# akofke/fountain

Measured on AMD Instinct MI355X. Metric: Mrays/s (primary+secondary) at fixed spp, higher is better.
Workload: dtype f32

## Files before the change

fountain_amd/csrc/ftn_device.h:

```cpp
#ifndef FTN_DEVICE_H
#define FTN_DEVICE_H

#include <hip/hip_runtime.h>
#include "ftn_math.h"
#include "../../include/fountain_hip.h"

namespace ftn {

#define FTN_DEV_NOINLINE __device__ inline

#define FTN_GS 3
enum : uint32_t { GF_KIND_SPHERE = 1u, GF_HAS_NORMALS = 2u, GF_HAS_UVS = 4u, GF_FLIP = 8u, GF_LEAF_END = 16u , GF_HAS_TANGENTS = 32u  };
enum : uint32_t { LK_POINT = 0, LK_DISTANT = 1, LK_INFINITE = 2, LK_AREA = 3 };

struct DSphere {
    float o2w[16], o2w_inv[16], w2o[16];
    float radius, z_min, z_max, theta_min, theta_max, phi_max;
    uint32_t reverse_orientation, _pad;
};

struct DLight {
    uint32_t kind; int32_t prim;
    float rgb[3];
    float v[3];
    float world_center[3]; float world_radius; float area;
    uint32_t env_w, env_h;
    const float4* texels;
    const float* cond_func;
    const float* cond_cdf;
    const float* cond_integral;
    const float* marg_func;
    const float* marg_cdf;
    float marg_integral; uint32_t nu, nv, _pad;
    float l2w[16], w2l[16];
    const float* cond_coarse; const float* marg_coarse;
    const float4* cells;
};

struct DImage { uint32_t w, h, wrap, n_levels; uint32_t off[16], lw[16], lh[16]; };

struct DScene {
    const float4* nodes; const float4* geom; const uint4* prim_info;
    uint32_t geom_stride, _pad_gs;
    const float* N; const float* UV;
    const float* T;
    const DSphere* spheres; const ftn_material* materials; const DLight* lights;
    uint32_t n_nodes, n_prims, n_lights, n_inf_lights, n_spheres, _pad;
    const uint32_t* inf_lights;
    const float4* fat;
    float root_lo[3], root_hi[3];
    uint32_t root_is_leaf, n_fat;
    const ftn_texture* textures; const ftn_material_textures* mtex; const DImage* images; const float4* texels;
    uint32_t n_textures;
    uint32_t material_types;
    uint32_t env_only, _pad2;
    DLight env0;
    const float4* srec;
    const float4* quad;
    uint32_t n_quads, quad_stack_bound;
    const uint4* oct; const float4* oct_xbox;
    uint32_t n_octs, oct_stack_bound;
    const unsigned char* prim_class;
};

struct DCamera {
    float c2w[16]; float r2c[16];
    float shutter_open, shutter_close, lens_radius, focal_dist;
    float dx_camera[3], dy_camera[3];
};

struct DRay { V3 o, d; float t_max, time; };
struct DHit { float t; int prim; float b0, b1, b2; };
struct DSurfHit { V3 p, p_err, n; float time; };
struct DSI { DSurfHit hit; V3 wo, shading_n, s_dpdu; int prim; int mat, light;  };
struct DSIX { V2 uv; V3 dpdu, dpdv, dndu, dndv; };

__device__ inline DRay spawn_ray(const DSurfHit& h, V3 dir) {
    DRay r; r.o = offset_ray_origin(h.p, h.p_err, h.n, dir); r.d = dir; r.t_max = FTN_INF; r.time = h.time; return r;
}
__device__ inline DRay spawn_ray_to_hit(const DSurfHit& a, const DSurfHit& to) {
    V3 origin = offset_ray_origin(a.p, a.p_err, a.n, to.p - a.p);
    V3 target = offset_ray_origin(to.p, to.p_err, to.n, origin - to.p);
    DRay r; r.o = origin; r.d = target - origin; r.t_max = 1.0f - 0.0001f; r.time = a.time; return r;
}

__device__ inline bool slab_test(float4 nlo, float4 nhi, V3 o, V3 inv, float t_max);
__device__ inline bool slab_test_node(float4 a, float4 b, V3 o, V3 inv, float t_max) {
    return slab_test(make_float4(a.x, a.z, b.x, 0.0f), make_float4(a.y, a.w, b.y, 0.0f), o, inv, t_max);
}
__device__ inline bool slab_test(float4 nlo, float4 nhi, V3 o, V3 inv, float t_max) {
    const float k = 1.0f + 2.0f * gamma_n(3);
    float tnx = (nlo.x - o.x) * inv.x, tfx = (nhi.x - o.x) * inv.x;
    float tny = (nlo.y - o.y) * inv.y, tfy = (nhi.y - o.y) * inv.y;
    float tnz = (nlo.z - o.z) * inv.z, tfz = (nhi.z - o.z) * inv.z;
    if (tnx > tfx) { float s = tnx; tnx = tfx; tfx = s; }
    if (tny > tfy) { float s = tny; tny = tfy; tfy = s; }
    if (tnz > tfz) { float s = tnz; tnz = tfz; tfz = s; }
    tfx *= k; tfy *= k; tfz *= k;
    const float t0 = fmax_(fmax_(fmax_(0.0f, tnx), tny), tnz);
    const float t1 = fmin_(fmin_(fmin_(t_max, tfx), tfy), tfz);
    return !(t0 > t1);
}
__device__ inline bool slab_test_node_iv(float4 a, float4 b, V3 o, V3 inv, float t_max, float* t0o, float* t1o) {
    const float k = 1.0f + 2.0f * gamma_n(3);
    float tnx = (a.x - o.x) * inv.x, tfx = (a.y - o.x) * inv.x;
    float tny = (a.z - o.y) * inv.y, tfy = (a.w - o.y) * inv.y;
    float tnz = (b.x - o.z) * inv.z, tfz = (b.y - o.z) * inv.z;
    if (tnx > tfx) { float s = tnx; tnx = tfx; tfx = s; }
    if (tny > tfy) { float s = tny; tny = tfy; tfy = s; }
    if (tnz > tfz) { float s = tnz; tnz = tfz; tfz = s; }
    tfx *= k; tfy *= k; tfz *= k;
    const float t0 = fmax_(fmax_(fmax_(0.0f, tnx), tny), tnz);
    const float t1 = fmin_(fmin_(fmin_(t_max, tfx), tfy), tfz);
    *t0o = t0; *t1o = t1;
    return !(t0 > t1);
}
__device__ inline void pin4(float4& v) { asm volatile("" : "+v"(v.x), "+v"(v.y), "+v"(v.z), "+v"(v.w)); }

__device__ inline bool tri_hit(V3 o, V3 d, float t_max, V3 p0, V3 p1, V3 p2, float* t_out, float* b0o, float* b1o, float* b2o) {
    V3 p0t = p0 - o, p1t = p1 - o, p2t = p2 - o;
    int kz = max_dimension(vabs(d));
    int kx = kz + 1; if (kx == 3) kx = 0;
    int ky = kx + 1; if (ky == 3) ky = 0;
    V3 dir(d.get(kx), d.get(ky), d.get(kz));
    p0t = V3(p0t.get(kx), p0t.get(ky), p0t.get(kz));
    p1t = V3(p1t.get(kx), p1t.get(ky), p1t.get(kz));
    p2t = V3(p2t.get(kx), p2t.get(ky), p2t.get(kz));
    float sx = -dir.x / dir.z, sy = -dir.y / dir.z, sz = 1.0f / dir.z;
    p0t.x += sx * p0t.z; p0t.y += sy * p0t.z;
    p1t.x += sx * p1t.z; p1t.y += sy * p1t.z;
    p2t.x += sx * p2t.z; p2t.y += sy * p2t.z;
    float e0 = p1t.x * p2t.y - p1t.y * p2t.x;
    float e1 = p2t.x * p0t.y - p2t.y * p0t.x;
    float e2 = p0t.x * p1t.y - p0t.y * p1t.x;
    if (e0 == 0.0f || e1 == 0.0f || e2 == 0.0f) {
        e0 = (float)((double)p1t.x * (double)p2t.y - (double)p1t.y * (double)p2t.x);
        e1 = (float)((double)p2t.x * (double)p0t.y - (double)p2t.y * (double)p0t.x);
        e2 = (float)((double)p0t.x * (double)p1t.y - (double)p0t.y * (double)p1t.x);
    }
    if (sign_pos(e0) != sign_pos(e1) || sign_pos(e1) != sign_pos(e2)) return false;
    float det = e0 + e1 + e2;
    if (det == 0.0f) return false;
    p0t.z *= sz; p1t.z *= sz; p2t.z *= sz;
    float t_scaled = e0 * p0t.z + e1 * p1t.z + e2 * p2t.z;
    if ((det < 0.0f && (t_scaled >= 0.0f || t_scaled < t_max * det)) || (det > 0.0f && (t_scaled <= 0.0f || t_scaled > t_max * det)))
        return false;
    float inv_det = 1.0f / det;
    float b0 = e0 * inv_det, b1 = e1 * inv_det, b2 = e2 * inv_det;
    float t = t_scaled * inv_det;
    float max_zt = fmax_(fmax_(fabsf(p0t.z), fabsf(p1t.z)), fabsf(p2t.z));
    float delta_z = gamma_n(3) * max_zt;
    float max_xt = fmax_(fmax_(fabsf(p0t.x), fabsf(p1t.x)), fabsf(p2t.x));
    float max_yt = fmax_(fmax_(fabsf(p0t.y), fabsf(p1t.y)), fabsf(p2t.y));
    float delta_x = gamma_n(5) * (max_xt + max_zt);
    float delta_y = gamma_n(5) * (max_yt + max_zt);
    float delta_e = 2.0f * (gamma_n(2) * max_xt * max_yt + delta_y * max_xt + delta_x * max_yt);
    float max_e = fmax_(fmax_(fabsf(e0), fabsf(e1)), fabsf(e2));
    float delta_t = 3.0f * (gamma_n(3) * max_e * max_zt + delta_e * max_zt + delta_z * max_e) * fabsf(inv_det);
    if (t <= delta_t) return false;
    *t_out = t; *b0o = b0; *b1o = b1; *b2o = b2;
    return true;
}
__device__ inline void prim_mat_light(const DScene& S, int prim, int* mat, int* light) {
    if (S.srec) { const float4* R = S.srec + 8 * (size_t)prim; *mat = (int)__float_as_uint(R[1].w); *light = (int)__float_as_uint(R[2].w); }
    else { const uint4 pi = S.prim_info[2 * prim]; *mat = (int)pi.x; *light = (int)pi.y; }
}
__device__ inline void prim_normals(const DScene& S, int prim, V3* n0, V3* n1, V3* n2) {
    if (S.srec) { const float4* R = S.srec + 8 * (size_t)prim; const float4 r3 = R[3], r4 = R[4], r5 = R[5]; *n0 = V3(r3.x, r3.y, r3.z); *n1 = V3(r4.x, r4.y, r4.z); *n2 = V3(r5.x, r5.y, r5.z); }
    else { const uint4 vi = S.prim_info[2 * prim + 1]; const float* N = S.N;
           *n0 = V3(N[3 * vi.x], N[3 * vi.x + 1], N[3 * vi.x + 2]); *n1 = V3(N[3 * vi.y], N[3 * vi.y + 1], N[3 * vi.y + 2]); *n2 = V3(N[3 * vi.z], N[3 * vi.z + 1], N[3 * vi.z + 2]); }
}
__device__ inline void prim_uvs(const DScene& S, int prim, float* u0x, float* u0y, float* u1x, float* u1y, float* u2x, float* u2y) {
    if (S.srec) { const float4* R = S.srec + 8 * (size_t)prim; const float4 r6 = R[6]; *u0x = R[3].w; *u0y = R[4].w; *u1x = R[5].w; *u1y = r6.x; *u2x = r6.y; *u2y = r6.z; }
    else { const uint4 vi = S.prim_info[2 * prim + 1]; const float* UV = S.UV;
           *u0x = UV[2 * vi.x]; *u0y = UV[2 * vi.x + 1]; *u1x = UV[2 * vi.y]; *u1y = UV[2 * vi.y + 1]; *u2x = UV[2 * vi.z]; *u2y = UV[2 * vi.z + 1]; }
}
__device__ inline bool tri_uv_degenerate_reject(const DScene& S, int prim, V3 p0, V3 p1, V3 p2) {
    float u0x, u0y, u1x, u1y, u2x, u2y;
    prim_uvs(S, prim, &u0x, &u0y, &u1x, &u1y, &u2x, &u2y);
    float determinant = (u0x - u2x) * (u1y - u2y) - (u0y - u2y) * (u1x - u2x);
    if (!(fabsf(determinant) < 1.0e-8f)) return false;
    V3 ng = cross(p2 - p0, p1 - p0);
    return len2(ng) == 0.0f;
}

__device__ inline bool sphere_clipped(const DSphere& s, V3 p, float phi) {
    return (s.z_min > -s.radius && p.z < s.z_min) || (s.z_max < s.radius && p.z > s.z_max) || phi > s.phi_max;
}
template <bool FILL = true>
FTN_DEV_NOINLINE bool sphere_intersect(const DSphere& s, const DRay& wr, float* t_out, DSI* si, DSIX* ex = nullptr) {
    V3 o_err, d_err;
    V3 ot = m4_point_exact_to_err(s.w2o, wr.o, &o_err);
    V3 dt_ = m4_vector_exact_to_err(s.w2o, wr.d, &d_err);
    float tmax = wr.t_max;
    float lsq = len2(dt_);
    if (lsq > 0.0f) { float dt = dot(vabs(dt_), o_err) / lsq; ot = ot + dt_ * dt; tmax -= dt; }
    EF ox = ef_err(ot.x, o_err.x), oy = ef_err(ot.y, o_err.y), oz = ef_err(ot.z, o_err.z);
    EF dx = ef_err(dt_.x, d_err.x), dy = ef_err(dt_.y, d_err.y), dz = ef_err(dt_.z, d_err.z);
    EF a = dx * dx + dy * dy + dz * dz;
    EF b = EF(2.0f) * (dx * ox + dy * oy + dz * oz);
    EF c = ox * ox + oy * oy + oz * oz - EF(s.radius) * EF(s.radius);
    EF t0, t1;
    if (!quadratic(a, b, c, &t0, &t1)) return false;
    if (t0.hi > tmax || t1.lo <= 0.0f) return false;
    EF th = t0;
    if (th.lo <= 0.0f) { th = t1; if (th.hi > tmax) return false; }
    V3 p = ot + (dt_ * th.v);
    p = p * (s.radius / len(p - V3(0.0f, 0.0f, 0.0f)));
    if (p.x == 0.0f && p.y == 0.0f) p.x = 1.0e-5f * s.radius;
    float phi = ftn_det::atan2f_det(p.y, p.x);
    if (phi < 0.0f) phi += 2.0f * FTN_PI;
    if (sphere_clipped(s, p, phi)) {
        if (th.v == t1.v) return false;
        if (t1.hi > tmax) return false;
// ... 760 lines not shown
```

fountain_amd/csrc/ftn_host.cpp:

```cpp
#include "ftn_kernels.h"
#include "ftn_wavefront.h"
#include "ftn_texture.h"

#include <algorithm>
#include <chrono>
#include <cstdio>
#include <cstring>
#include <string>
#include <vector>
#include <thread>
#include <memory>
#include <sched.h>
#include <atomic>
#include <limits>
#include <functional>
#include <cstdlib>

using namespace ftn;

static_assert(sizeof(ftn_transform) == 128 && sizeof(ftn_pixel) == 16 && sizeof(ftn_bvh_node) == 32 && sizeof(ftn_prim) == 16, "ABI");
static_assert(sizeof(ftn_mesh) == 20 && sizeof(ftn_sphere) == 288 && sizeof(ftn_material) == 48 && sizeof(ftn_light) == 160, "ABI");
static_assert(sizeof(ftn_envmap) == 16 && sizeof(ftn_camera_desc) == 296 && sizeof(ftn_film_desc) == 32 && sizeof(ftn_sampler_desc) == 24, "ABI");
static_assert(sizeof(ftn_integrator_desc) == 16 && sizeof(ftn_tile_range) == 16 && sizeof(ftn_render_options) == 16 && sizeof(ftn_stats) == 152, "ABI");

// ... 334 lines not shown
    }
    if (owners.size() >= (1u << 24)) return;
    out->n_records = (uint32_t)owners.size();
    out->rec.assign((size_t)32 * owners.size(), 0.0f);
    std::vector<uint32_t> bound(owners.size(), 0);
    const float kInf = std::numeric_limits<float>::infinity();
    auto put = [&](float* slot, const ftn_bvh_node* c, uint32_t c_index, uint32_t axis_bits) {
        uint32_t link = 0, meta = axis_bits;
        if (!c) { slot[0] = 0.0f; slot[1] = 0.0f; slot[2] = 0.0f; slot[3] = 0.0f; slot[4] = kInf; slot[5] = kInf; link = 0xffffffffu; meta |= 1u << 25; }
        else {
            slot[0] = c->bmin[0]; slot[1] = c->bmax[0]; slot[2] = c->bmin[1]; slot[3] = c->bmax[1]; slot[4] = c->bmin[2]; slot[5] = c->bmax[2];
            if (c->is_leaf) { link = c->idx | 0x80000000u; meta |= 1u << 24; }
            else link = owner_id[c_index] * 128u;
        }
        slot[6] = ftn_det::u2f(link); slot[7] = ftn_det::u2f(meta);
    };
    parallel_for(owners.size(), [&](size_t q0, size_t q1) {
        for (size_t q = q0; q < q1; q++) {
            const uint32_t r = owners[q];
            const uint32_t ch[2] = {r + 1u, nodes[r].idx};
            float* R = &out->rec[(size_t)32 * q];
            for (int k = 0; k < 2; k++) {
                const ftn_bvh_node& c = nodes[ch[k]];
                const uint32_t axes = k == 0 ? ((c.is_leaf ? 0u : (1u << c.axis)) | ((1u << nodes[r].axis) << 8) | ((nodes[ch[1]].is_leaf ? 0u : (1u << nodes[ch[1]].axis)) << 16)) : 0u;
                if (c.is_leaf) { put(R + 16 * k, &c, ch[k], axes); put(R + 16 * k + 8, nullptr, 0, 0u); }
                else { const uint32_t g0 = ch[k] + 1u, g1 = c.idx; put(R + 16 * k, &nodes[g0], g0, axes); put(R + 16 * k + 8, &nodes[g1], g1, 0u); }
            }
        }
    });
    for (size_t q = owners.size(); q-- > 0;) {
        const uint32_t r = owners[q];
        const uint32_t ch[2] = {r + 1u, nodes[r].idx};
        uint32_t valid = 0, deepest = 0;
        for (int k = 0; k < 2; k++) {
            const ftn_bvh_node& c = nodes[ch[k]];
            if (c.is_leaf) valid += 1;
            else {
                const uint32_t g0 = ch[k] + 1u, g1 = c.idx; valid += 2;
                if (!nodes[g0].is_leaf) deepest = std::max(deepest, bound[owner_id[g0]]);
                if (!nodes[g1].is_leaf) deepest = std::max(deepest, bound[owner_id[g1]]);
            }
        }
        bound[q] = (valid - 1u) + deepest;
    }
    out->stack_bound = bound[0];
    out->ok = true;
}

struct OctBvh { std::vector<uint32_t> rec; std::vector<float4> xbox; uint32_t n_records = 0, stack_bound = 0; bool ok = false; };
static void build_octs(const std::vector<ftn_bvh_node>& nodes, const std::vector<float4>& geom, OctBvh* out) {
    out->rec.clear(); out->xbox.clear(); out->n_records = 0; out->stack_bound = 0; out->ok = false;
    if (nodes.empty() || nodes[0].is_leaf) return;
    auto area = [&](uint32_t i) { const ftn_bvh_node& n = nodes[i]; const double dx = (double)n.bmax[0] - n.bmin[0], dy = (double)n.bmax[1] - n.bmin[1], dz = (double)n.bmax[2] - n.bmin[2]; return 2.0 * (dx * dy + dy * dz + dz * dx); };
    struct Rec { uint32_t root; uint32_t child[8]; int n; };
    std::vector<Rec> recs; std::vector<uint32_t> rec_of(nodes.size(), 0xffffffffu);
    {
        std::vector<uint32_t> todo{0u};
        while (!todo.empty()) {
            const uint32_t r = todo.back(); todo.pop_back();
            Rec R; R.root = r; R.n = 2; R.child[0] = r + 1u; R.child[1] = nodes[r].idx;
            for (;;) {
                if (R.n == 8) break;
                int best = -1; double ba = -1.0;
                for (int k = 0; k < R.n; k++) if (!nodes[R.child[k]].is_leaf) { const double a = area(R.child[k]); if (a > ba) { ba = a; best = k; } }
                if (best < 0) break;
                const uint32_t c = R.child[best];
                R.child[best] = c + 1u; R.child[R.n++] = nodes[c].idx;
            }
            rec_of[r] = (uint32_t)recs.size(); recs.push_back(R);
            for (int k = R.n - 1; k >= 0; k--) if (!nodes[R.child[k]].is_leaf) todo.push_back(R.child[k]);
        }
    }
    if (recs.size() >= (1u << 24)) return;
    out->rec.assign((size_t)32 * recs.size(), 0u);
    std::vector<uint32_t> bound(recs.size(), 0);
    auto leaf_is_implicit = [&](const ftn_bvh_node& c) {
        if (c.n_prims != 1 || geom.empty()) return false;
        const float4 g0 = geom[(size_t)FTN_GS * c.idx], g1 = geom[(size_t)FTN_GS * c.idx + 1], g2 = geom[(size_t)FTN_GS * c.idx + 2];
        if (ftn_det::f2u(g0.w) & GF_KIND_SPHERE) return false;
        const float lo[3] = {std::min(std::min(g0.x, g1.x), g2.x), std::min(std::min(g0.y, g1.y), g2.y), std::min(std::min(g0.z, g1.z), g2.z)};
        const float hi[3] = {std::max(std::max(g0.x, g1.x), g2.x), std::max(std::max(g0.y, g1.y), g2.y), std::max(std::max(g0.z, g1.z), g2.z)};
        for (int a = 0; a < 3; a++) if (ftn_det::f2u(lo[a]) != ftn_det::f2u(c.bmin[a]) || ftn_det::f2u(hi[a]) != ftn_det::f2u(c.bmax[a])) return false;
        return true;
    };
    std::vector<uint8_t> xmask(recs.size(), 0);
    parallel_for(recs.size(), [&](size_t q0, size_t q1) {
        for (size_t q = q0; q < q1; q++) {
            const Rec& R = recs[q]; uint8_t m = 0;
            for (int k = 0; k < R.n; k++) { const ftn_bvh_node& c = nodes[R.child[k]]; if (c.is_leaf && !leaf_is_implicit(c)) m |= (uint8_t)(1u << k); }
            xmask[q] = m;
        }
    });
    std::vector<uint32_t> xbase(recs.size(), 0);
    { uint32_t run = 0; for (size_t q = recs.size(); q-- > 0;) { xbase[q] = run; run += (uint32_t)__builtin_popcount(xmask[q]); } out->xbox.assign(2 * (size_t)run, make_float4(0.0f, 0.0f, 0.0f, 0.0f)); }
    parallel_for(recs.size(), [&](size_t q0, size_t q1) {
    for (size_t q = q0; q < q1; q++) {
        const Rec& R = recs[q];
        const ftn_bvh_node& root = nodes[R.root];
        uint32_t* W = &out->rec[(size_t)32 * q];
        uint32_t ebits[3]; float step[3];
        for (int a = 0; a < 3; a++) {
            const double ext = (double)root.bmax[a] - (double)root.bmin[a];
            int e = ext > 0.0 ? (int)ceil(log2(ext / 255.0)) : -126;
            if (e < -126) e = -126;
            for (;; e++) {
                bool fits = true;
                const float st = ldexpf(1.0f, e);
                for (int k = 0; k < R.n && fits; k++) {
                    const ftn_bvh_node& c = nodes[R.child[k]];
                    const double qh = ceil(((double)c.bmax[a] - (double)root.bmin[a]) / (double)st);
                    if (qh > 254.0) fits = false;
                }
                if (fits || e >= 126) break;
            }
            step[a] = ldexpf(1.0f, e); ebits[a] = (uint32_t)(e + 127);
            memcpy(&W[a], &root.bmin[a], 4);
        }
        W[3] = ebits[0] | (ebits[1] << 8) | (ebits[2] << 16);
        uint32_t xi = xbase[q];
        for (int k = 0; k < 8; k++) {
            uint32_t link = 0xffffffffu; uint32_t qb[6] = {255u, 0u, 255u, 0u, 255u, 0u};
            if (k < R.n) {
                const uint32_t ci = R.child[k]; const ftn_bvh_node& c = nodes[ci];
                for (int a = 0; a < 3; a++) {
                    const double o = (double)root.bmin[a], stp = (double)step[a];
                    double ql = floor(((double)c.bmin[a] - o) / stp), qh = ceil(((double)c.bmax[a] - o) / stp);
                    while (ql > 0.0 && o + ql * stp > (double)c.bmin[a]) ql -= 1.0;
                    while (o + qh * stp < (double)c.bmax[a]) qh += 1.0;
                    if (ql < 0.0) ql = 0.0;
                    if (qh > 255.0) qh = 255.0;
                    qb[2 * a] = (uint32_t)ql; qb[2 * a + 1] = (uint32_t)qh;
                }
                if (!c.is_leaf) link = rec_of[ci] * 128u;
                else if (!((xmask[q] >> k) & 1u)) link = 0x80000000u | c.idx;
                else {
                    link = 0xc0000000u | xi;
                    out->xbox[2 * (size_t)xi] = make_float4(c.bmin[0], c.bmin[1], c.bmin[2], ftn_det::u2f(c.idx));
                    out->xbox[2 * (size_t)xi + 1] = make_float4(c.bmax[0], c.bmax[1], c.bmax[2], 0.0f);
                    xi++;
                }
            }
            W[4 + k] = link;
            for (int j = 0; j < 6; j++) W[12 + 2 * j + (k >> 2)] |= qb[j] << (8 * (k & 3));
        }
    }
    });
    for (size_t q = recs.size(); q-- > 0;) {
        const Rec& R = recs[q]; uint32_t deepest = 0;
        for (int k = 0; k < R.n; k++) if (!nodes[R.child[k]].is_leaf) deepest = std::max(deepest, bound[rec_of[R.child[k]]]);
        bound[q] = (uint32_t)(R.n - 1) + deepest;
    }
    if (out->xbox.size() / 2 >= (1u << 30) || nodes.size() >= (1u << 30)) return;
    out->n_records = (uint32_t)recs.size(); out->stack_bound = bound[0]; out->ok = true;
}

static int bvh_default_threads() {
    int cores = (int)std::thread::hardware_concurrency();
#ifdef __linux__
    cpu_set_t set; CPU_ZERO(&set);
    if (sched_getaffinity(0, sizeof(set), &set) == 0) { const int c = CPU_COUNT(&set); if (c > 0) cores = c; }
#endif
    int ranks = 1;
    if (const char* e = getenv("LOCAL_WORLD_SIZE")) { const int r = atoi(e); if (r > 1) ranks = r; }
    return std::max(1, cores / ranks);
}

struct HostScene {
    std::vector<ftn_bvh_node> nodes; std::vector<uint32_t> order; uint32_t max_depth = 0; Aabb world;
    std::vector<int32_t> light_kind, light_prim;
};

static Aabb prim_bounds(const ftn_scene_desc* d, const ftn_prim& p) {
    Aabb b = aabb_empty();
    if (p.shape_kind == FTN_SHAPE_TRIANGLE) {
        for (int k = 0; k < 3; k++) { uint32_t v = d->tri_indices[3 * (size_t)p.shape_index + k]; aabb_join_point(b, V3(d->P[3 * v], d->P[3 * v + 1], d->P[3 * v + 2])); }
    } else {
        const ftn_sphere& s = d->spheres[p.shape_index];
        const float lo[3] = {-s.radius, -s.radius, s.z_min}, hi[3] = {s.radius, s.radius, s.z_max};
        for (int c = 0; c < 8; c++) {
            V3 q((c & 4) ? hi[0] : lo[0], (c & 2) ? hi[1] : lo[1], (c & 1) ? hi[2] : lo[2]);
            aabb_join_point(b, m4_point(s.object_to_world.m, q));
        }
    }
    return b;
}
static int validate_desc(const ftn_scene_desc* d) {
    if (!d) return fail(FTN_ERR_INVALID_ARGUMENT, "null scene description");
    if ((d->n_prims && !d->prims) || (d->n_triangles && (!d->tri_indices || !d->tri_mesh)) || (d->n_vertices && !d->P) || (d->n_meshes && !d->meshes) ||
        (d->n_spheres && !d->spheres) || (d->n_materials && !d->materials) || (d->n_area_emit && !d->area_emit) || (d->n_lights && !d->lights) || (d->n_envmaps && !d->envmaps))
        return fail(FTN_ERR_INVALID_ARGUMENT, "a count is non-zero but its array is NULL");
    for (uint32_t i = 0; i < d->n_materials; i++) if (d->materials[i].type > FTN_MAT_GLASS) return fail(FTN_ERR_INVALID_ARGUMENT, "unknown material type");
    for (uint32_t i = 0; i < d->n_meshes; i++) {
        if (d->meshes[i].has_normals && !d->N) return fail(FTN_ERR_INVALID_ARGUMENT, "a mesh has normals but N is NULL");
        if (d->meshes[i].has_uvs && !d->UV) return fail(FTN_ERR_INVALID_ARGUMENT, "a mesh has uvs but UV is NULL");
        if (d->meshes[i].has_tangents && !d->S) return fail(FTN_ERR_INVALID_ARGUMENT, "a mesh has tangents but S is NULL");
    }
    for (uint32_t i = 0; i < d->n_envmaps; i++) if (!d->envmaps[i].texels) return fail(FTN_ERR_INVALID_ARGUMENT, "environment map without texels");
    if (d->n_textures && d->textures) {
        const int nt = (int)d->n_textures, ni = d->images ? (int)d->n_images : 0;
        for (int i = 0; i < nt; i++) {
            const ftn_texture& t = d->textures[i];
            if (t.kind > FTN_TEX_IMAGE) return fail(FTN_ERR_INVALID_ARGUMENT, "unknown texture kind");
            if (t.kind == FTN_TEX_CHECKERBOARD && (t.tex1 < 0 || t.tex1 >= nt || t.tex2 < 0 || t.tex2 >= nt)) return fail(FTN_ERR_INVALID_ARGUMENT, "checkerboard child texture out of range");
            if (t.kind == FTN_TEX_IMAGE && (t.image < 0 || t.image >= ni)) return fail(FTN_ERR_INVALID_ARGUMENT, "image index out of range");
        }
        for (int i = 0; i < ni; i++) { const ftn_image& im = d->images[i]; if (im.width == 0 || im.height == 0 || !im.texels || im.wrap > FTN_WRAP_CLAMP) return fail(FTN_ERR_INVALID_ARGUMENT, "bad image"); }
        if (d->material_textures) for (uint32_t i = 0; i < d->n_materials; i++) { const ftn_material_textures& mt = d->material_textures[i];
            for (int32_t id : {mt.a, mt.b, mt.s0, mt.s1, mt.s2}) if (id >= nt) return fail(FTN_ERR_INVALID_ARGUMENT, "material texture index out of range"); }
    }
    for (uint32_t i = 0; i < d->n_triangles; i++) {
        if (d->tri_mesh[i] >= d->n_meshes) return fail(FTN_ERR_INVALID_ARGUMENT, "triangle mesh id out of range");
        for (int k = 0; k < 3; k++) if (d->tri_indices[3 * (size_t)i + k] >= d->n_vertices) return fail(FTN_ERR_INVALID_ARGUMENT, "vertex index out of range");
    }
    for (uint32_t i = 0; i < d->n_prims; i++) {
        const ftn_prim& p = d->prims[i];
        if (p.shape_kind == FTN_SHAPE_TRIANGLE) { if (p.shape_index >= d->n_triangles) return fail(FTN_ERR_INVALID_ARGUMENT, "triangle index out of range"); }
        else if (p.shape_kind == FTN_SHAPE_SPHERE) { if (p.shape_index >= d->n_spheres) return fail(FTN_ERR_INVALID_ARGUMENT, "sphere index out of range"); }
        else return fail(FTN_ERR_INVALID_ARGUMENT, "unknown shape kind");
        if (p.material >= (int)d->n_materials || p.area_emit >= (int)d->n_area_emit) return fail(FTN_ERR_INVALID_ARGUMENT, "material / area light index out of range");
    }
    for (uint32_t i = 0; i < d->n_envmaps; i++) {
        uint32_t w = d->envmaps[i].width, h = d->envmaps[i].height;
        if (w == 0 || h == 0) return fail(FTN_ERR_INVALID_ARGUMENT, "environment map without texels");
    }
    for (uint32_t i = 0; i < d->n_lights; i++) {
        if (d->lights[i].type > FTN_LIGHT_INFINITE) return fail(FTN_ERR_INVALID_ARGUMENT, "unknown light type");
        if (d->lights[i].type == FTN_LIGHT_INFINITE && (d->lights[i].envmap < 0 || d->lights[i].envmap >= (int)d->n_envmaps)) return fail(FTN_ERR_INVALID_ARGUMENT, "envmap index out of range");
    }
    return FTN_OK;
}
static int build_host_scene(const ftn_scene_desc* d, HostScene* hs) {
    int rc = validate_desc(d); if (rc) return rc;
    std::vector<Aabb> pb(d->n_prims);
    parallel_for(d->n_prims, [&](size_t i0, size_t i1) { for (size_t i = i0; i < i1; i++) pb[i] = prim_bounds(d, d->prims[i]); });
    hs->world = aabb_empty();
    if (d->n_prims) {
        BvhBuilder b(pb);
        int n_threads = bvh_default_threads();
        if (const char* e = getenv("FTN_BVH_THREADS")) n_threads = atoi(e);
        if (n_threads > 32) n_threads = 32;
        if (n_threads > 1 && d->n_prims >= (1u << 16)) {
            const bool dbg = getenv("FTN_BVH_DEBUG") != nullptr;
            auto t0 = std::chrono::steady_clock::now();
            ParallelBvh pb2(b, std::max<size_t>(4096, d->n_prims / (size_t)(n_threads * 8)));
            auto root = pb2.split(0, d->n_prims, 0);
            auto t1 = std::chrono::steady_clock::now();
            pb2.run_tasks(n_threads);
            auto t2 = std::chrono::steady_clock::now();
            pb2.stitch(root, n_threads);
            auto t3 = std::chrono::steady_clock::now();
            if (dbg) fprintf(stderr, "[ftn bvh] %d threads, %zu tasks: top split %.2fs, subtrees %.2fs, stitch %.2fs\n", n_threads, pb2.tasks.size(),
                             std::chrono::duration<double>(t1 - t0).count(), std::chrono::duration<double>(t2 - t1).count(), std::chrono::duration<double>(t3 - t2).count());
            std::function<void(int, bool, uint32_t)> walk = [&](int i, bool t, uint32_t dep) { if (t) return; if (dep > b.max_depth) b.max_depth = dep; walk(pb2.tops[i].child[0], pb2.tops[i].is_task[0], dep + 1); walk(pb2.tops[i].child[1], pb2.tops[i].is_task[1], dep + 1); };
            walk(root.first, root.second, 0);
        } else b.build(0, d->n_prims, 0);
        hs->nodes.swap(b.nodes); hs->order.swap(b.leaf_order); hs->max_depth = b.max_depth;
        for (int k = 0; k < 3; k++) { hs->world.lo[k] = hs->nodes[0].bmin[k]; hs->world.hi[k] = hs->nodes[0].bmax[k]; }
    }
    for (uint32_t i = 0; i < d->n_lights; i++) { hs->light_kind.push_back((int)d->lights[i].type); hs->light_prim.push_back(-1); }
    for (size_t i = 0; i < hs->order.size(); i++) if (d->prims[hs->order[i]].area_emit >= 0) { hs->light_kind.push_back((int)LK_AREA); hs->light_prim.push_back((int)i); }
    return FTN_OK;
}

static float dist1d_build(const float* f, size_t n, float* cdf) {
    cdf[0] = 0.0f;
    for (size_t i = 1; i < n + 1; i++) cdf[i] = cdf[i - 1] + (f[i - 1] / (float)n);
    float integral = cdf[n];
    if (integral == 0.0f) { for (size_t i = 1; i < n + 1; i++) cdf[i] = (float)i / (float)n; }
    else { for (size_t i = 1; i < n + 1; i++) cdf[i] /= integral; }
    return integral;
}

template <class T> struct DevBuf {
    T* p = nullptr; size_t n = 0;
    int upload(const T* src, size_t count) {
        n = count; if (!count) return FTN_OK;
        HIP_TRY(hipMalloc((void**)&p, count * sizeof(T)));
        HIP_TRY(hipMemcpy(p, src, count * sizeof(T), hipMemcpyHostToDevice));
        return FTN_OK;
    }
    int alloc_zero(size_t count) {
        n = count; if (!count) return FTN_OK;
        HIP_TRY(hipMalloc((void**)&p, count * sizeof(T)));
        HIP_TRY(hipMemset(p, 0, count * sizeof(T)));
        return FTN_OK;
    }
    void release() { if (p) (void)hipFree(p); p = nullptr; n = 0; }
};

}

namespace {
struct MipLevelHost { uint32_t w, h; std::vector<float> rgb; };
struct TapLine { size_t first; std::vector<float> w; };
static std::vector<TapLine> triangle_taps(size_t n_src, size_t n_dst) {
    const float ratio = (float)n_src / (float)n_dst;
    const float scale = ratio > 1.0f ? ratio : 1.0f;
    const float radius = ceilf(scale);
    std::vector<TapLine> lines(n_dst);
    for (size_t j = 0; j < n_dst; j++) {
        const float centre = ((float)j + 0.5f) * ratio - 0.5f;
        long lo = (long)ceilf(centre - radius), hi = (long)floorf(centre + radius);
        lo = std::min<long>(std::max<long>(lo, 0), (long)n_src - 1); hi = std::min<long>(std::max<long>(hi, 0), (long)n_src - 1);
        float total = 0.0f;
        for (long k = lo; k <= hi; k++) total += fmaxf(1.0f - fabsf(((float)k - centre) / scale), 0.0f);
        lines[j].first = (size_t)lo;
        for (long k = lo; k <= hi; k++) lines[j].w.push_back(fmaxf(1.0f - fabsf(((float)k - centre) / scale), 0.0f) / total);
    }
    return lines;
}
static void shrink_triangle(uint32_t w1, uint32_t h1, uint32_t w2, uint32_t h2, const std::vector<float>& src, std::vector<float>* dst) {
    const std::vector<TapLine> across = triangle_taps(w1, w2), down = triangle_taps(h1, h2);
    std::vector<float> mid((size_t)w1 * h2 * 3);
    for (size_t x = 0; x < w1; x++)
        for (size_t y = 0; y < h2; y++) {
            float a0 = 0.0f, a1 = 0.0f, a2 = 0.0f; const TapLine& L = down[y];
            for (size_t k = 0; k < L.w.size(); k++) { const float* q = &src[((L.first + k) * w1 + x) * 3]; a0 += q[0] * L.w[k]; a1 += q[1] * L.w[k]; a2 += q[2] * L.w[k]; }
            float* o = &mid[(x * h2 + y) * 3]; o[0] = a0; o[1] = a1; o[2] = a2;
        }
    dst->assign((size_t)w2 * h2 * 3, 0.0f);
    for (size_t y = 0; y < h2; y++)
        for (size_t x = 0; x < w2; x++) {
            float a0 = 0.0f, a1 = 0.0f, a2 = 0.0f; const TapLine& L = across[x];
            for (size_t k = 0; k < L.w.size(); k++) { const float* q = &mid[((L.first + k) * h2 + y) * 3]; a0 += q[0] * L.w[k]; a1 += q[1] * L.w[k]; a2 += q[2] * L.w[k]; }
            float* o = &(*dst)[(y * w2 + x) * 3]; o[0] = a0; o[1] = a1; o[2] = a2;
        }
}
static void build_mip_pyramid(uint32_t w, uint32_t h, const float* rgb, std::vector<MipLevelHost>* out) {
    out->clear();
    MipLevelHost l0; l0.w = w; l0.h = h; l0.rgb.assign(rgb, rgb + (size_t)w * h * 3); out->push_back(l0);
    uint32_t big = std::max(w, h); int n_levels = 1; while (big >>= 1) n_levels++;
    for (int l = 1; l < n_levels; l++) {
        const MipLevelHost& prev = out->back();
        MipLevelHost nx; nx.w = std::max<uint32_t>(1, prev.w / 2); nx.h = std::max<uint32_t>(1, prev.h / 2);
        shrink_triangle(prev.w, prev.h, nx.w, nx.h, prev.rgb, &nx.rgb);
        out->push_back(std::move(nx));
    }
}
}

struct ftn_scene {
    int device = 0;
    HostScene host;
    DScene d; uint32_t stack_entries = 1;
    DevBuf<float4> nodes, geom, fat, srec, quad, oct_xbox; DevBuf<uint4> prim_info, oct; DevBuf<float> N, UV, T; DevBuf<DSphere> spheres; DevBuf<ftn_material> materials; DevBuf<DLight> lights;
    DevBuf<uint32_t> inf_lights; DevBuf<unsigned char> prim_class; std::vector<DevBuf<float>> misc; std::vector<DevBuf<float4>> misc4;
    DevBuf<ftn_texture> textures; DevBuf<ftn_material_textures> mtex; DevBuf<DImage> images; DevBuf<float4> texels;
    DevBuf<float4> accA, accB, accC; DevBuf<DTile> tiles; DevBuf<DevStats> stats; size_t acc_pixels = 0;
    bool spill_acc_dirty = true;
    WavefrontState* wf = nullptr;
    std::vector<DTile> sel; int32_t tile_key[10] = {0};
    ~ftn_scene() {
        nodes.release(); geom.release(); fat.release(); srec.release(); quad.release(); oct.release(); oct_xbox.release(); prim_info.release(); N.release(); UV.release(); T.release(); spheres.release(); materials.release(); lights.release(); inf_lights.release(); prim_class.release();
        for (auto& b : misc) b.release();
        for (auto& b : misc4) b.release();
        textures.release(); mtex.release(); images.release(); texels.release();
        accA.release(); accB.release(); accC.release(); tiles.release(); stats.release();
        wavefront_destroy(wf);
    }
};

struct PhaseClock {
    bool on; std::chrono::steady_clock::time_point t;
    PhaseClock() : on(getenv("FTN_SCENE_DEBUG") != nullptr), t(std::chrono::steady_clock::now()) {}
    void mark(const char* what) {
        if (!on) return;
        const auto n = std::chrono::steady_clock::now();
        fprintf(stderr, "[ftn scene] %-44s %.3f s\n", what, std::chrono::duration<double>(n - t).count()); t = n;
    }
};
static int upload_scene(const ftn_scene_desc* d, ftn_scene* sc) {
    const HostScene& hs = sc->host;
    PhaseClock clk;
    const size_t np = hs.order.size();
    std::vector<float4> nodes(2 * hs.nodes.size());
    parallel_for(hs.nodes.size(), [&](size_t i0, size_t i1) { for (size_t i = i0; i < i1; i++) {
        const ftn_bvh_node& n = hs.nodes[i];
        nodes[2 * i] = make_float4(n.bmin[0], n.bmax[0], n.bmin[1], n.bmax[1]);
        const uint32_t link = n.is_leaf ? n.idx : n.idx * 32u;
        nodes[2 * i + 1] = make_float4(n.bmin[2], n.bmax[2], ftn_det::u2f(link), ftn_det::u2f((uint32_t)n.n_prims | ((1u << n.axis) << 16) | ((uint32_t)n.is_leaf << 24)));
    } });
    if (hs.nodes.size() >= (1u << 27)) return fail(FTN_ERR_UNSUPPORTED, "more than 2^27 BVH nodes (node links are 32-bit byte offsets)");
    auto env_is = [](const char* name, int value) { const char* v = getenv(name); return v && atoi(v) == value; };
    const bool want_fat = env_is("FTN_TRACE4", 0) || env_is("FTN_QUAD", 0) || env_is("FTN_FAT", 1);
    std::vector<uint32_t> fat_id(want_fat ? hs.nodes.size() : 0, 0xffffffffu);
    uint32_t n_fat = 0;
    if (want_fat) for (size_t i = 0; i < hs.nodes.size(); i++) if (!hs.nodes[i].is_leaf) fat_id[i] = n_fat++;
    std::vector<float4> fat(4 * (size_t)n_fat);
    std::vector<uint8_t> leaf_end(np, 0);
    for (size_t i = 0; i < hs.nodes.size(); i++) {
        const ftn_bvh_node& n = hs.nodes[i];
        if (n.is_leaf) { if (n.n_prims) leaf_end[n.idx + n.n_prims - 1] = 1; continue; }
        if (!want_fat) continue;
        const size_t ch[2] = {i + 1, (size_t)n.idx};
        for (int k = 0; k < 2; k++) {
            const ftn_bvh_node& c = hs.nodes[ch[k]];
            const uint32_t link = c.is_leaf ? c.idx : fat_id[ch[k]] * 64u;
            const uint32_t meta = (uint32_t)c.n_prims | (k == 0 ? ((1u << n.axis) << 16) : 0u) | ((uint32_t)c.is_leaf << 24);
            fat[4 * (size_t)fat_id[i] + 2 * k] = make_float4(c.bmin[0], c.bmax[0], c.bmin[1], c.bmax[1]);
            fat[4 * (size_t)fat_id[i] + 2 * k + 1] = make_float4(c.bmin[2], c.bmax[2], ftn_det::u2f(link), ftn_det::u2f(meta));
        }
    }
    std::vector<int> prim_light(np, -1);
    for (size_t l = 0; l < hs.light_prim.size(); l++) if (hs.light_prim[l] >= 0) prim_light[hs.light_prim[l]] = (int)l;
    std::vector<float4> geom((size_t)FTN_GS * np); std::vector<uint4> info(2 * np);
    parallel_for(np, [&](size_t i0, size_t i1) { for (size_t i = i0; i < i1; i++) {
        const ftn_prim& p = d->prims[hs.order[i]];
        uint32_t fl = 0;
        if (p.shape_kind == FTN_SHAPE_SPHERE) {
            fl = GF_KIND_SPHERE | (leaf_end[i] ? GF_LEAF_END : 0u);
            geom[FTN_GS * i] = make_float4(0, 0, 0, ftn_det::u2f(fl)); geom[FTN_GS * i + 1] = make_float4(0, 0, 0, ftn_det::u2f(p.shape_index)); geom[FTN_GS * i + 2] = make_float4(0, 0, 0, 0);
            info[2 * i + 1] = make_uint4(0, 0, 0, p.shape_index);
        } else {
            const ftn_mesh& m = d->meshes[d->tri_mesh[p.shape_index]];
            if (m.has_normals && d->N) fl |= GF_HAS_NORMALS;
            if (m.has_uvs && d->UV) fl |= GF_HAS_UVS;
            if (m.has_tangents && d->S) fl |= GF_HAS_TANGENTS;
            if (m.flip_normals) fl |= GF_FLIP;
            if (leaf_end[i]) fl |= GF_LEAF_END;
            const uint32_t* vi = d->tri_indices + 3 * (size_t)p.shape_index;
            const float* P = d->P;
            geom[FTN_GS * i] = make_float4(P[3 * vi[0]], P[3 * vi[0] + 1], P[3 * vi[0] + 2], ftn_det::u2f(fl));
            geom[FTN_GS * i + 1] = make_float4(P[3 * vi[1]], P[3 * vi[1] + 1], P[3 * vi[1] + 2], ftn_det::u2f(p.shape_index));
            geom[FTN_GS * i + 2] = make_float4(P[3 * vi[2]], P[3 * vi[2] + 1], P[3 * vi[2] + 2], 0.0f);
            info[2 * i + 1] = make_uint4(vi[0], vi[1], vi[2], p.shape_index);
        }
        info[2 * i] = make_uint4((uint32_t)p.material, (uint32_t)prim_light[i], fl, 0);
    } });
    clk.mark("node records, leaf-test records (host)");
    int rc;
    if ((rc = sc->nodes.upload(nodes.data(), nodes.size()))) return rc;
    clk.mark("upload nodes");
    if (n_fat && n_fat < (1u << 25)) { if ((rc = sc->fat.upload(fat.data(), fat.size()))) return rc; }
    uint32_t n_quads = 0, quad_bound = 0;
    if (!env_is("FTN_QUAD", 0)) {
        QuadBvh qb; build_quads(hs.nodes, &qb);
        if (qb.ok && qb.n_records) {
            if ((rc = sc->quad.upload(reinterpret_cast<const float4*>(qb.rec.data()), (size_t)8 * qb.n_records))) return rc;
            n_quads = qb.n_records; quad_bound = qb.stack_bound;
        }
    }
    clk.mark("four-box records (host + upload)");
    uint32_t n_octs = 0, oct_bound = 0;
    if (!env_is("FTN_OCT", 0) && n_quads != 0 && d->n_spheres == 0) {
        OctBvh ob; build_octs(hs.nodes, geom, &ob);
        if (ob.ok && ob.n_records) {
            if ((rc = sc->oct.upload(reinterpret_cast<const uint4*>(ob.rec.data()), (size_t)8 * ob.n_records))) return rc;
            if (!ob.xbox.empty() && (rc = sc->oct_xbox.upload(ob.xbox.data(), ob.xbox.size()))) return rc;
            n_octs = ob.n_records; oct_bound = ob.stack_bound;
        }
    }
    clk.mark("eight-box records (host + upload)");
    if (!env_is("FTN_SREC", 0) && np != 0 && (uint64_t)np * 128u <= (16ull << 30)) {
        std::unique_ptr<float4[]> rec(new float4[8 * np]);
        parallel_for(np, [&](size_t i0, size_t i1) { for (size_t i = i0; i < i1; i++) {
            float4* R = &rec[8 * i];
            for (int k = 3; k < 8; k++) R[k] = make_float4(0.0f, 0.0f, 0.0f, 0.0f);
            const uint4 pi = info[2 * i], vi = info[2 * i + 1];
            R[0] = geom[FTN_GS * i]; R[1] = geom[FTN_GS * i + 1]; R[2] = geom[FTN_GS * i + 2];
            R[1].w = ftn_det::u2f(pi.x); R[2].w = ftn_det::u2f(pi.y); R[6].w = ftn_det::u2f(vi.w);
            const uint32_t fl = ftn_det::f2u(R[0].w);
            if (fl & GF_KIND_SPHERE) continue;
            const uint32_t v[3] = {vi.x, vi.y, vi.z};
            if (fl & GF_HAS_NORMALS) for (int k = 0; k < 3; k++) { R[3 + k].x = d->N[3 * (size_t)v[k]]; R[3 + k].y = d->N[3 * (size_t)v[k] + 1]; R[3 + k].z = d->N[3 * (size_t)v[k] + 2]; }
            if (fl & GF_HAS_UVS) {
                R[3].w = d->UV[2 * (size_t)v[0]]; R[4].w = d->UV[2 * (size_t)v[0] + 1]; R[5].w = d->UV[2 * (size_t)v[1]];
                R[6].x = d->UV[2 * (size_t)v[1] + 1]; R[6].y = d->UV[2 * (size_t)v[2]]; R[6].z = d->UV[2 * (size_t)v[2] + 1];
            }
        } });
        if ((rc = sc->srec.upload(rec.get(), 8 * np))) return rc;
    }
    clk.mark("shading records (host + upload)");
    const bool geom_in_srec = sc->srec.p != nullptr && d->n_spheres == 0 && !env_is("FTN_GEOM", 1);
    if (!geom_in_srec && (rc = sc->geom.upload(geom.data(), geom.size()))) return rc;
    bool any_tangents = false;
    for (uint32_t i = 0; i < d->n_meshes; i++) if (d->meshes[i].has_tangents && d->S) any_tangents = true;
    if (!sc->srec.p || any_tangents || env_is("FTN_LEGACY_ARRAYS", 1)) {
        if ((rc = sc->prim_info.upload(info.data(), info.size()))) return rc;
        if (d->N && (rc = sc->N.upload(d->N, 3 * (size_t)d->n_vertices))) return rc;
        if (d->UV && (rc = sc->UV.upload(d->UV, 2 * (size_t)d->n_vertices))) return rc;
    }
    if (any_tangents && (rc = sc->T.upload(d->S, 3 * (size_t)d->n_vertices))) return rc;
    std::vector<DSphere> sph(d->n_spheres);
    for (uint32_t i = 0; i < d->n_spheres; i++) {
        const ftn_sphere& s = d->spheres[i]; DSphere& o = sph[i];
        memcpy(o.o2w, s.object_to_world.m, 64); memcpy(o.o2w_inv, s.object_to_world.inv, 64); memcpy(o.w2o, s.world_to_object.m, 64);
        o.radius = s.radius; o.z_min = s.z_min; o.z_max = s.z_max; o.theta_min = s.theta_min; o.theta_max = s.theta_max; o.phi_max = s.phi_max;
        o.reverse_orientation = s.reverse_orientation; o._pad = 0;
    }
    if ((rc = sc->spheres.upload(sph.data(), sph.size()))) return rc;
    std::vector<ftn_material> mats(d->materials, d->materials + d->n_materials);
    const bool has_tex = d->n_textures != 0 && d->textures != nullptr;
    for (size_t i = 0; i < mats.size(); i++) {
        bool textured = false;
        if (has_tex && d->material_textures) { const ftn_material_textures& mt = d->material_textures[i]; textured = (mt.a & mt.b & mt.s0 & mt.s1 & mt.s2) >= 0; }
        if (!textured) material_finalize(mats[i]);
    }
    if ((rc = sc->materials.upload(mats.data(), mats.size()))) return rc;
    clk.mark("leaf-test / attribute arrays, spheres, materials");
    {
        std::vector<unsigned char> cls(np);
        for (size_t i = 0; i < np; i++) { const int m = (int)info[2 * i].x; cls[i] = (unsigned char)(m < 0 || (size_t)m >= mats.size() ? 7u : std::min<uint32_t>(2u + mats[(size_t)m].type, 7u)); }
        if ((rc = sc->prim_class.upload(cls.data(), cls.size()))) return rc;
    }
    std::vector<DLight> lights(hs.light_kind.size());
    std::vector<uint32_t> inf;
    V3 wc((hs.world.lo[0] + hs.world.hi[0]) / 2.0f, (hs.world.lo[1] + hs.world.hi[1]) / 2.0f, (hs.world.lo[2] + hs.world.hi[2]) / 2.0f);
    wc = V3(0.0f, 0.0f, 0.0f) + wc;
    float wr = len(wc - V3(hs.world.hi[0], hs.world.hi[1], hs.world.hi[2]));
    for (size_t l = 0; l < lights.size(); l++) {
        DLight& L = lights[l]; memset(&L, 0, sizeof(L));
        L.kind = (uint32_t)hs.light_kind[l]; L.prim = hs.light_prim[l];
        if (L.kind == LK_AREA) {
            const ftn_prim& p = d->prims[hs.order[L.prim]];
            for (int k = 0; k < 3; k++) L.rgb[k] = d->area_emit[3 * p.area_emit + k];
            if (p.shape_kind == FTN_SHAPE_SPHERE) { const ftn_sphere& s = d->spheres[p.shape_index]; L.area = s.phi_max * s.radius * (s.z_max - s.z_min); }
            else {
                const uint32_t* vi = d->tri_indices + 3 * (size_t)p.shape_index; const float* P = d->P;
                V3 p0(P[3 * vi[0]], P[3 * vi[0] + 1], P[3 * vi[0] + 2]), p1(P[3 * vi[1]], P[3 * vi[1] + 1], P[3 * vi[1] + 2]), p2(P[3 * vi[2]], P[3 * vi[2] + 1], P[3 * vi[2] + 2]);
                L.area = 0.5f * len(cross(p1 - p0, p2 - p0));
            }
            continue;
        }
        const ftn_light& src = d->lights[l];
        for (int k = 0; k < 3; k++) { L.rgb[k] = src.rgb[k]; L.v[k] = src.v[k]; }
        if (L.kind == LK_DISTANT || L.kind == LK_INFINITE) { L.world_center[0] = wc.x; L.world_center[1] = wc.y; L.world_center[2] = wc.z; L.world_radius = wr; }
        if (L.kind == LK_INFINITE) {
            inf.push_back((uint32_t)l);
            const ftn_envmap& e = d->envmaps[src.envmap];
            memcpy(L.l2w, src.light_to_world.m, 64); memcpy(L.w2l, src.light_to_world.inv, 64);
            L.env_w = e.width; L.env_h = e.height;
            const uint32_t height = e.width, width = e.height;
            std::vector<float4> tex4((size_t)e.width * e.height);
            for (size_t k = 0; k < tex4.size(); k++) tex4[k] = make_float4(e.texels[3 * k], e.texels[3 * k + 1], e.texels[3 * k + 2], 0.0f);
            DLight hostL = L; hostL.texels = tex4.data();
            std::vector<float> img((size_t)width * height);
            for (uint32_t j = 0; j < height; j++) {
                float v = (float)j / (float)height;
                float sin_theta = ftn_det::sinf_det(FTN_PI * ((float)j + 0.5f) / (float)height);
                for (uint32_t i = 0; i < width; i++) {
                    float u = (float)i / (float)width;
                    Rgb tex = (e.width == 1 && e.height == 1) ? env_texel(hostL, 0, 0) : env_lookup(hostL, V2(u, v));
                    img[i + (size_t)j * width] = tex.luminance() * sin_theta;
                }
            }
            const uint32_t nu = width, nv = height;
            std::vector<float> ccdf((size_t)nv * (nu + 1)), cint(nv), mcdf(nv + 1);
            for (uint32_t v2 = 0; v2 < nv; v2++) cint[v2] = dist1d_build(&img[(size_t)v2 * nu], nu, &ccdf[(size_t)v2 * (nu + 1)]);
            float mint = dist1d_build(cint.data(), nv, mcdf.data());
            L.nu = nu; L.nv = nv; L.marg_integral = mint;
            DevBuf<float4> b0; DevBuf<float> b1, b2, b3, b4, b5;
            if ((rc = b0.upload(tex4.data(), tex4.size()))) return rc;
            if ((rc = b1.upload(img.data(), img.size()))) return rc;
            if ((rc = b2.upload(ccdf.data(), ccdf.size()))) return rc;
            if ((rc = b3.upload(cint.data(), cint.size()))) return rc;
            if ((rc = b4.upload(cint.data(), cint.size()))) return rc;
            if ((rc = b5.upload(mcdf.data(), mcdf.size()))) return rc;
            L.texels = b0.p; L.cond_func = b1.p; L.cond_cdf = b2.p; L.cond_integral = b3.p; L.marg_func = b4.p; L.marg_cdf = b5.p;
            if (e.width == e.height && (uint64_t)e.width * e.height * 128u <= (2ull << 30) && !env_is("FTN_ENV_CELLS", 0)) {
                const int w = (int)e.width, h = (int)e.height;
                std::unique_ptr<float4[]> cells(new float4[8 * (size_t)w * h]);
                parallel_for((size_t)h, [&](size_t y0, size_t y1) { for (size_t cy = y0; cy < y1; cy++) for (int cx = 0; cx < w; cx++) {
                    float* c = reinterpret_cast<float*>(&cells[8 * (cy * (size_t)w + (size_t)cx)]);
                    for (int dy = -1; dy <= 1; dy++) for (int dx = -1; dx <= 1; dx++) {
                        const int sx = ((cx + dx) % w + w) % w, sy = (((int)cy + dy) % h + h) % h;
                        const float4 t = tex4[(size_t)sy * w + sx];
                        float* o = c + 3 * ((dy + 1) * 3 + dx + 1);
                        o[0] = t.x; o[1] = t.y; o[2] = t.z;
                    }
                    c[27] = img[(size_t)cx + cy * (size_t)width];
                    c[28] = c[29] = c[30] = c[31] = 0.0f;
                } });
                DevBuf<float4> bc;
                if ((rc = bc.upload(cells.get(), 8 * (size_t)w * h))) return rc;
                L.cells = bc.p; sc->misc4.push_back(bc);
            }
            {
                bool monotone = true;
                auto check = [&](const float* c, uint32_t n) { for (uint32_t k = 0; k < n; k++) if (!(c[k] <= c[k + 1])) monotone = false; };
                for (uint32_t v2 = 0; v2 < nv; v2++) check(&ccdf[(size_t)v2 * (nu + 1)], nu);
                check(mcdf.data(), nv);
                if (monotone && !getenv("FTN_NO_COARSE_CDF")) {
                    const uint32_t nbu = (nu + 31u) / 32u, nbv = (nv + 31u) / 32u;
                    std::vector<float> cc((size_t)nv * (nbu + 1)), mc(nbv + 1);
                    for (uint32_t v2 = 0; v2 < nv; v2++) for (uint32_t k = 0; k <= nbu; k++) cc[(size_t)v2 * (nbu + 1) + k] = ccdf[(size_t)v2 * (nu + 1) + std::min(k * 32u, nu)];
                    for (uint32_t k = 0; k <= nbv; k++) mc[k] = mcdf[std::min(k * 32u, nv)];
                    DevBuf<float> b6, b7;
                    if ((rc = b6.upload(cc.data(), cc.size()))) return rc;
                    if ((rc = b7.upload(mc.data(), mc.size()))) return rc;
                    L.cond_coarse = b6.p; L.marg_coarse = b7.p;
                    sc->misc.push_back(b6); sc->misc.push_back(b7);
                }
            }
            sc->misc4.push_back(b0); sc->misc.push_back(b1); sc->misc.push_back(b2); sc->misc.push_back(b3); sc->misc.push_back(b4); sc->misc.push_back(b5);
        }
    }
    if ((rc = sc->lights.upload(lights.data(), lights.size()))) return rc;
    if ((rc = sc->inf_lights.upload(inf.data(), inf.size()))) return rc;
    clk.mark("classes, lights, environment tables, textures");
    DScene& D = sc->d; memset(&D, 0, sizeof(D));
    D.nodes = sc->nodes.p; D.geom = geom_in_srec ? sc->srec.p : sc->geom.p; D.geom_stride = geom_in_srec ? 8u : (uint32_t)FTN_GS; D.prim_info = sc->prim_info.p; D.N = sc->N.p; D.UV = sc->UV.p; D.T = sc->T.p; D.spheres = sc->spheres.p;
    D.materials = sc->materials.p; D.lights = sc->lights.p; D.inf_lights = sc->inf_lights.p;
    D.n_nodes = (uint32_t)hs.nodes.size(); D.n_prims = (uint32_t)np; D.n_lights = (uint32_t)lights.size(); D.n_inf_lights = (uint32_t)inf.size(); D.n_spheres = d->n_spheres;
    D.srec = sc->srec.p; D.prim_class = sc->prim_class.p;
    D.quad = sc->quad.p; D.n_quads = n_quads; D.quad_stack_bound = quad_bound;
    D.oct = sc->oct.p; D.oct_xbox = sc->oct_xbox.p; D.n_octs = n_octs; D.oct_stack_bound = oct_bound;
    D.fat = sc->fat.p; D.n_fat = n_fat; D.root_is_leaf = (!hs.nodes.empty() && hs.nodes[0].is_leaf) ? 1u : 0u;
    for (int k = 0; k < 3; k++) { D.root_lo[k] = hs.nodes.empty() ? 0.0f : hs.nodes[0].bmin[k]; D.root_hi[k] = hs.nodes.empty() ? 0.0f : hs.nodes[0].bmax[k]; }
    if (lights.size() == 1 && lights[0].kind == LK_INFINITE) { D.env_only = 1; D.env0 = lights[0]; }
    sc->stack_entries = std::max<uint32_t>(hs.max_depth, 1u);
    for (const ftn_material& m : mats) if (m.type < 32u) D.material_types |= 1u << m.type;
    if ((rc = sc->stats.alloc_zero(1))) return rc;
    if (has_tex) {
        const int nt = (int)d->n_textures, ni = d->images ? (int)d->n_images : 0;
        for (int i = 0; i < nt; i++) {
            const ftn_texture& t = d->textures[i];
            if (t.kind > FTN_TEX_IMAGE) return fail(FTN_ERR_INVALID_ARGUMENT, "unknown texture kind");
            if (t.kind == FTN_TEX_CHECKERBOARD && (t.tex1 < 0 || t.tex1 >= nt || t.tex2 < 0 || t.tex2 >= nt)) return fail(FTN_ERR_INVALID_ARGUMENT, "checkerboard child texture out of range");
            if (t.kind == FTN_TEX_IMAGE && (t.image < 0 || t.image >= ni)) return fail(FTN_ERR_INVALID_ARGUMENT, "image index out of range");
        }
        std::vector<ftn_material_textures> mt(d->n_materials);
        for (uint32_t i = 0; i < d->n_materials; i++) {
            if (d->material_textures) mt[i] = d->material_textures[i]; else { mt[i].a = mt[i].b = mt[i].s0 = mt[i].s1 = mt[i].s2 = -1; }
            for (int32_t id : {mt[i].a, mt[i].b, mt[i].s0, mt[i].s1, mt[i].s2}) if (id >= nt) return fail(FTN_ERR_INVALID_ARGUMENT, "material texture index out of range");
        }
        std::vector<DImage> imgs((size_t)ni); std::vector<float4> texels;
        for (int i = 0; i < ni; i++) {
            const ftn_image& im = d->images[i];
            if (im.width == 0 || im.height == 0 || !im.texels || im.wrap > FTN_WRAP_CLAMP) return fail(FTN_ERR_INVALID_ARGUMENT, "bad image");
            std::vector<MipLevelHost> pyr; build_mip_pyramid(im.width, im.height, im.texels, &pyr);
            if (pyr.size() > 16) return fail(FTN_ERR_UNSUPPORTED, "image larger than 32768 texels on a side");
            DImage& D2 = imgs[(size_t)i]; memset(&D2, 0, sizeof(D2));
            D2.w = im.width; D2.h = im.height; D2.wrap = im.wrap; D2.n_levels = (uint32_t)pyr.size();
            for (size_t l = 0; l < pyr.size(); l++) {
                D2.off[l] = (uint32_t)texels.size(); D2.lw[l] = pyr[l].w; D2.lh[l] = pyr[l].h;
                for (size_t k = 0; k < (size_t)pyr[l].w * pyr[l].h; k++) texels.push_back(make_float4(pyr[l].rgb[3 * k], pyr[l].rgb[3 * k + 1], pyr[l].rgb[3 * k + 2], 0.0f));
            }
        }
        if ((rc = sc->textures.upload(d->textures, (size_t)nt)) || (rc = sc->mtex.upload(mt.data(), mt.size())) || (rc = sc->images.upload(imgs.data(), imgs.size())) ||
            (rc = sc->texels.upload(texels.data(), texels.size()))) return rc;
        D.textures = sc->textures.p; D.mtex = sc->mtex.p; D.images = sc->images.p; D.texels = sc->texels.p; D.n_textures = (uint32_t)nt;
    }
    return FTN_OK;
}

static int set_device(int device) {
    int n = 0;
    if (hipGetDeviceCount(&n) != hipSuccess || n == 0) return fail(FTN_ERR_NO_DEVICE, "no HIP device available: the fountain HIP path needs an AMD GPU (there is no CPU fallback)");
    if (device >= 0) {
        hipError_t e = hipSetDevice(device);
        if (e != hipSuccess) { (void)hipGetLastError();
                               return fail(FTN_ERR_NO_DEVICE, std::string("hipSetDevice(device): ") + hipGetErrorString(e)); }
    }
    return FTN_OK;
}

extern "C" {

const char* ftn_last_error(void) { return g_err.c_str(); }
const char* ftn_version(void) { return "fountain_hip 0.3 (gfx950)"; }
int ftn_abi_version(void) { return FTN_ABI_VERSION; }
int ftn_device_count(void) { int n = 0; if (hipGetDeviceCount(&n) != hipSuccess) return 0; return n; }

int ftn_bvh_build(const ftn_scene_desc* d, ftn_bvh_node* nodes_out, uint32_t* order_out, uint32_t* n_nodes_out, uint32_t* max_depth_out) {
    HostScene hs; int rc = build_host_scene(d, &hs); if (rc) return rc;
    if (nodes_out) memcpy(nodes_out, hs.nodes.data(), hs.nodes.size() * sizeof(ftn_bvh_node));
    if (order_out) memcpy(order_out, hs.order.data(), hs.order.size() * sizeof(uint32_t));
    if (n_nodes_out) *n_nodes_out = (uint32_t)hs.nodes.size();
    if (max_depth_out) *max_depth_out = hs.max_depth;
    return FTN_OK;
}

int ftn_bvh_quads(const ftn_bvh_node* nodes, uint32_t n_nodes, float* records_out, uint32_t* n_records_out, uint32_t* stack_bound_out) {
    if (!nodes && n_nodes) return fail(FTN_ERR_INVALID_ARGUMENT, "null nodes");
    std::vector<ftn_bvh_node> v(nodes, nodes + n_nodes);
    for (uint32_t i = 0; i < n_nodes; i++) if (!v[i].is_leaf && (v[i].idx <= i + 1 || v[i].idx >= n_nodes || v[i].axis > 2)) return fail(FTN_ERR_INVALID_ARGUMENT, "not a flattened BVH (bvh.rs:133-158)");
    QuadBvh qb; build_quads(v, &qb);
    if (!qb.ok) return fail(FTN_ERR_UNSUPPORTED, "more than 2^24 four-box records");
    if (records_out) memcpy(records_out, qb.rec.data(), qb.rec.size() * sizeof(float));
    if (n_records_out) *n_records_out = qb.n_records;
    if (stack_bound_out) *stack_bound_out = qb.stack_bound;
    return FTN_OK;
}

int ftn_bvh_octs(const ftn_bvh_node* nodes, uint32_t n_nodes, uint32_t* records_out, uint32_t* n_records_out, uint32_t* stack_bound_out, float* xbox_out, uint32_t* n_xbox_out) {
    if (!nodes && n_nodes) return fail(FTN_ERR_INVALID_ARGUMENT, "null nodes");
    std::vector<ftn_bvh_node> v(nodes, nodes + n_nodes);
    for (uint32_t i = 0; i < n_nodes; i++) if (!v[i].is_leaf && (v[i].idx <= i + 1 || v[i].idx >= n_nodes || v[i].axis > 2)) return fail(FTN_ERR_INVALID_ARGUMENT, "not a flattened BVH (bvh.rs:133-158)");
    OctBvh ob; build_octs(v, std::vector<float4>(), &ob);
    if (!ob.ok) return fail(FTN_ERR_UNSUPPORTED, "no interior node, or more than 2^24 eight-box records");
    if (records_out) memcpy(records_out, ob.rec.data(), ob.rec.size() * sizeof(uint32_t));
    if (n_records_out) *n_records_out = ob.n_records;
    if (stack_bound_out) *stack_bound_out = ob.stack_bound;
    if (xbox_out) memcpy(xbox_out, ob.xbox.data(), ob.xbox.size() * sizeof(float4));
    if (n_xbox_out) *n_xbox_out = (uint32_t)(ob.xbox.size() / 2);
    return FTN_OK;
}

int ftn_scene_create(const ftn_scene_desc* d, int device, ftn_scene** out) {
    if (!out) return fail(FTN_ERR_INVALID_ARGUMENT, "null output");
    int rc = set_device(device); if (rc) return rc;
    ftn_scene* sc = new ftn_scene();
    sc->device = device;
    PhaseClock clk;
    rc = build_host_scene(d, &sc->host);
    clk.mark("host scene: bounds, BVH, lights");
    if (!rc && sc->host.max_depth > 64) rc = fail(FTN_ERR_BVH_TOO_DEEP, "BVH deeper than the reference's 64-entry traversal stack (bvh.rs:168)");
    if (!rc) rc = upload_scene(d, sc);
    if (rc) { delete sc; return rc; }
    *out = sc; return FTN_OK;
}
void ftn_scene_destroy(ftn_scene* s) { delete s; }
int ftn_scene_info(const ftn_scene* s, uint32_t* n_nodes, uint32_t* n_prims, uint32_t* n_lights, uint32_t* max_depth, float wb[6]) {
    if (n_nodes) *n_nodes = (uint32_t)s->host.nodes.size();
    if (n_prims) *n_prims = (uint32_t)s->host.order.size();
    if (n_lights) *n_lights = (uint32_t)s->host.light_kind.size();
    if (max_depth) *max_depth = s->host.max_depth;
    if (wb) for (int i = 0; i < 3; i++) { wb[i] = s->host.world.lo[i]; wb[3 + i] = s->host.world.hi[i]; }
    return FTN_OK;
}
int ftn_scene_memory_info(const ftn_scene* s, ftn_scene_memory* m) {
    if (!s || !m) return fail(FTN_ERR_INVALID_ARGUMENT, "null scene / output");
    memset(m, 0, sizeof(*m));
    m->oct = s->oct.n * sizeof(uint4) + s->oct_xbox.n * sizeof(float4);
    m->nodes = s->nodes.n * sizeof(float4); m->quad = s->quad.n * sizeof(float4); m->fat = s->fat.n * sizeof(float4); m->geom = s->geom.n * sizeof(float4);
    m->srec = s->srec.n * sizeof(float4); m->indexed_attributes = s->prim_info.n * sizeof(uint4) + (s->N.n + s->UV.n + s->T.n) * sizeof(float);
    m->prim_class = s->prim_class.n;
    m->lights = s->lights.n * sizeof(DLight) + s->inf_lights.n * sizeof(uint32_t);
    for (const auto& b : s->misc) m->lights += b.n * sizeof(float);
    for (const auto& b : s->misc4) m->lights += b.n * sizeof(float4);
    m->textures = s->textures.n * sizeof(ftn_texture) + s->mtex.n * sizeof(ftn_material_textures) + s->images.n * sizeof(DImage) + s->texels.n * sizeof(float4);
    m->other = s->spheres.n * sizeof(DSphere) + s->materials.n * sizeof(ftn_material) + s->stats.n * sizeof(DevStats);
    m->total = m->oct + m->nodes + m->quad + m->fat + m->geom + m->srec + m->indexed_attributes + m->prim_class + m->lights + m->textures + m->other;
    return FTN_OK;
}
int ftn_scene_get_nodes(const ftn_scene* s, ftn_bvh_node* nodes, uint32_t* order) {
    if (nodes) memcpy(nodes, s->host.nodes.data(), s->host.nodes.size() * sizeof(ftn_bvh_node));
    if (order) memcpy(order, s->host.order.data(), s->host.order.size() * sizeof(uint32_t));
    return FTN_OK;
}
int ftn_scene_get_lights(const ftn_scene* s, int32_t* kind, int32_t* prim) {
    for (size_t i = 0; i < s->host.light_kind.size(); i++) { kind[i] = s->host.light_kind[i]; prim[i] = s->host.light_prim[i]; }
    return FTN_OK;
}

static void stats_out(const DevStats& ds, ftn_stats* st, double ms) {
    if (!st) return;
    memset(st, 0, sizeof(*st));
    st->rays_closest = ds.rays_closest; st->rays_any = ds.rays_any; st->nodes_visited = ds.nodes_visited; st->prims_tested = ds.prims_tested;
    st->camera_samples = ds.camera_samples; st->spill_samples = ds.spill_samples; st->kernel_ms = ms;
    st->nodes_visited_any = ds.nodes_any; st->prims_tested_any = ds.prims_any;
    st->quad_records = ds.quad_records; st->quad_records_any = ds.quad_records_any;
}
static int trace_batch(const ftn_scene* cs, const float* rays, size_t n, int mode, float* t_hit, int32_t* prim, float* bary, uint8_t* occ, float* out24, ftn_stats* st) {
    ftn_scene* s = const_cast<ftn_scene*>(cs);
    int rc = set_device(s->device); if (rc) return rc;
    DevBuf<float> d_rays, d_t, d_b, d_o; DevBuf<int> d_p; DevBuf<unsigned char> d_occ;
    auto cleanup = [&]() { d_rays.release(); d_t.release(); d_b.release(); d_o.release(); d_p.release(); d_occ.release(); };
    if ((rc = d_rays.upload(rays, 8 * n))) { cleanup(); return rc; }
    if (mode == 0) { if ((rc = d_t.alloc_zero(n)) || (rc = d_p.alloc_zero(n)) || (rc = d_b.alloc_zero(3 * n))) { cleanup(); return rc; } }
    else if (mode == 1) { if ((rc = d_occ.alloc_zero(n))) { cleanup(); return rc; } }
    else { if ((rc = d_o.alloc_zero(24 * n))) { cleanup(); return rc; } }
    HIP_TRY(hipMemset(s->stats.p, 0, sizeof(DevStats)));
    hipEvent_t e0, e1; HIP_TRY(hipEventCreate(&e0)); HIP_TRY(hipEventCreate(&e1));
    HIP_TRY(hipEventRecord(e0, 0));
    if (getenv("FTN_BATCH_SIMPLE")) launch_trace_batch(s->d, d_rays.p, n, mode, d_t.p, d_p.p, d_b.p, d_occ.p, d_o.p, s->stats.p, s->stack_entries, st != nullptr, 0);
    else if ((rc = wavefront_trace_batch(&s->wf, s->d, s->stack_entries, d_rays.p, n, mode, st != nullptr, d_t.p, d_p.p, d_b.p, d_occ.p, d_o.p, s->stats.p, 0))) { cleanup(); return fail(rc, wavefront_error()); }
    HIP_TRY(hipEventRecord(e1, 0));
    HIP_TRY(hipEventSynchronize(e1));
    HIP_TRY(hipGetLastError());
    float ms = 0.0f; (void)hipEventElapsedTime(&ms, e0, e1); (void)hipEventDestroy(e0); (void)hipEventDestroy(e1);
    if (t_hit) HIP_TRY(hipMemcpy(t_hit, d_t.p, n * 4, hipMemcpyDeviceToHost));
    if (prim) HIP_TRY(hipMemcpy(prim, d_p.p, n * 4, hipMemcpyDeviceToHost));
    if (bary) HIP_TRY(hipMemcpy(bary, d_b.p, 3 * n * 4, hipMemcpyDeviceToHost));
    if (occ) HIP_TRY(hipMemcpy(occ, d_occ.p, n, hipMemcpyDeviceToHost));
    if (out24) HIP_TRY(hipMemcpy(out24, d_o.p, 24 * n * 4, hipMemcpyDeviceToHost));
    DevStats ds; HIP_TRY(hipMemcpy(&ds, s->stats.p, sizeof(ds), hipMemcpyDeviceToHost));
    stats_out(ds, st, ms);
    cleanup();
    return FTN_OK;
}
int ftn_intersect(const ftn_scene* s, const float* rays, size_t n, float* t_hit, int32_t* prim, float* bary, ftn_stats* st) {
    return trace_batch(s, rays, n, 0, t_hit, prim, bary, nullptr, nullptr, st);
}
int ftn_intersect_test(const ftn_scene* s, const float* rays, size_t n, uint8_t* occluded, ftn_stats* st) {
    return trace_batch(s, rays, n, 1, nullptr, nullptr, nullptr, occluded, nullptr, st);
}
int ftn_intersect_full(const ftn_scene* s, const float* rays, size_t n, float* out24) {
    return trace_batch(s, rays, n, 2, nullptr, nullptr, nullptr, nullptr, out24, nullptr);
}

int ftn_render_device(const ftn_scene* cs, const ftn_camera_desc* cam, const ftn_film_desc* film, const ftn_sampler_desc* sd, const ftn_integrator_desc* id,
                      const ftn_tile_range* tr, const ftn_render_options* opt, void* device_pixels, void* stream_v, ftn_stats* st) {
    if (!cs || !cam || !film || !sd || !id || !device_pixels) return fail(FTN_ERR_INVALID_ARGUMENT, "null argument");
    ftn_scene* s = const_cast<ftn_scene*>(cs);
    if (opt && opt->device >= 0 && s->device >= 0 && opt->device != s->device) return fail(FTN_ERR_INVALID_ARGUMENT, "ftn_render_options.device differs from the device the scene was created on");
    int rc = set_device(opt && opt->device >= 0 ? opt->device : s->device); if (rc) return rc;
    hipStream_t stream = (hipStream_t)stream_v;
    const bool indexed = sd->kind == FTN_SAMPLER_INDEXED;
    if (indexed && ((uint64_t)sd->first_sample > (uint64_t)sd->samples_per_pixel || (uint64_t)sd->first_sample + (uint64_t)sd->sample_count > (uint64_t)sd->samples_per_pixel))
        return fail(FTN_ERR_INVALID_ARGUMENT, "sample range outside [0, samples_per_pixel]");
    if (!indexed && sd->kind != FTN_SAMPLER_TILE_SERIAL) return fail(FTN_ERR_INVALID_ARGUMENT, "unknown sampler kind");
    if (!indexed && (sd->first_sample != 0 || (sd->sample_count != 0 && sd->sample_count != sd->samples_per_pixel)))
        return fail(FTN_ERR_INVALID_ARGUMENT, "sample ranges need FTN_SAMPLER_INDEXED");
    if (id->kind != FTN_INTEGRATOR_PATH && id->kind != FTN_INTEGRATOR_DIRECT_LIGHTING && id->kind != FTN_INTEGRATOR_WHITTED) return fail(FTN_ERR_INVALID_ARGUMENT, "unknown integrator kind");
    if (id->max_depth > 65535u) return fail(FTN_ERR_INVALID_ARGUMENT, "max_depth is a u16 in the reference (integrator/path.rs:14)");
    uint32_t pipeline = opt ? opt->pipeline : FTN_PIPELINE_AUTO;
    const bool wf_ok = indexed ? (id->kind != FTN_INTEGRATOR_WHITTED || s->d.n_lights <= 32u) : id->kind == FTN_INTEGRATOR_PATH;
    const bool auto_pipeline = pipeline == FTN_PIPELINE_AUTO;
    if (auto_pipeline) pipeline = wf_ok ? FTN_PIPELINE_WAVEFRONT : FTN_PIPELINE_MEGAKERNEL;
    if (pipeline == FTN_PIPELINE_WAVEFRONT && !wf_ok)
        return fail(FTN_ERR_UNSUPPORTED, "the wavefront pipeline renders PathIntegrator with either sampler, DirectLightingIntegrator / WhittedIntegrator (up to 32 lights) with FTN_SAMPLER_INDEXED");
    const bool count = opt && opt->count_traffic;
    const bool count_production = opt && opt->count_traffic == 2;

    const uint32_t stride = tr && tr->stride ? tr->stride : 1, first = tr ? tr->first : 0, cnt = tr ? tr->count : 0;
    int32_t key[10] = {film->crop[0], film->crop[1], film->crop[2], film->crop[3], (int32_t)ftn_det::f2u(film->filter_radius[0]), (int32_t)ftn_det::f2u(film->filter_radius[1]),
                       (int32_t)first, (int32_t)stride, (int32_t)cnt, 1};
    const bool tiles_cached = memcmp(key, s->tile_key, sizeof(key)) == 0;
    if (!tiles_cached) {
        memset(s->tile_key, 0, sizeof(s->tile_key));
        std::vector<DTile> all; list_tiles(film, &all);
        s->sel.clear();
        for (size_t i = first, k = 0; i < all.size() && (cnt == 0 || k < cnt); i += stride, k++) s->sel.push_back(all[i]);
        uint32_t off = 0; for (DTile& t : s->sel) { t.valid_off = off; t._pad = 0; off += (uint32_t)((t.x1 - t.x0) * (t.y1 - t.y0)); }
    }
    std::vector<DTile>& sel = s->sel;
    if (auto_pipeline && !indexed && pipeline == FTN_PIPELINE_WAVEFRONT && sel.size() < 2048) pipeline = FTN_PIPELINE_MEGAKERNEL;

    RenderParams P; memset(&P, 0, sizeof(P));
    P.S = s->d;
    memcpy(P.C.c2w, cam->camera_to_world.m, 64); memcpy(P.C.r2c, cam->raster_to_camera.m, 64);
    P.C.shutter_open = cam->shutter_open; P.C.shutter_close = cam->shutter_close; P.C.lens_radius = cam->lens_radius; P.C.focal_dist = cam->focal_dist;
    for (int k = 0; k < 3; k++) { P.C.dx_camera[k] = cam->dx_camera[k]; P.C.dy_camera[k] = cam->dy_camera[k]; }
    for (int i = 0; i < 4; i++) P.crop[i] = film->crop[i];
    P.radius[0] = film->filter_radius[0]; P.radius[1] = film->filter_radius[1]; P.inv_radius[0] = 1.0f / P.radius[0]; P.inv_radius[1] = 1.0f / P.radius[1];
    P.sampler_kind = sd->kind; P.spp = sd->samples_per_pixel; P.seed = sd->seed;
    P.first_sample = indexed ? sd->first_sample : 0;
    P.last_sample = indexed ? sd->first_sample + (sd->sample_count ? sd->sample_count : (sd->samples_per_pixel - sd->first_sample)) : sd->samples_per_pixel;
    P.integrator_kind = id->kind; P.max_depth = id->max_depth; P.rr_threshold = id->rr_threshold;
    P.stack_entries = s->stack_entries;

    const size_t npix = (size_t)std::max(0, film->crop[2] - film->crop[0]) * (size_t)std::max(0, film->crop[3] - film->crop[1]);
    if (npix > s->acc_pixels) {
        s->accA.release(); s->accB.release(); s->accC.release();
        HIP_TRY(hipMalloc((void**)&s->accA.p, npix * sizeof(float4))); HIP_TRY(hipMalloc((void**)&s->accB.p, npix * sizeof(float4))); HIP_TRY(hipMalloc((void**)&s->accC.p, npix * sizeof(float4)));
        s->acc_pixels = npix; s->spill_acc_dirty = true;
    }
    if (sel.size() > s->tiles.n) { s->tiles.release(); HIP_TRY(hipMalloc((void**)&s->tiles.p, sel.size() * sizeof(DTile))); s->tiles.n = sel.size(); }
    HIP_TRY(hipMemsetAsync(s->accA.p, 0, npix * sizeof(float4), stream));
    if (s->spill_acc_dirty) {
        HIP_TRY(hipMemsetAsync(s->accB.p, 0, npix * sizeof(float4), stream));
        HIP_TRY(hipMemsetAsync(s->accC.p, 0, npix * sizeof(float4), stream));
    }
    s->spill_acc_dirty = true;
    HIP_TRY(hipMemsetAsync(s->stats.p, 0, sizeof(DevStats), stream));
    if (!tiles_cached) {
        if (!sel.empty()) HIP_TRY(hipMemcpyAsync(s->tiles.p, sel.data(), sel.size() * sizeof(DTile), hipMemcpyHostToDevice, stream));
        memcpy(s->tile_key, key, sizeof(key));
    }
    P.tiles = s->tiles.p; P.n_tiles = (uint32_t)sel.size();
    P.accA = s->accA.p; P.accB = s->accB.p; P.accC = s->accC.p; P.stats = s->stats.p;

    struct EventPair {
        hipEvent_t a = nullptr, b = nullptr;
        ~EventPair() { if (a) (void)hipEventDestroy(a); if (b) (void)hipEventDestroy(b); }
    } ev;
    HIP_TRY(hipEventCreate(&ev.a)); HIP_TRY(hipEventCreate(&ev.b));
    HIP_TRY(hipEventRecord(ev.a, stream));
    WavefrontTimes wt; memset(&wt, 0, sizeof(wt));
    if (pipeline == FTN_PIPELINE_WAVEFRONT) { rc = wavefront_render(&s->wf, P, sel, count, stream, &wt, count_production); if (rc) return fail(rc, wavefront_error()); }
    else launch_render_mega(P, count, stream);
    launch_film_resolve(P, (ftn_pixel*)device_pixels, stream);
    HIP_TRY(hipEventRecord(ev.b, stream));
    HIP_TRY(hipEventSynchronize(ev.b));
    HIP_TRY(hipGetLastError());
    float ms = 0.0f; (void)hipEventElapsedTime(&ms, ev.a, ev.b);
    DevStats ds; HIP_TRY(hipMemcpy(&ds, s->stats.p, sizeof(ds), hipMemcpyDeviceToHost));
// ... 81 lines not shown
```

fountain_amd/csrc/ftn_trace4.hip:

```cpp
#include "ftn_wf_common.h"

namespace ftn {

enum : uint32_t { T4_IDLE = 0, T4_NODE = 1, T4_LEAF = 2 };
#define T4_NONE 0xffffffffu

typedef float t4_f2 __attribute__((ext_vector_type(2)));
__device__ inline bool slab4(float4 a, float4 b, V3 o, V3 inv, float t_max, float* t0o, float* t1o) {
    const float k = 1.0f + 2.0f * gamma_n(3);
    const t4_f2 px = {a.x, a.y}, py = {a.z, a.w}, pz = {b.x, b.y};
    const t4_f2 tx = (px - (t4_f2){o.x, o.x}) * (t4_f2){inv.x, inv.x};
    const t4_f2 ty = (py - (t4_f2){o.y, o.y}) * (t4_f2){inv.y, inv.y};
    const t4_f2 tz = (pz - (t4_f2){o.z, o.z}) * (t4_f2){inv.z, inv.z};
    const float far_k = fmin_(fmin_(fmax_(tx.x, tx.y), fmax_(ty.x, ty.y)), fmax_(tz.x, tz.y)) * k;
    const float t0 = fmax_(fmax_(fmax_(0.0f, fmin_(tx.x, tx.y)), fmin_(ty.x, ty.y)), fmin_(tz.x, tz.y));
    const float t1 = fmin_(t_max, far_k);
    *t0o = t0; *t1o = t1;
    return !(t0 > t1);
}

struct WaveQueue {
    uint32_t chunk_next, chunk_end, slice, slices_done, chunk; bool exhausted;
};
__device__ inline void wq_init(WaveQueue& q, uint32_t count, uint32_t chunk_max) {
    q.chunk_next = 0; q.chunk_end = 0; q.exhausted = count == 0; q.slice = blockIdx.x & 7u; q.slices_done = 0;
    uint32_t c = count / (gridDim.x * 4u * 16u); c &= ~63u; q.chunk = c < 64u ? 64u : (c > chunk_max ? chunk_max : c);
}
__device__ inline bool wq_refill(WaveQueue& q, uint32_t count, uint32_t* head, uint32_t lane) {
    bool just_dry = false;
    while (q.chunk_next == q.chunk_end && !q.exhausted) {
        const uint32_t s_lo = (uint32_t)(((unsigned long long)count * q.slice) >> 3) & ~63u, s_hi = q.slice == 7u ? count : ((uint32_t)(((unsigned long long)count * (q.slice + 1u)) >> 3) & ~63u);
        uint32_t base = 0;
        if (lane == 0) base = atomicAdd(head + CTR(q.slice), q.chunk);
        base = __shfl(base, 0, 64) + s_lo;
        if (base >= s_hi) { q.slice = (q.slice + 1u) & 7u; if (++q.slices_done == 8u) { q.exhausted = true; just_dry = true; } }
        else { q.chunk_next = base; q.chunk_end = base + q.chunk < s_hi ? base + q.chunk : s_hi; }
    }
    return just_dry;
}

struct RaySetup { V3 o, inv, dorig; float t_max, sx, sy, sz; uint32_t neg24 ; int kz; };
__device__ inline bool ray_is_exceptional(float ox, float oy, float oz, float ix, float iy, float iz) {
    return !(fabsf(ix) < FTN_INF && fabsf(iy) < FTN_INF && fabsf(iz) < FTN_INF && ix != 0.0f && iy != 0.0f && iz != 0.0f &&
             fabsf(ox) < FTN_INF && fabsf(oy) < FTN_INF && fabsf(oz) < FTN_INF &&
             fabsf(ox * ix) < FTN_INF && fabsf(oy * iy) < FTN_INF && fabsf(oz * iz) < FTN_INF);
}
template <bool SPHERES>
__device__ inline void ray_setup(RaySetup& R, float4 a, float4 b) {
    R.o = V3(a.x, a.y, a.z); const V3 d(b.x, b.y, b.z); R.t_max = b.w;
    if (SPHERES) R.dorig = d;
    R.inv = V3(1.0f / d.x, 1.0f / d.y, 1.0f / d.z);
    R.neg24 = ((d.x < 0.0f ? 1u : 0u) | (d.y < 0.0f ? 2u : 0u) | (d.z < 0.0f ? 4u : 0u)) * 0x010101u;
    R.kz = max_dimension(vabs(d));
    const bool k0 = R.kz == 0, k1 = R.kz == 1;
    const V3 dperm(k0 ? d.y : (k1 ? d.z : d.x), k0 ? d.z : (k1 ? d.x : d.y), k0 ? d.x : (k1 ? d.y : d.z));
    R.sx = -dperm.x / dperm.z; R.sy = -dperm.y / dperm.z; R.sz = 1.0f / dperm.z;
}

template <class E> struct T4Stack {
    E* base; E* lim; E* sp; E* spill; size_t n_lanes, gl; uint32_t spill_levels;
    __device__ inline size_t spill_at() const { const uint32_t lv = (uint32_t)((sp - lim) >> 8); return (size_t)(lv < spill_levels ? lv : spill_levels - 1u) * n_lanes + gl; }
    template <bool CHECK> __device__ inline void push(E v) {
        if (!CHECK || sp < lim) *sp = v; else if (spill_levels) spill[spill_at()] = v;
        sp += 256;
    }
    template <bool CHECK> __device__ inline E pop() {
        sp -= 256;
        if (!CHECK || sp < lim) return *sp;
        return spill_levels ? spill[spill_at()] : *base;
    }
    __device__ inline bool empty() const { return sp == base; }
};

struct T4Lane { uint32_t mode, cur, lp; bool finish; };

template <bool CHECK>
__device__ inline void t4_pop_next(T4Stack<uint2>& St, T4Lane& L, float t_max) {
    for (;;) {
        if (St.empty()) { L.finish = true; return; }
        const uint2 v = St.template pop<CHECK>();
        if (!(__uint_as_float(v.y) > t_max)) {
            if (v.x >> 31) { L.lp = v.x & 0x7fffffffu; L.mode = T4_LEAF; } else { L.cur = v.x; L.mode = T4_NODE; }
            return;
        }
    }
}

template <bool CHECK>
__device__ inline void t4_record_step(const DScene& S, const RaySetup& R, T4Stack<uint2>& St, T4Lane& L) {
    const float4* rec = reinterpret_cast<const float4*>(reinterpret_cast<const char*>(S.quad) + L.cur);
    const float4 q0 = rec[0], q1 = rec[1], q2 = rec[2], q3 = rec[3], q4 = rec[4], q5 = rec[5], q6 = rec[6], q7 = rec[7];
    float ta, tb, tc, td, x1;
    const bool ha = slab4(q0, q1, R.o, R.inv, R.t_max, &ta, &x1), hb = slab4(q2, q3, R.o, R.inv, R.t_max, &tb, &x1);
    const bool hc = slab4(q4, q5, R.o, R.inv, R.t_max, &tc, &x1), hd = slab4(q6, q7, R.o, R.inv, R.t_max, &td, &x1);
    const uint32_t ea = ha ? __float_as_uint(q1.z) : T4_NONE, eb = hb ? __float_as_uint(q3.z) : T4_NONE, ec = hc ? __float_as_uint(q5.z) : T4_NONE, ed = hd ? __float_as_uint(q7.z) : T4_NONE;
    const uint32_t ax = __float_as_uint(q1.w) & R.neg24;
    const bool sA = (ax & 0xffu) != 0, sR = (ax & 0xff00u) != 0, sB = (ax & 0xff0000u) != 0;
    const uint32_t ex0 = sA ? eb : ea, ex1 = sA ? ea : eb, ey0 = sB ? ed : ec, ey1 = sB ? ec : ed;
    const float tx0 = sA ? tb : ta, tx1 = sA ? ta : tb, ty0 = sB ? td : tc, ty1 = sB ? tc : td;
    const uint32_t e0 = sR ? ey0 : ex0, e1 = sR ? ey1 : ex1, e2 = sR ? ex0 : ey0, e3 = sR ? ex1 : ey1;
    const float t1_ = sR ? ty1 : tx1, t2_ = sR ? tx0 : ty0, t3_ = sR ? tx1 : ty1;
    const bool h0 = e0 != T4_NONE, h1 = e1 != T4_NONE, h2 = e2 != T4_NONE, h3 = e3 != T4_NONE;
    const bool h01 = h0 || h1, h012 = h01 || h2;
    if (h3 && h012) St.template push<CHECK>(make_uint2(e3, __float_as_uint(t3_)));
    if (h2 && h01) St.template push<CHECK>(make_uint2(e2, __float_as_uint(t2_)));
    if (h1 && h0) St.template push<CHECK>(make_uint2(e1, __float_as_uint(t1_)));
    if (h012 || h3) {
        const uint32_t next = h0 ? e0 : (h1 ? e1 : (h2 ? e2 : e3));
        if (next >> 31) { L.lp = next & 0x7fffffffu; L.mode = T4_LEAF; } else L.cur = next;
    } else t4_pop_next<CHECK>(St, L, R.t_max);
}

template <bool COUNT, bool SPHERES, int BURST>
__global__ void __launch_bounds__(256, (SPHERES ? 1 : 5)) k_wf_trace4(DScene S, WfBuffers W, const uint32_t* __restrict__ queue, const uint32_t* count_ptr, uint32_t* head, DevStats* stats,
                                                   uint32_t refill, uint32_t leaf_batch, uint32_t chunk_max, uint32_t lds_entries, uint2* __restrict__ spill, uint32_t spill_levels) {
    T4Stack<uint2> St;
    extern __shared__ uint2 lds_stack2[];
    St.base = lds_stack2 + threadIdx.x;
    St.lim = St.base + 256u * lds_entries; St.sp = St.base; St.spill = spill; St.spill_levels = spill_levels;
    St.n_lanes = (size_t)gridDim.x * 256u; St.gl = (size_t)blockIdx.x * 256u + threadIdx.x;
    const bool st_tiny = lds_entries < 3u;
    uint2* const st_soft = st_tiny ? St.base : St.lim - 3 * 256;
    const uint32_t count = *count_ptr;
    const uint32_t lane = lane_id();
    unsigned long long n_rec = 0, n_prim = 0;
    unsigned long long occ[7] = {0, 0, 0, 0, 0, 0, 0};
    T4Lane L; L.mode = T4_IDLE; L.cur = 0; L.lp = 0; L.finish = false;
    WaveQueue Q; wq_init(Q, count, chunk_max);
    uint32_t rid = 0;
    RaySetup R; R.o = V3(0.0f, 0.0f, 0.0f); R.inv = R.o; R.dorig = R.o; R.t_max = 0.0f; R.neg24 = 0; R.kz = 0; R.sx = R.sy = R.sz = 0.0f;
    int hprim = -1; float hb0 = 0.0f, hb1 = 0.0f, hb2 = 0.0f; bool found = false;
    const float4 rlo = make_float4(S.root_lo[0], S.root_lo[1], S.root_lo[2], 0.0f), rhi = make_float4(S.root_hi[0], S.root_hi[1], S.root_hi[2], 0.0f);
    for (;;) {
        const unsigned long long idle = __ballot(L.mode == T4_IDLE);
        if (!Q.exhausted && (uint32_t)__popcll(idle) >= refill) {
            const uint32_t need = (uint32_t)__popcll(idle);
            if (wq_refill(Q, count, head, lane)) {
                if (W.drain_sig && lane == 0 && atomicAdd(&W.counters[CTR(11)], 1u) + 1u == W.drain_at)
                    __hip_atomic_store(W.drain_sig, W.drain_seq, __ATOMIC_RELAXED, __HIP_MEMORY_SCOPE_SYSTEM);
            }
            const uint32_t avail = Q.chunk_end - Q.chunk_next;
            const uint32_t rank = (uint32_t)__popcll(idle & ((1ull << lane) - 1ull));
            bool hand_back = false; uint32_t q_entry = 0;
            if (COUNT) { occ[5]++; occ[6] += need < avail ? need : avail; }
            if (L.mode == T4_IDLE && rank < avail) {
                float4 a, b;
                q_entry = queue[Q.chunk_next + rank];
                load_queued_ray<false>(W, q_entry, &a, &b, &rid);
                ray_setup<SPHERES>(R, a, b);
                St.sp = St.base; L.cur = 0; found = false; hprim = -1; hb0 = 0.0f; hb1 = 0.0f; hb2 = 0.0f;
                if (ray_is_exceptional(R.o.x, R.o.y, R.o.z, R.inv.x, R.inv.y, R.inv.z)) hand_back = true;
                else if (S.n_nodes == 0 || !slab_test(rlo, rhi, R.o, R.inv, R.t_max)) { W.hit[rid] = make_float4(FTN_INF, 0.0f, 0.0f, 0.0f); W.hit_prim[rid] = -1; }
                else if (S.root_is_leaf) { L.lp = 0; L.mode = T4_LEAF; }
                else L.mode = T4_NODE;
            }
            if (__ballot(hand_back) != 0) wave_push(hand_back, q_entry, W.q_exc_closest, &W.counters[CTR(32)]);
            Q.chunk_next += (need < avail ? need : avail);
        }
        const unsigned long long m_node = __ballot(L.mode == T4_NODE), m_leaf = __ballot(L.mode == T4_LEAF);
        if ((m_node | m_leaf) == 0) { if (Q.exhausted) break; else continue; }
        L.finish = false;
        if (COUNT) occ[0]++;
        if (m_node != 0 && (uint32_t)__popcll(m_leaf) < leaf_batch) {
#pragma unroll
            for (int burst = 0; burst < BURST; burst++) {
                const bool on = L.mode == T4_NODE && !L.finish;
                if (COUNT && on) n_rec++;
                if (COUNT) { const unsigned long long m_on = __ballot(on); if (m_on) { occ[1]++; occ[2] += (unsigned long long)__popcll(m_on); } }
                if (__builtin_expect(__ballot(on && (st_tiny || St.sp > st_soft)) == 0, 1)) { if (on) t4_record_step<false>(S, R, St, L); }
                else if (on) t4_record_step<true>(S, R, St, L);
            }
        } else {
            if (COUNT) { occ[3]++; occ[4] += (unsigned long long)__popcll(m_leaf); }
            if (L.mode == T4_LEAF) {
                const uint32_t prim = L.lp;
                float4 g0 = S.geom[S.geom_stride * prim], g1 = S.geom[S.geom_stride * prim + 1], g2 = S.geom[S.geom_stride * prim + 2];
                pin4(g0); pin4(g1); pin4(g2);
                if (COUNT) n_prim++;
                float t = 0.0f, b0 = 0.0f, b1 = 0.0f, b2 = 0.0f;
                const bool hh = prim_hit<SPHERES>(S, prim, g0, g1, g2, R.o, R.dorig, R.t_max, R.kz, R.sx, R.sy, R.sz, &t, &b0, &b1, &b2);
                if (hh) { found = true; R.t_max = t; hprim = (int)prim; hb0 = b0; hb1 = b1; hb2 = b2; }
                if (__float_as_uint(g0.w) & GF_LEAF_END) t4_pop_next<true>(St, L, R.t_max);
                else L.lp++;
            }
        }
        if (L.finish) {
            W.hit[rid] = make_float4(found ? R.t_max : FTN_INF, hb0, hb1, hb2); W.hit_prim[rid] = hprim;
            L.mode = T4_IDLE;
        }
    }
    if (COUNT) {
        for (int off = 32; off > 0; off >>= 1) { n_rec += __shfl_down(n_rec, off, 64); n_prim += __shfl_down(n_prim, off, 64); }
        if (lane == 0) { if (n_rec) atomicAdd(&stats->quad_records, n_rec); if (n_prim) atomicAdd(&stats->prims_tested, n_prim); for (int k = 0; k < 7; k++) if (occ[k]) atomicAdd(&stats->t4_occ[k], occ[k]); }
    }
    if (blockIdx.x == 0 && threadIdx.x == 0) atomicAdd(&stats->rays_closest, (unsigned long long)count);
}

extern __shared__ uint32_t lds_stack1[];
template <bool CHECK, int POLICY>
__device__ inline void t4_any_step(const DScene& S, const RaySetup& R, T4Stack<uint32_t>& St, T4Lane& L) {
    const float4* rec = reinterpret_cast<const float4*>(reinterpret_cast<const char*>(S.quad) + L.cur);
    const float4 q0 = rec[0], q1 = rec[1], q2 = rec[2], q3 = rec[3], q4 = rec[4], q5 = rec[5], q6 = rec[6], q7 = rec[7];
    float a0, a1, b0, b1, c0, c1, d0, d1;
    const bool ha = slab4(q0, q1, R.o, R.inv, R.t_max, &a0, &a1), hb = slab4(q2, q3, R.o, R.inv, R.t_max, &b0, &b1);
    const bool hc = slab4(q4, q5, R.o, R.inv, R.t_max, &c0, &c1), hd = slab4(q6, q7, R.o, R.inv, R.t_max, &d0, &d1);
    const uint32_t ea = __float_as_uint(q1.z), eb = __float_as_uint(q3.z), ec = __float_as_uint(q5.z), ed = __float_as_uint(q7.z);
    uint32_t next = 0; bool have = ha || hb || hc || hd;
    if (POLICY == 1) {
        const float sa = ha ? fmaxf(a1 - a0, 0.0f) : -1.0f, sb = hb ? fmaxf(b1 - b0, 0.0f) : -1.0f, sc = hc ? fmaxf(c1 - c0, 0.0f) : -1.0f, sd = hd ? fmaxf(d1 - d0, 0.0f) : -1.0f;
        const float best = fmaxf(fmaxf(sa, sb), fmaxf(sc, sd));
        const bool pa = sa == best, pb = !pa && sb == best, pc = !pa && !pb && sc == best, pd = !pa && !pb && !pc;
        next = pa ? ea : (pb ? eb : (pc ? ec : ed));
        if (ha && !pa) St.template push<CHECK>(ea);
        if (hb && !pb) St.template push<CHECK>(eb);
        if (hc && !pc) St.template push<CHECK>(ec);
        if (hd && !pd) St.template push<CHECK>(ed);
    } else {
        next = ha ? ea : (hb ? eb : (hc ? ec : ed));
        if (hd && (ha || hb || hc)) St.template push<CHECK>(ed);
        if (hc && (ha || hb)) St.template push<CHECK>(ec);
        if (hb && ha) St.template push<CHECK>(eb);
    }
    if (!have) {
        if (St.empty()) { L.finish = true; return; }
        next = St.template pop<CHECK>();
    }
    if (next >> 31) { L.lp = next & 0x7fffffffu; L.mode = T4_LEAF; } else L.cur = next;
}

template <bool COUNT, bool SPHERES, int BURST, int POLICY>
__global__ void __launch_bounds__(256) k_wf_trace4_any(DScene S, WfBuffers W, const uint32_t* __restrict__ queue, const uint32_t* count_ptr, uint32_t* head, DevStats* stats,
                                                       uint32_t refill, uint32_t leaf_batch, uint32_t chunk_max, uint32_t lds_entries, uint32_t* __restrict__ spill, uint32_t spill_levels) {
    T4Stack<uint32_t> St;
    St.base = lds_stack1 + threadIdx.x;
    St.lim = St.base + 256u * lds_entries; St.sp = St.base; St.spill = spill; St.spill_levels = spill_levels;
    St.n_lanes = (size_t)gridDim.x * 256u; St.gl = (size_t)blockIdx.x * 256u + threadIdx.x;
    const bool st_tiny = lds_entries < 3u;
    uint32_t* const st_soft = st_tiny ? St.base : St.lim - 3 * 256;
    const uint32_t count = *count_ptr;
    const uint32_t lane = lane_id();
    unsigned long long n_rec = 0, n_prim = 0;
    unsigned long long occ[7] = {0, 0, 0, 0, 0, 0, 0};
    T4Lane L; L.mode = T4_IDLE; L.cur = 0; L.lp = 0; L.finish = false;
    WaveQueue Q; wq_init(Q, count, chunk_max);
    uint32_t rid = 0;
    RaySetup R; R.o = V3(0.0f, 0.0f, 0.0f); R.inv = R.o; R.dorig = R.o; R.t_max = 0.0f; R.neg24 = 0; R.kz = 0; R.sx = R.sy = R.sz = 0.0f;
    bool found = false;
    const float4 rlo = make_float4(S.root_lo[0], S.root_lo[1], S.root_lo[2], 0.0f), rhi = make_float4(S.root_hi[0], S.root_hi[1], S.root_hi[2], 0.0f);
    for (;;) {
        const unsigned long long idle = __ballot(L.mode == T4_IDLE);
        if (!Q.exhausted && (uint32_t)__popcll(idle) >= refill) {
            const uint32_t need = (uint32_t)__popcll(idle);
            (void)wq_refill(Q, count, head, lane);
            const uint32_t avail = Q.chunk_end - Q.chunk_next;
            const uint32_t rank = (uint32_t)__popcll(idle & ((1ull << lane) - 1ull));
            bool hand_back = false; uint32_t q_entry = 0;
            if (COUNT) { occ[5]++; occ[6] += need < avail ? need : avail; }
            if (L.mode == T4_IDLE && rank < avail) {
                float4 a, b;
                q_entry = queue[Q.chunk_next + rank];
                load_queued_ray<true>(W, q_entry, &a, &b, &rid);
                ray_setup<SPHERES>(R, a, b);
                St.sp = St.base; L.cur = 0; found = false;
                if (ray_is_exceptional(R.o.x, R.o.y, R.o.z, R.inv.x, R.inv.y, R.inv.z)) hand_back = true;
                else if (S.n_nodes == 0 || !slab_test(rlo, rhi, R.o, R.inv, R.t_max)) store_occluded(W, rid, false);
                else if (S.root_is_leaf) { L.lp = 0; L.mode = T4_LEAF; }
                else L.mode = T4_NODE;
            }
            if (__ballot(hand_back) != 0) wave_push(hand_back, q_entry, W.q_exc_any, &W.counters[CTR(33)]);
            Q.chunk_next += (need < avail ? need : avail);
        }
        const unsigned long long m_node = __ballot(L.mode == T4_NODE), m_leaf = __ballot(L.mode == T4_LEAF);
        if ((m_node | m_leaf) == 0) { if (Q.exhausted) break; else continue; }
        L.finish = false;
        if (COUNT) occ[0]++;
        if (m_node != 0 && (uint32_t)__popcll(m_leaf) < leaf_batch) {
#pragma unroll
            for (int burst = 0; burst < BURST; burst++) {
                const bool on = L.mode == T4_NODE && !L.finish;
                if (COUNT && on) n_rec++;
                if (COUNT) { const unsigned long long m_on = __ballot(on); if (m_on) { occ[1]++; occ[2] += (unsigned long long)__popcll(m_on); } }
                if (__builtin_expect(__ballot(on && (st_tiny || St.sp > st_soft)) == 0, 1)) { if (on) t4_any_step<false, POLICY>(S, R, St, L); }
                else if (on) t4_any_step<true, POLICY>(S, R, St, L);
            }
        } else {
            if (COUNT) { occ[3]++; occ[4] += (unsigned long long)__popcll(m_leaf); }
            if (L.mode == T4_LEAF) {
                const uint32_t prim = L.lp;
                float4 g0 = S.geom[S.geom_stride * prim], g1 = S.geom[S.geom_stride * prim + 1], g2 = S.geom[S.geom_stride * prim + 2];
                pin4(g0); pin4(g1); pin4(g2);
                if (COUNT) n_prim++;
                float t = 0.0f, b0 = 0.0f, b1 = 0.0f, b2 = 0.0f;
                const bool hh = prim_hit<SPHERES>(S, prim, g0, g1, g2, R.o, R.dorig, R.t_max, R.kz, R.sx, R.sy, R.sz, &t, &b0, &b1, &b2);
                if (hh) { found = true; L.finish = true; }
                else if (__float_as_uint(g0.w) & GF_LEAF_END) {
                    if (St.empty()) L.finish = true;
                    else { const uint32_t next = St.template pop<true>(); if (next >> 31) L.lp = next & 0x7fffffffu; else { L.cur = next; L.mode = T4_NODE; } }
                } else L.lp++;
            }
        }
        if (L.finish) { store_occluded(W, rid, found); L.mode = T4_IDLE; }
    }
    if (COUNT) {
        for (int off = 32; off > 0; off >>= 1) { n_rec += __shfl_down(n_rec, off, 64); n_prim += __shfl_down(n_prim, off, 64); }
        if (lane == 0) {
            if (n_rec) { atomicAdd(&stats->quad_records, n_rec); atomicAdd(&stats->quad_records_any, n_rec); }
            if (n_prim) { atomicAdd(&stats->prims_tested, n_prim); atomicAdd(&stats->prims_any, n_prim); }
            for (int k = 0; k < 7; k++) if (occ[k]) atomicAdd(&stats->t4_occ[7 + k], occ[k]);
        }
    }
    if (blockIdx.x == 0 && threadIdx.x == 0) atomicAdd(&stats->rays_any, (unsigned long long)count);
}

enum : uint32_t { T8_IDLE = 0, T8_NODE = 1, T8_LEAF = 2, T8_LEAF_IN = 3  };
#define T8_XBOX 0x40000000u
__device__ inline bool ray_out_of_range8(float ox, float oy, float oz, float ix, float iy, float iz) {
    const float big_i = 1.152921504606846976e18f , big_o = 1.099511627776e12f ;
    return !(fabsf(ix) <= big_i && fabsf(iy) <= big_i && fabsf(iz) <= big_i && fabsf(ox) <= big_o && fabsf(oy) <= big_o && fabsf(oz) <= big_o);
}
struct T8Axis { float a, bn, bf; uint32_t n03, n47, f03, f47; };
__device__ inline T8Axis t8_axis(float org, uint32_t ebyte, float o, float inv, uint32_t lo03, uint32_t lo47, uint32_t hi03, uint32_t hi47) {
    T8Axis A;
    const float step = __uint_as_float(ebyte << 23);
    A.a = step * inv;
    const float b = (org - o) * inv;
    const float m = (fabsf(b) + 255.0f * fabsf(A.a)) * 9.5367431640625e-07f;
    A.bn = b - m; A.bf = b + m;
    const bool neg = inv < 0.0f;
    A.n03 = neg ? hi03 : lo03; A.n47 = neg ? hi47 : lo47; A.f03 = neg ? lo03 : hi03; A.f47 = neg ? lo47 : hi47;
    return A;
}
#define T8_BYTE(w, k) ((float)(((w) >> (8 * (k))) & 0xffu))
#define T8_CHILD(c, t0v, t1v) \
    { const uint32_t kx_ = (c) & 3; \
      const t4_f2 tx_ = __builtin_elementwise_fma((t4_f2){T8_BYTE((c) < 4 ? X.n03 : X.n47, kx_), T8_BYTE((c) < 4 ? X.f03 : X.f47, kx_)}, (t4_f2){X.a, X.a}, (t4_f2){X.bn, X.bf}); \
      const t4_f2 ty_ = __builtin_elementwise_fma((t4_f2){T8_BYTE((c) < 4 ? Y.n03 : Y.n47, kx_), T8_BYTE((c) < 4 ? Y.f03 : Y.f47, kx_)}, (t4_f2){Y.a, Y.a}, (t4_f2){Y.bn, Y.bf}); \
      const t4_f2 tz_ = __builtin_elementwise_fma((t4_f2){T8_BYTE((c) < 4 ? Z.n03 : Z.n47, kx_), T8_BYTE((c) < 4 ? Z.f03 : Z.f47, kx_)}, (t4_f2){Z.a, Z.a}, (t4_f2){Z.bn, Z.bf}); \
      t0v = fmax_(fmax_(fmax_(0.0f, tx_.x), ty_.x), tz_.x); t1v = fmin_(t_max, fmin_(fmin_(tx_.y, ty_.y), tz_.y) * k2); }

template <bool CHECK, int POLICY>
__device__ __forceinline__ void t8_any_step(const DScene& S, T4Stack<uint32_t>& St, T4Lane& L, V3 o, V3 inv, float t_max) {
    const uint4* rec = reinterpret_cast<const uint4*>(reinterpret_cast<const char*>(S.oct) + L.cur);
    const uint4 r0 = rec[0], r1 = rec[1], r2 = rec[2], r3 = rec[3], r4 = rec[4], r5 = rec[5];
    const float k2 = 1.0f + 4.0f * gamma_n(3);
    const T8Axis X = t8_axis(__uint_as_float(r0.x), r0.w & 0xffu, o.x, inv.x, r3.x, r3.y, r3.z, r3.w);
    const T8Axis Y = t8_axis(__uint_as_float(r0.y), (r0.w >> 8) & 0xffu, o.y, inv.y, r4.x, r4.y, r4.z, r4.w);
    const T8Axis Z = t8_axis(__uint_as_float(r0.z), (r0.w >> 16) & 0xffu, o.z, inv.z, r5.x, r5.y, r5.z, r5.w);
    float a0, a1, b0, b1, c0, c1, d0, d1, e0, e1, f0, f1, g0, g1, h0, h1;
    T8_CHILD(0, a0, a1) T8_CHILD(1, b0, b1) T8_CHILD(2, c0, c1) T8_CHILD(3, d0, d1) T8_CHILD(4, e0, e1) T8_CHILD(5, f0, f1) T8_CHILD(6, g0, g1) T8_CHILD(7, h0, h1)
    const uint32_t la = r1.x, lb = r1.y, lc = r1.z, ld = r1.w, le = r2.x, lf = r2.y, lg = r2.z, lh = r2.w;
    const bool ha = !(a0 > a1) && la != T4_NONE, hb = !(b0 > b1) && lb != T4_NONE, hc = !(c0 > c1) && lc != T4_NONE, hd = !(d0 > d1) && ld != T4_NONE;
    const bool he = !(e0 > e1) && le != T4_NONE, hf = !(f0 > f1) && lf != T4_NONE, hg = !(g0 > g1) && lg != T4_NONE, hh = !(h0 > h1) && lh != T4_NONE;
    uint32_t next = T4_NONE;
    if (POLICY == 1) {
        const float sa = ha ? a1 - a0 : -1.0f, sb = hb ? b1 - b0 : -1.0f, sc = hc ? c1 - c0 : -1.0f, sd = hd ? d1 - d0 : -1.0f;
        const float se = he ? e1 - e0 : -1.0f, sf = hf ? f1 - f0 : -1.0f, sg = hg ? g1 - g0 : -1.0f, sh = hh ? h1 - h0 : -1.0f;
        const float best = fmaxf(fmaxf(fmaxf(sa, sb), fmaxf(sc, sd)), fmaxf(fmaxf(se, sf), fmaxf(sg, sh)));
        bool taken = !(best >= 0.0f);
#define T8_PICK(hx, sx, lx) { const bool me_ = hx && !taken && sx == best; if (me_) { next = lx; taken = true; } else if (hx) St.template push<CHECK>(lx); }
        T8_PICK(ha, sa, la) T8_PICK(hb, sb, lb) T8_PICK(hc, sc, lc) T8_PICK(hd, sd, ld) T8_PICK(he, se, le) T8_PICK(hf, sf, lf) T8_PICK(hg, sg, lg) T8_PICK(hh, sh, lh)
#undef T8_PICK
    } else {
        bool taken = false;
#define T8_PICK(hx, lx) { if (hx) { if (!taken) { next = lx; taken = true; } else St.template push<CHECK>(lx); } }
        T8_PICK(ha, la) T8_PICK(hb, lb) T8_PICK(hc, lc) T8_PICK(hd, ld) T8_PICK(he, le) T8_PICK(hf, lf) T8_PICK(hg, lg) T8_PICK(hh, lh)
#undef T8_PICK
    }
    if (next == T4_NONE) {
        if (St.empty()) { L.finish = true; return; }
        next = St.template pop<CHECK>();
    }
    if (next >> 31) { L.lp = next & 0x7fffffffu; L.mode = T8_LEAF; } else L.cur = next;
}

template <bool COUNT, int BURST, int POLICY>
__global__ void __launch_bounds__(256) k_wf_trace8_any(DScene S, WfBuffers W, const uint32_t* __restrict__ queue, const uint32_t* count_ptr, uint32_t* head, DevStats* stats,
                                                       uint32_t refill, uint32_t leaf_batch, uint32_t chunk_max, uint32_t lds_entries, uint32_t* __restrict__ spill, uint32_t spill_levels) {
    T4Stack<uint32_t> St;
    St.base = lds_stack1 + threadIdx.x;
    St.lim = St.base + 256u * lds_entries; St.sp = St.base; St.spill = spill; St.spill_levels = spill_levels;
    St.n_lanes = (size_t)gridDim.x * 256u; St.gl = (size_t)blockIdx.x * 256u + threadIdx.x;
    const bool st_tiny = lds_entries < 7u;
    uint32_t* const st_soft = st_tiny ? St.base : St.lim - 7 * 256;
    const uint32_t count = *count_ptr;
    const uint32_t lane = lane_id();
    unsigned long long n_rec = 0, n_prim = 0;
    unsigned long long occ[7] = {0, 0, 0, 0, 0, 0, 0};
    T4Lane L; L.mode = T8_IDLE; L.cur = 0; L.lp = 0; L.finish = false;
    WaveQueue Q; wq_init(Q, count, chunk_max);
    uint32_t rid = 0;
    RaySetup R; R.o = V3(0.0f, 0.0f, 0.0f); R.inv = R.o; R.dorig = R.o; R.t_max = 0.0f; R.neg24 = 0; R.kz = 0; R.sx = R.sy = R.sz = 0.0f;
    bool found = false;
    const float4 rlo = make_float4(S.root_lo[0], S.root_lo[1], S.root_lo[2], 0.0f), rhi = make_float4(S.root_hi[0], S.root_hi[1], S.root_hi[2], 0.0f);
    for (;;) {
        const unsigned long long idle = __ballot(L.mode == T8_IDLE);
        if (!Q.exhausted && (uint32_t)__popcll(idle) >= refill) {
            const uint32_t need = (uint32_t)__popcll(idle);
            (void)wq_refill(Q, count, head, lane);
            const uint32_t avail = Q.chunk_end - Q.chunk_next;
            const uint32_t rank = (uint32_t)__popcll(idle & ((1ull << lane) - 1ull));
            bool hand_back = false; uint32_t q_entry = 0;
            if (COUNT) { occ[5]++; occ[6] += need < avail ? need : avail; }
            if (L.mode == T8_IDLE && rank < avail) {
                float4 a, b;
                q_entry = queue[Q.chunk_next + rank];
                load_queued_ray<true>(W, q_entry, &a, &b, &rid);
                ray_setup<false>(R, a, b);
                St.sp = St.base; L.cur = 0; found = false;
                if (ray_is_exceptional(R.o.x, R.o.y, R.o.z, R.inv.x, R.inv.y, R.inv.z) || ray_out_of_range8(R.o.x, R.o.y, R.o.z, R.inv.x, R.inv.y, R.inv.z)) hand_back = true;
                else if (!slab_test(rlo, rhi, R.o, R.inv, R.t_max)) store_occluded(W, rid, false);
                else L.mode = T8_NODE;
            }
            if (__ballot(hand_back) != 0) wave_push(hand_back, q_entry, W.q_exc_any, &W.counters[CTR(33)]);
            Q.chunk_next += (need < avail ? need : avail);
        }
        const unsigned long long m_node = __ballot(L.mode == T8_NODE), m_leaf = __ballot(L.mode >= T8_LEAF);
        if ((m_node | m_leaf) == 0) { if (Q.exhausted) break; else continue; }
        L.finish = false;
        if (COUNT) occ[0]++;
        if (m_node != 0 && (uint32_t)__popcll(m_leaf) < leaf_batch) {
#pragma unroll
            for (int burst = 0; burst < BURST; burst++) {
                const bool on = L.mode == T8_NODE && !L.finish;
                if (COUNT && on) n_rec++;
                if (COUNT) { const unsigned long long m_on = __ballot(on); if (m_on) { occ[1]++; occ[2] += (unsigned long long)__popcll(m_on); } }
                if (__builtin_expect(__ballot(on && (st_tiny || St.sp > st_soft)) == 0, 1)) { if (on) t8_any_step<false, POLICY>(S, St, L, R.o, R.inv, R.t_max); }
                else if (on) t8_any_step<true, POLICY>(S, St, L, R.o, R.inv, R.t_max);
            }
        } else {
            if (COUNT) { occ[3]++; occ[4] += (unsigned long long)__popcll(m_leaf); }
            if (L.mode >= T8_LEAF) {
                const bool entering = L.mode == T8_LEAF;
                uint32_t prim = L.lp & 0x3fffffffu;
                float4 x0 = make_float4(0.0f, 0.0f, 0.0f, 0.0f), x1 = x0;
                const bool explicit_box = entering && (L.lp & T8_XBOX);
                if (explicit_box) { x0 = S.oct_xbox[2 * (size_t)prim]; x1 = S.oct_xbox[2 * (size_t)prim + 1]; prim = __float_as_uint(x0.w); }
                float4 g0 = S.geom[S.geom_stride * prim], g1 = S.geom[S.geom_stride * prim + 1], g2 = S.geom[S.geom_stride * prim + 2];
                pin4(g0); pin4(g1); pin4(g2);
                bool pass = true;
                if (entering) {
                    if (!explicit_box) {
                        x0 = make_float4(fmin_(fmin_(g0.x, g1.x), g2.x), fmin_(fmin_(g0.y, g1.y), g2.y), fmin_(fmin_(g0.z, g1.z), g2.z), 0.0f);
                        x1 = make_float4(fmax_(fmax_(g0.x, g1.x), g2.x), fmax_(fmax_(g0.y, g1.y), g2.y), fmax_(fmax_(g0.z, g1.z), g2.z), 0.0f);
                    }
                    pass = slab_test(x0, x1, R.o, R.inv, R.t_max);
                }
                bool hh = false;
                if (pass) {
                    if (COUNT) n_prim++;
                    float t = 0.0f, b0 = 0.0f, b1 = 0.0f, b2 = 0.0f;
                    hh = prim_hit<false>(S, prim, g0, g1, g2, R.o, R.dorig, R.t_max, R.kz, R.sx, R.sy, R.sz, &t, &b0, &b1, &b2);
                }
                if (hh) { found = true; L.finish = true; }
                else if (!pass || (__float_as_uint(g0.w) & GF_LEAF_END)) {
                    if (St.empty()) L.finish = true;
                    else { const uint32_t next = St.template pop<true>(); if (next >> 31) { L.lp = next & 0x7fffffffu; L.mode = T8_LEAF; } else { L.cur = next; L.mode = T8_NODE; } }
                } else { L.lp = prim + 1u; L.mode = T8_LEAF_IN; }
            }
        }
        if (L.finish) { store_occluded(W, rid, found); L.mode = T8_IDLE; }
    }
    if (COUNT) {
        for (int off = 32; off > 0; off >>= 1) { n_rec += __shfl_down(n_rec, off, 64); n_prim += __shfl_down(n_prim, off, 64); }
        if (lane == 0) {
            if (n_rec) { atomicAdd(&stats->quad_records, n_rec); atomicAdd(&stats->quad_records_any, n_rec); }
            if (n_prim) { atomicAdd(&stats->prims_tested, n_prim); atomicAdd(&stats->prims_any, n_prim); }
            for (int k = 0; k < 7; k++) if (occ[k]) atomicAdd(&stats->t4_occ[7 + k], occ[k]);
        }
    }
    if (blockIdx.x == 0 && threadIdx.x == 0) atomicAdd(&stats->rays_any, (unsigned long long)count);
}

Trace4Plan trace4_plan(const DScene& S, int n_cu, uint32_t knob_entries_closest, uint32_t knob_entries_any, uint32_t knob_wg_closest, uint32_t knob_wg_any, uint32_t knob_wg_oct, uint32_t knob_entries_oct) {
    Trace4Plan p; memset(&p, 0, sizeof(p));
    const uint32_t bound = S.quad_stack_bound ? S.quad_stack_bound : 1u;
    const uint32_t wg_c = knob_wg_closest ? knob_wg_closest : 5u, wg_a = knob_wg_any ? knob_wg_any : 4u;
    const uint32_t budget_c = ((158u * 1024u) / wg_c) & ~1023u, budget_a = ((158u * 1024u) / wg_a) & ~1023u;
    uint32_t ec = knob_entries_closest ? knob_entries_closest : budget_c / (256u * 8u);
    uint32_t ea = knob_entries_any ? knob_entries_any : budget_a / (256u * 4u);
    p.entries_closest = ec < bound ? ec : bound; p.entries_any = ea < bound ? ea : bound;
    if (p.entries_closest == 0) p.entries_closest = 1;
    if (p.entries_any == 0) p.entries_any = 1;
    p.spill_closest = bound - p.entries_closest; p.spill_any = bound - p.entries_any;
    p.lds_closest = (size_t)p.entries_closest * 256u * 8u; p.lds_any = (size_t)p.entries_any * 256u * 4u;
    auto per_cu = [](size_t lds, uint32_t wg) { return (unsigned)std::max<size_t>(1, std::min<size_t>(wg, (size_t)(158 * 1024) / std::max<size_t>(lds, 1))); };
    p.grid_closest = (unsigned)n_cu * per_cu(p.lds_closest, wg_c); p.grid_any = (unsigned)n_cu * per_cu(p.lds_any, wg_a);
    if (S.oct && S.n_octs) {
        const uint32_t wg_8 = knob_wg_oct ? knob_wg_oct : 5u, budget_8 = ((158u * 1024u) / wg_8) & ~1023u, bound8 = S.oct_stack_bound ? S.oct_stack_bound : 1u;
        const uint32_t e8 = knob_entries_oct ? knob_entries_oct : budget_8 / (256u * 4u);
        p.entries_oct = e8 < bound8 ? e8 : bound8;
        p.spill_oct = bound8 - p.entries_oct;
        p.lds_oct = (size_t)p.entries_oct * 256u * 4u;
        p.grid_oct = (unsigned)n_cu * per_cu(p.lds_oct, wg_8);
        p.oct_ok = true;
    }
    return p;
}

void launch_trace4(int kind, bool count, bool spheres, unsigned grid, size_t lds, uint32_t lds_entries, void* spill, hipStream_t stream, const DScene& S, const WfBuffers& W,
                   const uint32_t* queue, const uint32_t* count_ptr, uint32_t* head, DevStats* stats, uint32_t refill, uint32_t leaf_batch, uint32_t chunk, uint32_t burst, uint32_t any_policy, uint32_t spill_levels) {
    const bool any = kind != T4K_CLOSEST;
#define FTN_T4(K, SPILL_T, ...) hipLaunchKernelGGL((K<__VA_ARGS__>), dim3(grid), dim3(256), lds, stream, S, W, queue, count_ptr, head, stats, refill, leaf_batch, chunk, lds_entries, (SPILL_T)spill, spill_levels)
    if (kind == T4K_ANY_OCT) {
#define FTN_T8(C, B) do { if (any_policy == 0) FTN_T4(k_wf_trace8_any, uint32_t*, C, B, 0); else FTN_T4(k_wf_trace8_any, uint32_t*, C, B, 1); } while (0)
        if (count) FTN_T8(true, 2);
        else if (burst <= 1) FTN_T8(false, 1); else if (burst == 2) FTN_T8(false, 2); else FTN_T8(false, 3);
#undef FTN_T8
    } else if (any) {
#define FTN_T4A(C, Sp, B) do { if (any_policy == 0) FTN_T4(k_wf_trace4_any, uint32_t*, C, Sp, B, 0); else FTN_T4(k_wf_trace4_any, uint32_t*, C, Sp, B, 1); } while (0)
        if (count) { if (spheres) FTN_T4A(true, true, 2); else FTN_T4A(true, false, 2); }
        else if (spheres) { if (burst <= 2) FTN_T4A(false, true, 2); else FTN_T4A(false, true, 4); }
        else { if (burst <= 1) FTN_T4A(false, false, 1); else if (burst == 2) FTN_T4A(false, false, 2); else if (burst == 3) FTN_T4A(false, false, 3); else FTN_T4A(false, false, 4); }
#undef FTN_T4A
    } else {
        if (count) { if (spheres) FTN_T4(k_wf_trace4, uint2*, true, true, 2); else FTN_T4(k_wf_trace4, uint2*, true, false, 2); }
        else if (spheres) { if (burst <= 2) FTN_T4(k_wf_trace4, uint2*, false, true, 2); else FTN_T4(k_wf_trace4, uint2*, false, true, 4); }
        else { if (burst <= 1) FTN_T4(k_wf_trace4, uint2*, false, false, 1); else if (burst == 2) FTN_T4(k_wf_trace4, uint2*, false, false, 2); else if (burst == 3) FTN_T4(k_wf_trace4, uint2*, false, false, 3); else FTN_T4(k_wf_trace4, uint2*, false, false, 4); }
    }
#undef FTN_T4
}

}
```

fountain_amd/csrc/ftn_wavefront.hip:

```cpp
#include "ftn_wf_common.h"
#include "ftn_texture.h"
#include <string>
#include <cstdlib>
#include <hipcub/hipcub.hpp>

namespace ftn {

__global__ void __launch_bounds__(256) k_wf_generate(RenderParams P, WfBuffers W, int write_state) {
    const uint32_t i = blockIdx.x * 256u + threadIdx.x;
    if (i >= W.n_paths) return;
    const uint32_t slot = i / W.samples, s = i % W.samples;
    const DTile tile = P.tiles[slot >> 8];
    const int px = tile.x0 + (int)(slot & 15u), py = tile.y0 + (int)((slot >> 4) & 15u);
    if (px < tile.x1 && py < tile.y1) {
        Rng rng; rng.seed(indexed_key(P.seed, px, py, W.first_sample + s));
        V2 j = rng.next2();
        V2 p_film((float)px + j.x, (float)py + j.y);
        V2 p_lens = rng.next2();
        float time_u = rng.next();
        DRay ray = camera_ray(P.C, p_film, p_lens, time_u);
        W.ray[2 * (size_t)(i)] = make_float4(ray.o.x, ray.o.y, ray.o.z, 0.0f);
        W.ray[2 * (size_t)(i) + 1] = make_float4(ray.d.x, ray.d.y, ray.d.z, ray.t_max);
        if (write_state) {
            W.beta[i] = make_float4(1.0f, 1.0f, 1.0f, __uint_as_float(PS_ALIVE));
// ... 829 lines not shown
            }
            float* f = reinterpret_cast<float*>((in_tile ? P.accB : P.accC) + ((size_t)(y - F.crop[1]) * width + (size_t)(x - F.crop[0])));
            atomicAdd(f + 0, contrib.r); atomicAdd(f + 1, contrib.g); atomicAdd(f + 2, contrib.b); atomicAdd(f + 3, 1.0f);
            (*bc_writes)++;
        }
    if (touched != 1) (*spill)++;
}
#define WF_ACC_CHUNK 8u
__global__ void __launch_bounds__(256) k_wf_accumulate(RenderParams P, WfBuffers W) {
    __shared__ float4 s_rad[256 * WF_ACC_CHUNK];
    const uint32_t slot = blockIdx.x * 256u + threadIdx.x;
    uint32_t spill = 0, bc = 0, cam = 0; int err = 0;
    bool valid = false, in_crop = false; int px = 0, py = 0; size_t ai = 0;
    FilmCtxW F; float4 acc = make_float4(0.0f, 0.0f, 0.0f, 0.0f);
    if (slot < W.n_slots) {
        const DTile tile = P.tiles[slot >> 8];
        px = tile.x0 + (int)(slot & 15u); py = tile.y0 + (int)((slot >> 4) & 15u);
        if (px < tile.x1 && py < tile.y1) {
            valid = true;
            for (int i = 0; i < 4; i++) F.crop[i] = P.crop[i];
            F.sb[0] = tile.x0; F.sb[1] = tile.y0; F.sb[2] = tile.x1; F.sb[3] = tile.y1; F.radius[0] = P.radius[0]; F.radius[1] = P.radius[1];
            int p0x = f2i_sat(ceilf((float)tile.x0 - 0.5f - P.radius[0])), p0y = f2i_sat(ceilf((float)tile.y0 - 0.5f - P.radius[1]));
            int p1x = f2i_sat(ceilf((float)tile.x1 - 0.5f + P.radius[0] + 1.0f)), p1y = f2i_sat(ceilf((float)tile.y1 - 0.5f - P.radius[1] + 1.0f));
            F.tpb[0] = max(p0x, P.crop[0]); F.tpb[1] = max(p0y, P.crop[1]); F.tpb[2] = min(p1x, P.crop[2]); F.tpb[3] = min(p1y, P.crop[3]);
            in_crop = px >= P.crop[0] && px < P.crop[2] && py >= P.crop[1] && py < P.crop[3];
            ai = in_crop ? ((size_t)(py - P.crop[1]) * (size_t)(P.crop[2] - P.crop[0]) + (size_t)(px - P.crop[0])) : 0;
            if (in_crop) acc = P.accA[ai];
        }
    }
    const size_t block_first = (size_t)blockIdx.x * 256u * W.samples;
    for (uint32_t s0 = 0; s0 < W.samples; s0 += WF_ACC_CHUNK) {
        const uint32_t n = W.samples - s0 < WF_ACC_CHUNK ? W.samples - s0 : WF_ACC_CHUNK;
        for (uint32_t e = threadIdx.x; e < 256u * n; e += 256u) {
            const uint32_t sl = e / n, k = e - sl * n;
            const size_t p = block_first + (size_t)sl * W.samples + s0 + k;
            if (p < W.n_paths) s_rad[sl * WF_ACC_CHUNK + k] = W.rad[p];
        }
        __syncthreads();
        if (valid) {
            for (uint32_t k = 0; k < n; k++) {
                const float4 l = s_rad[threadIdx.x * WF_ACC_CHUNK + k];
                Rgb L(l.x, l.y, l.z);
                if (L.has_nans()) err = FTN_ERR_NAN_RADIANCE;
                Rng crng; crng.seed(indexed_key(P.seed, px, py, W.first_sample + s0 + k));
                const V2 j = crng.next2();
                wf_film_add(P, F, V2((float)px + j.x, (float)py + j.y), L, in_crop ? px : (-2147483647), py, &acc, &spill, &bc);
                cam++;
            }
        }
        __syncthreads();
    }
    if (valid && in_crop) P.accA[ai] = acc;
    (void)cam;
    if (spill) atomicAdd(&P.stats->spill_samples, (unsigned long long)spill);
    if (bc) atomicAdd(&P.stats->bc_writes, (unsigned long long)bc);
    if (err) atomicCAS(&P.stats->error, 0, err);
}

template <bool TEX>
__global__ void __launch_bounds__(256) k_wf_serial_advance(RenderParams P, WfBuffers W, int out_q, int init) {
    const uint32_t t = blockIdx.x * 256u + threadIdx.x;
    bool push = false;
    uint32_t spill = 0, bc = 0, cam = 0; int err = 0;
    if (t < W.n_paths) {
        const DTile tile = P.tiles[t];
        const uint32_t tw = (uint32_t)(tile.x1 - tile.x0), npix = tw * (uint32_t)(tile.y1 - tile.y0);
        Rng rng; uint2 cur = make_uint2(0u, 0u); bool start = false;
        if (init) { rng.seed(tile.tile_id); start = npix > 0u && P.spp > 0u; W.ser_retired[t] = 0; }
        else if (W.ser_retired[t]) {
            W.ser_retired[t] = 0;
            { const ulonglong2 a = W.rng01[t], b = W.rng23[t]; rng.s0 = a.x; rng.s1 = a.y; rng.s2 = b.x; rng.s3 = b.y; }
            cur = W.ser_cursor[t];
            const float4 l = W.rad[t]; const float2 pf = W.ser_pfilm[t];
            Rgb L(l.x, l.y, l.z);
            if (L.has_nans()) err = FTN_ERR_NAN_RADIANCE;
            FilmCtxW F;
            for (int i = 0; i < 4; i++) F.crop[i] = P.crop[i];
            F.sb[0] = tile.x0; F.sb[1] = tile.y0; F.sb[2] = tile.x1; F.sb[3] = tile.y1; F.radius[0] = P.radius[0]; F.radius[1] = P.radius[1];
            const int p0x = f2i_sat(ceilf((float)tile.x0 - 0.5f - P.radius[0])), p0y = f2i_sat(ceilf((float)tile.y0 - 0.5f - P.radius[1]));
            const int p1x = f2i_sat(ceilf((float)tile.x1 - 0.5f + P.radius[0] + 1.0f)), p1y = f2i_sat(ceilf((float)tile.y1 - 0.5f - P.radius[1] + 1.0f));
            F.tpb[0] = max(p0x, P.crop[0]); F.tpb[1] = max(p0y, P.crop[1]); F.tpb[2] = min(p1x, P.crop[2]); F.tpb[3] = min(p1y, P.crop[3]);
            float4 none = make_float4(0.0f, 0.0f, 0.0f, 0.0f);
            wf_film_add(P, F, V2(pf.x, pf.y), L, WF_OWN_SERIAL, 0, &none, &spill, &bc);
            cam = 1;
            if (++cur.y == P.spp) { cur.y = 0; cur.x++; }
            start = cur.x < npix;
        }
        if (start) {
            const int px = tile.x0 + (int)(cur.x % tw), py = tile.y0 + (int)(cur.x / tw);
            const V2 j = rng.next2();
            const V2 p_film((float)px + j.x, (float)py + j.y);
            const V2 p_lens = rng.next2();
            const float time_u = rng.next();
            const DRay ray = camera_ray(P.C, p_film, p_lens, time_u);
            W.ray[2 * (size_t)t] = make_float4(ray.o.x, ray.o.y, ray.o.z, 0.0f);
            W.ray[2 * (size_t)t + 1] = make_float4(ray.d.x, ray.d.y, ray.d.z, ray.t_max);
            W.beta[t] = make_float4(1.0f, 1.0f, 1.0f, __uint_as_float(PS_ALIVE));
            W.rad[t] = make_float4(0.0f, 0.0f, 0.0f, 0.0f);
            W.rng01[t] = make_ulonglong2(rng.s0, rng.s1); W.rng23[t] = make_ulonglong2(rng.s2, rng.s3);
            W.ser_cursor[t] = cur; W.ser_pfilm[t] = make_float2(p_film.x, p_film.y);
            if (TEX) {
                const DRayDiff rd = camera_ray_diff(P.C, p_film, p_lens, ray, 1.0f / sqrtf((float)P.spp));
                W.dfd[t] = make_float4(rd.rxo.x, rd.rxo.y, rd.rxo.z, rd.rxd.x); W.dfd[(size_t)W.n_paths + t] = make_float4(rd.ryo.x, rd.ryo.y, rd.ryo.z, rd.rxd.y);
                W.dfd[2 * (size_t)W.n_paths + t] = make_float4(rd.ryd.x, rd.ryd.y, rd.ryd.z, rd.rxd.z);
            }
            push = true;
        }
    }
    {
        const bool pred[2] = {push, push};
        const uint32_t val[2] = {t | (P.max_depth == 0 ? WF_Q_DEPTH : 0u), t};
        uint32_t* const qs[2] = {W.q_active[out_q], W.q_closest};
        uint32_t* const cs[2] = {&W.counters[CTR(out_q == 0 ? 0 : 1)], &W.counters[CTR(2)]};
        block_push<2>(pred, val, qs, cs);
    }
    if (cam) atomicAdd(&P.stats->camera_samples, (unsigned long long)cam);
    if (spill) atomicAdd(&P.stats->spill_samples, (unsigned long long)spill);
    if (bc) atomicAdd(&P.stats->bc_writes, (unsigned long long)bc);
    if (err) atomicCAS(&P.stats->error, 0, err);
}

static thread_local std::string g_wf_err;
const char* wavefront_error() { return g_wf_err.c_str(); }

__device__ inline uint32_t spread3(uint32_t v) {
    v &= 0x3ffu; v = (v | (v << 16)) & 0x030000ffu; v = (v | (v << 8)) & 0x0300f00fu; v = (v | (v << 4)) & 0x030c30c3u; v = (v | (v << 2)) & 0x09249249u; return v;
}
template <bool ANY>
__global__ void __launch_bounds__(256) k_wf_ray_keys(DScene S, WfBuffers W, const uint32_t* __restrict__ queue, uint32_t count, uint32_t* __restrict__ keys, uint32_t bits) {
    const uint32_t i = blockIdx.x * 256u + threadIdx.x;
    if (i >= count) return;
    float4 a, b; uint32_t slot;
    load_queued_ray<ANY>(W, queue[i], &a, &b, &slot);
    const float ex = S.root_hi[0] - S.root_lo[0], ey = S.root_hi[1] - S.root_lo[1], ez = S.root_hi[2] - S.root_lo[2];
    const float sc = (float)(1u << bits);
    const float fx = fminf(fmaxf((a.x - S.root_lo[0]) / ex, 0.0f), 0.999f) * sc, fy = fminf(fmaxf((a.y - S.root_lo[1]) / ey, 0.0f), 0.999f) * sc, fz = fminf(fmaxf((a.z - S.root_lo[2]) / ez, 0.0f), 0.999f) * sc;
    const uint32_t m = spread3((uint32_t)fx) | (spread3((uint32_t)fy) << 1) | (spread3((uint32_t)fz) << 2);
    const uint32_t oct = (b.x < 0.0f ? 1u : 0u) | (b.y < 0.0f ? 2u : 0u) | (b.z < 0.0f ? 4u : 0u);
    keys[i] = (m << 3) | oct;
}

struct WavefrontState {
    void* sort_tmp = nullptr; size_t sort_tmp_bytes = 0;
    size_t cap_paths = 0;
    void* mem[40]; int n_mem = 0;
    WfBuffers W;
    float4* br = nullptr; float4* pd = nullptr;
    hipEvent_t ev[64]; int n_ev = 0;
    hipStream_t side = nullptr; hipEvent_t ev_ready = nullptr, ev_side = nullptr;
    uint32_t* drain_sig = nullptr; uint32_t drain_seq = 0;
    uint32_t* host_counters = nullptr;
    int n_cu = 256;
    void* dl_mem[8] = {nullptr, nullptr, nullptr, nullptr, nullptr, nullptr, nullptr, nullptr}; size_t dl_paths = 0; uint32_t dl_levels = 0, dl_slots = 0; bool dl_tex = false;
    Trace4Plan t4; bool t4_on = false, t8_on = false;
    void* ser_mem[4] = {nullptr, nullptr, nullptr, nullptr}; size_t ser_paths = 0; bool ser_tex = false; uint32_t* ser_host = nullptr;
    void* t4_spill_c = nullptr; void* t4_spill_a = nullptr; size_t t4_spill_c_bytes = 0, t4_spill_a_bytes = 0;
};
#define WF_TRY(expr) do { hipError_t e_ = (expr); if (e_ != hipSuccess) { g_wf_err = std::string(#expr ": ") + hipGetErrorString(e_); return e_ == hipErrorOutOfMemory ? FTN_ERR_OUT_OF_MEMORY : FTN_ERR_NO_DEVICE; } } while (0)

static void wf_free(WavefrontState* st) { for (int i = 0; i < st->n_mem; i++) (void)hipFree(st->mem[i]); st->n_mem = 0; st->cap_paths = 0; }
void wavefront_destroy(WavefrontState* st) {
    if (!st) return;
    wf_free(st);
    if (st->sort_tmp) (void)hipFree(st->sort_tmp);
    for (int i = 0; i < st->n_ev; i++) (void)hipEventDestroy(st->ev[i]);
    if (st->ev_ready) (void)hipEventDestroy(st->ev_ready);
    if (st->ev_side) (void)hipEventDestroy(st->ev_side);
    if (st->side) (void)hipStreamDestroy(st->side);
    if (st->drain_sig) (void)hipFree(st->drain_sig);
    for (void* m : st->dl_mem) if (m) (void)hipFree(m);
    for (void* m : st->ser_mem) if (m) (void)hipFree(m);
    if (st->t4_spill_c) (void)hipFree(st->t4_spill_c);
    if (st->t4_spill_a) (void)hipFree(st->t4_spill_a);
    if (st->host_counters) (void)hipHostFree(st->host_counters);
    if (st->ser_host) (void)hipHostFree(st->ser_host);
    delete st;
}
template <class T> static int wf_alloc(WavefrontState* st, T** p, size_t n) {
    WF_TRY(hipMalloc((void**)p, n * sizeof(T)));
    st->mem[st->n_mem++] = (void*)*p;
    return FTN_OK;
}
static int wf_reserve(WavefrontState* st, size_t n) {
    if (n <= st->cap_paths) return FTN_OK;
    wf_free(st);
    WfBuffers& W = st->W; int rc;
    if ((rc = wf_alloc(st, &W.ray, 4 * n)) || (rc = wf_alloc(st, &W.hit, 2 * n)) || (rc = wf_alloc(st, &W.hit_prim, 2 * n)) ||
        (rc = wf_alloc(st, &W.sh, 2 * n)) || (rc = wf_alloc(st, &W.occluded, 2 * n)) || (rc = wf_alloc(st, &W.beta, n)) || (rc = wf_alloc(st, &W.rad, n)) ||
        (rc = wf_alloc(st, &W.rng01, n)) || (rc = wf_alloc(st, &W.rng23, n)) || (rc = wf_alloc(st, &W.pend0, n)) || (rc = wf_alloc(st, &W.pend1, n)) || (rc = wf_alloc(st, &W.pend2, n)) ||
        (rc = wf_alloc(st, &W.q_active[0], n)) || (rc = wf_alloc(st, &W.q_active[1], n)) || (rc = wf_alloc(st, &W.q_closest, 2 * n)) || (rc = wf_alloc(st, &W.q_shadow, 2 * n)) || (rc = wf_alloc(st, &W.q_sorted, 8 * n)) || (rc = wf_alloc(st, &W.cls, 8 * 32)) ||
        (rc = wf_alloc(st, &W.q_exc_closest, 2 * n)) || (rc = wf_alloc(st, &W.q_exc_any, 2 * n)) || (rc = wf_alloc(st, &W.counters, 64 * 32)) || (rc = wf_alloc(st, &st->br, 2 * n)) || (rc = wf_alloc(st, &st->pd, 4 * n))) return rc;
    st->cap_paths = n;
    return FTN_OK;
}

#include <unordered_map>
static thread_local std::unordered_map<std::string, std::pair<bool, uint32_t>> g_knobs;
static void knobs_begin() { g_knobs.clear(); }
static uint32_t knob(const char* name, uint32_t def) {
    auto it = g_knobs.find(name);
    if (it == g_knobs.end()) { const char* v = getenv(name); it = g_knobs.emplace(name, std::make_pair(v != nullptr, v ? (uint32_t)atoi(v) : 0u)).first; }
    return it->second.first ? it->second.second : def;
}

static int sort_ray_queue(WavefrontState* st, const RenderParams& P, const WfBuffers& W, bool any, uint32_t* queue, uint32_t cnt, uint32_t* out,
                          uint32_t* k_in, uint32_t* k_out, uint32_t bits, hipStream_t stream, const uint32_t** sorted_q) {
    *sorted_q = queue;
    if (cnt < knob("FTN_WF_SORT_MIN", 16384u)) return FTN_OK;
    if (any) hipLaunchKernelGGL(k_wf_ray_keys<true>, dim3((cnt + 255) / 256), dim3(256), 0, stream, P.S, W, queue, cnt, k_in, bits);
    else hipLaunchKernelGGL(k_wf_ray_keys<false>, dim3((cnt + 255) / 256), dim3(256), 0, stream, P.S, W, queue, cnt, k_in, bits);
    const int end_bit = (int)(3 * bits + 3);
    size_t need = 0;
    hipcub::DoubleBuffer<uint32_t> keys(k_in, k_out), vals(queue, out);
    WF_TRY(hipcub::DeviceRadixSort::SortPairs(nullptr, need, keys, vals, (int)cnt, 0, end_bit, stream));
    if (need > st->sort_tmp_bytes) { if (st->sort_tmp) (void)hipFree(st->sort_tmp); st->sort_tmp = nullptr; st->sort_tmp_bytes = 0; WF_TRY(hipMalloc(&st->sort_tmp, need)); st->sort_tmp_bytes = need; }
    WF_TRY(hipcub::DeviceRadixSort::SortPairs(st->sort_tmp, need, keys, vals, (int)cnt, 0, end_bit, stream));
    *sorted_q = vals.Current();
    return FTN_OK;
}


#ifdef FTN_DRAIN_PROBE
static uint32_t g_probe_bounce = 0;
#endif
static int trace4_prepare(WavefrontState* st, const DScene& S) {
    st->t4_on = S.quad != nullptr && knob("FTN_TRACE4", 1) != 0;
    if (!st->t4_on) return FTN_OK;
    st->t4 = trace4_plan(S, st->n_cu, knob("FTN_T4_ENTRIES", 0), knob("FTN_T4_ENTRIES_ANY", 0), knob("FTN_T4_WG", 0), knob("FTN_T4_WG_ANY", 0), knob("FTN_T8_WG", 0), knob("FTN_T8_ENTRIES", 0));
    const size_t need_c = (size_t)st->t4.grid_closest * 256u * st->t4.spill_closest * sizeof(uint2);
    st->t8_on = st->t4.oct_ok && S.n_spheres == 0 && knob("FTN_T8", 1) != 0;
    const size_t need_a8 = st->t8_on ? (size_t)st->t4.grid_oct * 256u * st->t4.spill_oct * sizeof(uint32_t) : 0;
    const size_t need_a = std::max<size_t>(need_a8, (size_t)st->t4.grid_any * 256u * st->t4.spill_any * sizeof(uint32_t));
    if (need_c > st->t4_spill_c_bytes) { if (st->t4_spill_c) (void)hipFree(st->t4_spill_c); st->t4_spill_c = nullptr; st->t4_spill_c_bytes = 0; WF_TRY(hipMalloc(&st->t4_spill_c, need_c)); st->t4_spill_c_bytes = need_c; }
    if (need_a > st->t4_spill_a_bytes) { if (st->t4_spill_a) (void)hipFree(st->t4_spill_a); st->t4_spill_a = nullptr; st->t4_spill_a_bytes = 0; WF_TRY(hipMalloc(&st->t4_spill_a, need_a)); st->t4_spill_a_bytes = need_a; }
    return FTN_OK;
}

static void launch_trace(WavefrontState* st, bool any, int count, bool spheres, unsigned grid, size_t lds, hipStream_t stream, const RenderParams& P, const WfBuffers& W,
                         const uint32_t* queue, const uint32_t* count_ptr, uint32_t* head, uint32_t max_rays, bool camera_rays = false) {
    if (st->t4_on && count != 1) {
        const Trace4Plan& T = st->t4;
        const bool oct = any && st->t8_on;
        const unsigned g = std::min<unsigned>(oct ? T.grid_oct : (any ? T.grid_any : T.grid_closest), std::max<unsigned>(1u, (max_rays + 255u) / 256u));
        uint32_t chunk4 = knob("FTN_TRACE_CHUNK", 128);
        while (chunk4 > 64u && (uint64_t)chunk4 * g * 4u * 4u > (uint64_t)max_rays) chunk4 >>= 1;
        if (oct) launch_trace4(T4K_ANY_OCT, count == 2, false, g, T.lds_oct, T.entries_oct, st->t4_spill_a, stream, P.S, W, queue, count_ptr, head, P.stats,
                               camera_rays ? knob("FTN_T8_REFILL1", 16) : knob("FTN_T8_REFILL", 24), camera_rays ? knob("FTN_T8_LEAF_BATCH1", 16) : knob("FTN_T8_LEAF_BATCH", 16), chunk4, knob("FTN_T8_BURST", 2), knob("FTN_T8_POLICY", 1), T.spill_oct);
        else launch_trace4(any ? T4K_ANY : T4K_CLOSEST, count == 2, spheres, g, any ? T.lds_any : T.lds_closest, any ? T.entries_any : T.entries_closest, any ? st->t4_spill_a : st->t4_spill_c, stream, P.S, W,
                      queue, count_ptr, head, P.stats,
                      any ? knob("FTN_T4_ANY_REFILL", 32) : (camera_rays ? knob("FTN_T4_REFILL0", 64) : knob("FTN_T4_REFILL", 32)),
                      any ? knob("FTN_T4_ANY_LEAF_BATCH", 16) : (camera_rays ? knob("FTN_T4_LEAF_BATCH0", 2) : knob("FTN_T4_LEAF_BATCH", 16)), chunk4,
                      any ? knob("FTN_T4_ANY_BURST", 4) : (camera_rays ? knob("FTN_T4_BURST0", 3) : knob("FTN_T4_BURST", 2)), knob("FTN_T4_ANY_POLICY", 1), any ? T.spill_any : T.spill_closest);
        const unsigned ge = std::min<unsigned>(grid, (unsigned)st->n_cu);
        uint32_t* ecount = &W.counters[CTR(any ? 33 : 32)]; uint32_t* ehead = &W.counters[CTR(any ? 48 : 40)];
        DevStats* none = nullptr;
#define FTN_TRE(A, Sp) hipLaunchKernelGGL((k_wf_trace<A, false, Sp, 8>), dim3(ge), dim3(256), lds, stream, P.S, W, any ? W.q_exc_any : W.q_exc_closest, ecount, ehead, none, 24u, 2u, 64u, 8u)
        if (any) { if (spheres) FTN_TRE(true, true); else FTN_TRE(true, false); } else { if (spheres) FTN_TRE(false, true); else FTN_TRE(false, false); }
#undef FTN_TRE
        return;
    }
    const bool count_b = count != 0;
    const uint32_t refill = knob("FTN_TRACE_REFILL", 24), leaf_batch = knob("FTN_TRACE_LEAF_BATCH", 2), chunk_knob = knob("FTN_TRACE_CHUNK", 128), node_burst = knob("FTN_TRACE_BURST", 8);
    uint32_t chunk = chunk_knob;
    const uint32_t waves = grid * 4u;
    while (chunk > 64u && (uint64_t)chunk * waves * 4u > (uint64_t)max_rays) chunk >>= 1;
    if (any && !count_b && knob("FTN_TRACE_ANY2", 1) && P.S.fat) {
        const uint32_t refill2 = knob("FTN_ANY2_REFILL", 16), leaf_batch2 = knob("FTN_ANY2_LEAF_BATCH", leaf_batch);
        uint32_t policy2 = knob("FTN_ANY2_POLICY", 2);
#ifdef FTN_DRAIN_PROBE
        policy2 |= g_probe_bounce << 8;
#endif
        if (spheres) hipLaunchKernelGGL((k_wf_trace_any2<true>), dim3(grid), dim3(256), lds, stream, P.S, W, queue, count_ptr, head, P.stats, refill2, leaf_batch2, chunk, policy2);
        else hipLaunchKernelGGL((k_wf_trace_any2<false>), dim3(grid), dim3(256), lds, stream, P.S, W, queue, count_ptr, head, P.stats, refill2, leaf_batch2, chunk, policy2);
        return;
    }
    lds += knob("FTN_TRACE_LDS_PAD", 0);
#define FTN_TR(A, C, Sp, B) hipLaunchKernelGGL((k_wf_trace<A, C, Sp, B>), dim3(grid), dim3(256), lds, stream, P.S, W, queue, count_ptr, head, P.stats, refill, leaf_batch, chunk, node_burst)
    const bool fixed = node_burst == 8 && !count_b && !knob("FTN_TRACE_NO_UNROLL", 0);
    if (fixed) { if (any) { if (spheres) FTN_TR(true, false, true, 8); else FTN_TR(true, false, false, 8); } else { if (spheres) FTN_TR(false, false, true, 8); else FTN_TR(false, false, false, 8); } }
    else if (any) { if (count_b) { if (spheres) FTN_TR(true, true, true, 0); else FTN_TR(true, true, false, 0); } else { if (spheres) FTN_TR(true, false, true, 0); else FTN_TR(true, false, false, 0); } }
    else { if (count_b) { if (spheres) FTN_TR(false, true, true, 0); else FTN_TR(false, true, false, 0); } else { if (spheres) FTN_TR(false, false, true, 0); else FTN_TR(false, false, false, 0); } }
#undef FTN_TR
}

static void wf_free_dl(WavefrontState* st) { for (void*& m : st->dl_mem) { if (m) (void)hipFree(m); m = nullptr; } st->dl_paths = 0; st->dl_levels = 0; st->dl_slots = 0; st->dl_tex = false; }
static int wf_reserve_dl(WavefrontState* st, size_t n, uint32_t levels, uint32_t slots, bool tex) {
    if (n <= st->dl_paths && levels <= st->dl_levels && slots <= st->dl_slots && (!tex || st->dl_tex)) return FTN_OK;
    wf_free_dl(st);
    const size_t sl = std::max<uint32_t>(slots, 2u);
    WF_TRY(hipMalloc(&st->dl_mem[0], (size_t)levels * n * sizeof(float4)));
    WF_TRY(hipMalloc(&st->dl_mem[1], (size_t)levels * n * sizeof(float4)));
    WF_TRY(hipMalloc(&st->dl_mem[2], (size_t)slots * n * sizeof(float4)));
    WF_TRY(hipMalloc(&st->dl_mem[3], 2 * (size_t)slots * n * sizeof(float4)));
    WF_TRY(hipMalloc(&st->dl_mem[4], sl * n));
    WF_TRY(hipMalloc(&st->dl_mem[5], sl * n * sizeof(uint32_t)));
    WF_TRY(hipMalloc(&st->dl_mem[6], sl * n * sizeof(uint32_t)));
    if (tex) WF_TRY(hipMalloc(&st->dl_mem[7], 3 * n * sizeof(float4)));
    st->dl_paths = n; st->dl_levels = levels; st->dl_slots = slots; st->dl_tex = tex;
    return FTN_OK;
}

static int wf_state_init(WavefrontState** state) {
    if (*state) return FTN_OK;
    *state = new WavefrontState();
    for (int i = 0; i < 64; i++) { WF_TRY(hipEventCreate(&(*state)->ev[i])); (*state)->n_ev = i + 1; }
    {
        int least = 0, greatest = 0;
        WF_TRY(hipDeviceGetStreamPriorityRange(&least, &greatest));
        WF_TRY(hipStreamCreateWithPriority(&(*state)->side, hipStreamNonBlocking, knob("FTN_WF_SIDE_PRIO", 1) ? least : 0));
    }
    WF_TRY(hipEventCreateWithFlags(&(*state)->ev_ready, hipEventDisableTiming));
    WF_TRY(hipEventCreateWithFlags(&(*state)->ev_side, hipEventDisableTiming));
    {
        int dev = 0, can = 0;
        WF_TRY(hipGetDevice(&dev));
        if (hipDeviceGetAttribute(&can, hipDeviceAttributeCanUseStreamWaitValue, dev) == hipSuccess && can) {
            if (hipExtMallocWithFlags((void**)&(*state)->drain_sig, 8, hipMallocSignalMemory) != hipSuccess) { (void)hipGetLastError(); (*state)->drain_sig = nullptr; }
            else WF_TRY(hipMemset((*state)->drain_sig, 0, 8));
        }
    }
    WF_TRY(hipHostMalloc((void**)&(*state)->host_counters, 16 * 32 * sizeof(uint32_t)));
    hipDeviceProp_t prop; int dev = 0; WF_TRY(hipGetDevice(&dev)); WF_TRY(hipGetDeviceProperties(&prop, dev));
    (*state)->n_cu = prop.multiProcessorCount > 0 ? prop.multiProcessorCount : 256;
    return FTN_OK;
}

__global__ void __launch_bounds__(256) k_batch_setup(const float* __restrict__ rays8, uint32_t n, float4* __restrict__ ray, uint32_t* __restrict__ queue) {
    const uint32_t i = blockIdx.x * 256u + threadIdx.x;
    if (i >= n) return;
    const float* r = rays8 + 8 * (size_t)i;
    ray[2 * (size_t)i] = make_float4(r[0], r[1], r[2], r[7]);
    ray[2 * (size_t)i + 1] = make_float4(r[3], r[4], r[5], r[6]);
    queue[i] = i;
}
__global__ void __launch_bounds__(256) k_batch_finish(DScene S, const float* __restrict__ rays8, uint32_t n, const float4* __restrict__ hit, const int* __restrict__ hit_prim,
                                                      float* t_hit, int* prim, float* bary, float* out24) {
    const uint32_t i = blockIdx.x * 256u + threadIdx.x;
    if (i >= n) return;
    const float4 h4 = hit[i]; const int hp = hit_prim[i];
    if (t_hit) t_hit[i] = hp >= 0 ? h4.x : FTN_INF;
    if (prim) prim[i] = hp;
    if (bary) { bary[3 * (size_t)i] = hp >= 0 ? h4.y : 0.0f; bary[3 * (size_t)i + 1] = hp >= 0 ? h4.z : 0.0f; bary[3 * (size_t)i + 2] = hp >= 0 ? h4.w : 0.0f; }
    if (out24) {
        float* o = out24 + 24 * (size_t)i;
        if (hp < 0) { for (int k = 0; k < 24; k++) o[k] = 0.0f; o[23] = -1.0f; }
        else {
            const float* r = rays8 + 8 * (size_t)i;
            DRay ray0; ray0.o = V3(r[0], r[1], r[2]); ray0.d = V3(r[3], r[4], r[5]); ray0.t_max = r[6]; ray0.time = r[7];
            DHit h; h.t = h4.x; h.b0 = h4.y; h.b1 = h4.z; h.b2 = h4.w; h.prim = hp;
            DSI si; make_interaction(S, h, ray0, &si);
            o[0] = si.hit.p.x; o[1] = si.hit.p.y; o[2] = si.hit.p.z; o[3] = si.hit.p_err.x; o[4] = si.hit.p_err.y; o[5] = si.hit.p_err.z;
            o[6] = si.hit.n.x; o[7] = si.hit.n.y; o[8] = si.hit.n.z; o[9] = 0.0f; o[10] = 0.0f;
            o[11] = si.wo.x; o[12] = si.wo.y; o[13] = si.wo.z; o[14] = si.s_dpdu.x; o[15] = si.s_dpdu.y; o[16] = si.s_dpdu.z;
            o[17] = 0.0f; o[18] = 0.0f; o[19] = 0.0f; o[20] = si.shading_n.x; o[21] = si.shading_n.y; o[22] = si.shading_n.z; o[23] = h.t;
        }
    }
}
int wavefront_trace_batch(WavefrontState** state, const DScene& S, uint32_t stack_entries, const float* d_rays8, size_t n_rays, int mode, bool count,
                          float* t_hit, int* prim, float* bary, unsigned char* occluded, float* out24, DevStats* stats, hipStream_t stream) {
    if (n_rays == 0) return FTN_OK;
    if (n_rays >= (1ull << 31)) { g_wf_err = "too many rays in one batch"; return FTN_ERR_INVALID_ARGUMENT; }
    knobs_begin();
    int rc = wf_state_init(state); if (rc) return rc;
    WavefrontState* st = *state;
    if ((rc = trace4_prepare(st, S))) return rc;
    const uint32_t n = (uint32_t)n_rays;
    const bool any = mode == 1;
    float4 *ray = nullptr, *hit = nullptr; int* hit_prim = nullptr; uint32_t *queue = nullptr, *scratch = nullptr, *counters = nullptr, *q_exc = nullptr;
    auto cleanup = [&]() { (void)hipFree(ray); (void)hipFree(hit); (void)hipFree(hit_prim); (void)hipFree(queue); (void)hipFree(scratch); (void)hipFree(counters); (void)hipFree(q_exc); };
#define WFB_TRY(expr) do { hipError_t e_ = (expr); if (e_ != hipSuccess) { g_wf_err = std::string(#expr ": ") + hipGetErrorString(e_); cleanup(); return e_ == hipErrorOutOfMemory ? FTN_ERR_OUT_OF_MEMORY : FTN_ERR_NO_DEVICE; } } while (0)
    WFB_TRY(hipMalloc((void**)&ray, (size_t)n * 32)); WFB_TRY(hipMalloc((void**)&queue, (size_t)n * 4)); WFB_TRY(hipMalloc((void**)&scratch, (size_t)n * 12));
    WFB_TRY(hipMalloc((void**)&counters, 64 * 32 * 4)); WFB_TRY(hipMemsetAsync(counters, 0, 64 * 32 * 4, stream));
    WFB_TRY(hipMalloc((void**)&q_exc, (size_t)n * 4));
    if (!any) { WFB_TRY(hipMalloc((void**)&hit, (size_t)n * 16)); WFB_TRY(hipMalloc((void**)&hit_prim, (size_t)n * 4)); }
    hipLaunchKernelGGL(k_batch_setup, dim3((n + 255) / 256), dim3(256), 0, stream, d_rays8, n, ray, queue);
    WFB_TRY(hipMemcpyAsync(&counters[CTR(any ? 3 : 2)], &n, 4, hipMemcpyHostToDevice, stream));
    WfBuffers W; memset(&W, 0, sizeof(W));
    W.n_paths = n; W.ray = ray; W.sh = ray; W.hit = hit; W.hit_prim = hit_prim; W.occluded = occluded; W.counters = counters; W.q_exc_closest = q_exc; W.q_exc_any = q_exc;
    RenderParams P; memset(&P, 0, sizeof(P)); P.S = S; P.stats = stats;
    const uint32_t* q = queue;
    if (knob("FTN_WF_SORT", 0)) { rc = sort_ray_queue(st, P, W, any, queue, n, scratch, scratch + n, scratch + 2 * (size_t)n, 7, stream, &q); if (rc) { cleanup(); return rc; } }
    const size_t lds = (size_t)stack_entries * 256 * sizeof(uint32_t);
    const unsigned per_cu = (unsigned)std::max<size_t>(1, std::min<size_t>(8, (size_t)(160 * 1024) / std::max<size_t>(lds, 1)));
    const unsigned grid = std::min<unsigned>((unsigned)st->n_cu * per_cu, (n + 255) / 256);
    launch_trace(st, any, count ? 1 : 0, S.n_spheres != 0, grid, lds, stream, P, W, q, &counters[CTR(any ? 3 : 2)], &counters[CTR(any ? 24 : 16)], n);
    if (!any) hipLaunchKernelGGL(k_batch_finish, dim3((n + 255) / 256), dim3(256), 0, stream, S, d_rays8, n, hit, hit_prim, t_hit, prim, bary, out24);
    WFB_TRY(hipStreamSynchronize(stream));
    WFB_TRY(hipGetLastError());
#undef WFB_TRY
    cleanup();
    return FTN_OK;
}

static int wavefront_render_serial(WavefrontState* st, const RenderParams& P, uint32_t n_tiles, bool count, bool count_production, hipStream_t stream, WavefrontTimes* times) {
    int rc = wf_reserve(st, (size_t)std::max<uint32_t>(n_tiles, 256u));
    if (rc) { wf_free(st); return rc; }
    const bool tex = P.S.n_textures != 0;
    if (n_tiles > st->ser_paths || (tex && !st->ser_tex)) {
        for (void*& m : st->ser_mem) { if (m) (void)hipFree(m); m = nullptr; }
        st->ser_paths = 0;
        WF_TRY(hipMalloc(&st->ser_mem[0], (size_t)n_tiles * sizeof(uint2)));
        WF_TRY(hipMalloc(&st->ser_mem[1], (size_t)n_tiles * sizeof(float2)));
        WF_TRY(hipMalloc(&st->ser_mem[2], (size_t)n_tiles));
        if (tex) WF_TRY(hipMalloc(&st->ser_mem[3], 3 * (size_t)n_tiles * sizeof(float4)));
        st->ser_paths = n_tiles; st->ser_tex = tex;
// ... 286 lines not shown
```

fountain_amd/csrc/ftn_wf_common.h:

```cpp
#ifndef FTN_WF_COMMON_H
#define FTN_WF_COMMON_H
#include "ftn_wavefront.h"

namespace ftn {

enum : uint32_t { PS_BOUNCE_MASK = 0xffffu, PS_SPECULAR = 1u << 16, PS_ALIVE = 1u << 17, PS_DIRECT = 1u << 18, PS_SHADOW = 1u << 19, PS_MIS = 1u << 20, PS_DELTA = 1u << 21, PS_MIS_ANY = 1u << 22  };
#define PS_DRAWS_SHIFT 23
#define WF_MIS_BIT 0x80000000u

struct WfBuffers {
    uint32_t n_paths;
    uint32_t n_slots;
    uint32_t samples;
    uint32_t first_sample;
    float4 *ray;
    float4* hit;
    int* hit_prim;
    float4 *sh;
    unsigned char* occluded;
    float4 *beta;
    float4 *rad;
    float4* br;
    ulonglong2 *rng01, *rng23;
    float4 *pend0, *pend1, *pend2;
    float4* pd;
    uint32_t pd_md, pd_occ;
    uint32_t *q_active[2], *q_closest, *q_shadow;
    uint32_t* q_sorted;
    uint32_t* cls;
    uint32_t seg_cap;
    uint32_t* counters;
    uint32_t valid_per_sample;
    uint32_t* drain_sig; uint32_t drain_seq, drain_at;
    uint32_t *q_exc_closest, *q_exc_any;
    float4 *dlA, *dlB, *whT;
    float4* dfd;
    uint32_t serial;
    uint2* ser_cursor;
    float2* ser_pfilm;
    unsigned char* ser_retired;
    uint32_t rng_replay;
    uint32_t gen_blocks;
    uint32_t mis_any;
};

#define WF_Q_FIN 0x80000000u
#define WF_Q_DEPTH 0x40000000u
#define WF_Q_ID_MASK 0x0fffffffu

#define CTR(i) ((i) * 32)
__device__ inline uint32_t lane_id() { return threadIdx.x & 63u; }
__device__ inline void wave_push(bool pred, uint32_t value, uint32_t* queue, uint32_t* counter) {
    const unsigned long long m = __ballot(pred);
    if (m == 0) return;
    const int leader = __ffsll((long long)m) - 1;
    uint32_t base = 0;
    if ((int)lane_id() == leader) base = atomicAdd(counter, (uint32_t)__popcll(m));
    base = __shfl(base, leader, 64);
    if (pred) queue[base + (uint32_t)__popcll(m & ((1ull << lane_id()) - 1ull))] = value;
}

template <int NQ>
__device__ inline void block_push(const bool (&pred)[NQ], const uint32_t (&value)[NQ], uint32_t* const (&queue)[NQ], uint32_t* const (&counter)[NQ]) {
    __shared__ uint32_t s_cnt[NQ][4];
    __shared__ uint32_t s_base[NQ];
    const uint32_t wave = threadIdx.x >> 6, lane = lane_id();
    unsigned long long m[NQ];
#pragma unroll
    for (int q = 0; q < NQ; q++) { m[q] = __ballot(pred[q]); if (lane == 0) s_cnt[q][wave] = (uint32_t)__popcll(m[q]); }
    __syncthreads();
    if (threadIdx.x < NQ) {
        const uint32_t q = threadIdx.x;
        const uint32_t tot = s_cnt[q][0] + s_cnt[q][1] + s_cnt[q][2] + s_cnt[q][3];
        s_base[q] = tot ? atomicAdd(counter[q], tot) : 0u;
    }
    __syncthreads();
#pragma unroll
    for (int q = 0; q < NQ; q++) {
        if (pred[q]) {
            uint32_t off = s_base[q];
            for (uint32_t w = 0; w < wave; w++) off += s_cnt[q][w];
            if (queue[q]) queue[q][off + (uint32_t)__popcll(m[q] & ((1ull << lane) - 1ull))] = value[q];
        }
    }
    __syncthreads();
}

__device__ inline void store_occluded(const WfBuffers& W, uint32_t slot, bool occ) {
    if (W.pd_occ) {
        if (!occ) return;
        const bool mis = slot >= W.n_paths;
        const uint32_t p = mis ? slot - W.n_paths : slot;
        ((unsigned char*)(W.pd + 4 * (size_t)p + 3))[12 + (mis ? 1 : 0)] = occ ? 1 : 0;
    } else W.occluded[slot] = occ ? 1 : 0;
}

template <bool ANY>
__device__ inline void load_queued_ray(const WfBuffers& W, uint32_t rid, float4* a, float4* b, uint32_t* slot) {
    const uint32_t pid = rid & ~WF_MIS_BIT;
    if (ANY && !(rid & WF_MIS_BIT)) { *a = W.sh[2 * (size_t)pid]; *b = W.sh[2 * (size_t)pid + 1]; *slot = pid; }
    else { const uint32_t r = (rid & WF_MIS_BIT) ? pid + W.n_paths : pid; *a = W.ray[2 * (size_t)r]; *b = W.ray[2 * (size_t)r + 1]; *slot = r; }
}

template <bool SPHERES>
__device__ inline bool prim_hit(const DScene& S, uint32_t prim, float4 g0, float4 g1, float4 g2, V3 o, V3 dorig, float t_max, int kz, float sx, float sy, float sz,
                                float* t_out, float* b0o, float* b1o, float* b2o) {
    const uint32_t fl = __float_as_uint(g0.w);
    float t = 0.0f, b0 = 0.0f, b1 = 0.0f, b2 = 0.0f; bool hh = false;
    if (SPHERES && (fl & GF_KIND_SPHERE)) {
        DRay r; r.o = o; r.d = dorig; r.t_max = t_max; r.time = 0.0f;
        hh = sphere_intersect<false>(S.spheres[__float_as_uint(g1.w)], r, &t, nullptr);
    } else {
        const bool k0 = kz == 0, k1 = kz == 1;
#define FTN_PERM(v) V3(k0 ? (v).y : (k1 ? (v).z : (v).x), k0 ? (v).z : (k1 ? (v).x : (v).y), k0 ? (v).x : (k1 ? (v).y : (v).z))
        const V3 op = FTN_PERM(o);
        V3 p0t = FTN_PERM(g0), p1t = FTN_PERM(g1), p2t = FTN_PERM(g2);
#undef FTN_PERM
        p0t = V3(p0t.x - op.x, p0t.y - op.y, p0t.z - op.z);
        p1t = V3(p1t.x - op.x, p1t.y - op.y, p1t.z - op.z);
        p2t = V3(p2t.x - op.x, p2t.y - op.y, p2t.z - op.z);
        p0t.x += sx * p0t.z; p0t.y += sy * p0t.z;
        p1t.x += sx * p1t.z; p1t.y += sy * p1t.z;
        p2t.x += sx * p2t.z; p2t.y += sy * p2t.z;
        float e0 = p1t.x * p2t.y - p1t.y * p2t.x;
        float e1 = p2t.x * p0t.y - p2t.y * p0t.x;
        float e2 = p0t.x * p1t.y - p0t.y * p1t.x;
        if (e0 == 0.0f || e1 == 0.0f || e2 == 0.0f) {
            e0 = (float)((double)p1t.x * (double)p2t.y - (double)p1t.y * (double)p2t.x);
            e1 = (float)((double)p2t.x * (double)p0t.y - (double)p2t.y * (double)p0t.x);
            e2 = (float)((double)p0t.x * (double)p1t.y - (double)p0t.y * (double)p1t.x);
        }
        const float det = e0 + e1 + e2;
        if (!(sign_pos(e0) != sign_pos(e1) || sign_pos(e1) != sign_pos(e2)) && det != 0.0f) {
            p0t.z *= sz; p1t.z *= sz; p2t.z *= sz;
            const float t_scaled = e0 * p0t.z + e1 * p1t.z + e2 * p2t.z;
            if (!((det < 0.0f && (t_scaled >= 0.0f || t_scaled < t_max * det)) || (det > 0.0f && (t_scaled <= 0.0f || t_scaled > t_max * det)))) {
                const float inv_det = 1.0f / det;
                b0 = e0 * inv_det; b1 = e1 * inv_det; b2 = e2 * inv_det; t = t_scaled * inv_det;
                const float max_zt = fmax_(fmax_(fabsf(p0t.z), fabsf(p1t.z)), fabsf(p2t.z));
                const float delta_z = gamma_n(3) * max_zt;
                const float max_xt = fmax_(fmax_(fabsf(p0t.x), fabsf(p1t.x)), fabsf(p2t.x));
                const float max_yt = fmax_(fmax_(fabsf(p0t.y), fabsf(p1t.y)), fabsf(p2t.y));
                const float delta_x = gamma_n(5) * (max_xt + max_zt), delta_y = gamma_n(5) * (max_yt + max_zt);
                const float delta_e = 2.0f * (gamma_n(2) * max_xt * max_yt + delta_y * max_xt + delta_x * max_yt);
                const float max_e = fmax_(fmax_(fabsf(e0), fabsf(e1)), fabsf(e2));
                const float delta_t = 3.0f * (gamma_n(3) * max_e * max_zt + delta_e * max_zt + delta_z * max_e) * fabsf(inv_det);
                hh = !(t <= delta_t);
                if (hh && (fl & GF_HAS_UVS) && tri_uv_degenerate_reject(S, (int)prim, V3(g0.x, g0.y, g0.z), V3(g1.x, g1.y, g1.z), V3(g2.x, g2.y, g2.z))) hh = false;
            }
        }
    }
    *t_out = t; *b0o = b0; *b1o = b1; *b2o = b2;
    return hh;
}


struct Trace4Plan {
    uint32_t entries_closest, entries_any;
    uint32_t spill_closest, spill_any;
    size_t lds_closest, lds_any;
    unsigned grid_closest, grid_any;
    bool oct_ok; uint32_t entries_oct, spill_oct; size_t lds_oct; unsigned grid_oct;
};
enum : int { T4K_CLOSEST = 0, T4K_ANY = 1, T4K_ANY_OCT = 2 };
Trace4Plan trace4_plan(const DScene& S, int n_cu, uint32_t knob_entries_closest, uint32_t knob_entries_any, uint32_t knob_wg_closest, uint32_t knob_wg_any, uint32_t knob_wg_oct, uint32_t knob_entries_oct);
void launch_trace4(int kind, bool count, bool spheres, unsigned grid, size_t lds, uint32_t lds_entries, void* spill, hipStream_t stream, const DScene& S, const WfBuffers& W,
                   const uint32_t* queue, const uint32_t* count_ptr, uint32_t* head, DevStats* stats, uint32_t refill, uint32_t leaf_batch, uint32_t chunk, uint32_t burst, uint32_t any_policy, uint32_t spill_levels);

}
#endif
```

Measured before the change: 3088.

## Add quantized 64-byte four-box BVH records for closest-hit traversal

```diff
diff --git a/fountain_amd/csrc/ftn_device.h b/fountain_amd/csrc/ftn_device.h
--- a/fountain_amd/csrc/ftn_device.h
+++ b/fountain_amd/csrc/ftn_device.h
@@ -60,6 +60,8 @@
     uint32_t n_quads, quad_stack_bound;
     const uint4* oct; const float4* oct_xbox;
     uint32_t n_octs, oct_stack_bound;
+    const uint4* quad64; const float4* quad64_xbox;
+    uint32_t n_quad64, quad64_stack_bound;
     const unsigned char* prim_class;
 };
 
diff --git a/fountain_amd/csrc/ftn_host.cpp b/fountain_amd/csrc/ftn_host.cpp
--- a/fountain_amd/csrc/ftn_host.cpp
+++ b/fountain_amd/csrc/ftn_host.cpp
@@ -510,6 +510,93 @@
     }
     if (out->xbox.size() / 2 >= (1u << 30) || nodes.size() >= (1u << 30)) return;
     out->n_records = (uint32_t)recs.size(); out->stack_bound = bound[0]; out->ok = true;
+}
+
+struct Quad64Bvh { std::vector<uint32_t> rec; std::vector<float4> xbox; uint32_t n_records = 0, stack_bound = 0; bool ok = false; };
+static void build_quad64s(const QuadBvh& qb, const std::vector<float4>& geom, Quad64Bvh* out) {
+    out->rec.clear(); out->xbox.clear(); out->n_records = 0; out->stack_bound = 0; out->ok = false;
+    if (!qb.ok || qb.n_records == 0) return;
+    const size_t n = qb.n_records;
+    auto slot = [&](size_t q, int s) { return &qb.rec[(size_t)32 * q + 8 * s]; };
+    auto meta = [&](const float* S) { return ftn_det::f2u(S[7]); };
+    auto leaf_is_implicit = [&](const float* S) {
+        const uint32_t p = ftn_det::f2u(S[6]) & 0x7fffffffu;
+        if (geom.empty() || (size_t)FTN_GS * p + 2 >= geom.size()) return false;
+        const float4 g0 = geom[(size_t)FTN_GS * p], g1 = geom[(size_t)FTN_GS * p + 1], g2 = geom[(size_t)FTN_GS * p + 2];
+        const uint32_t fl = ftn_det::f2u(g0.w);
+        if ((fl & GF_KIND_SPHERE) || !(fl & GF_LEAF_END)) return false;
+        const float lo[3] = {std::min(std::min(g0.x, g1.x), g2.x), std::min(std::min(g0.y, g1.y), g2.y), std::min(std::min(g0.z, g1.z), g2.z)};
+        const float hi[3] = {std::max(std::max(g0.x, g1.x), g2.x), std::max(std::max(g0.y, g1.y), g2.y), std::max(std::max(g0.z, g1.z), g2.z)};
+        for (int a = 0; a < 3; a++) if (ftn_det::f2u(lo[a]) != ftn_det::f2u(S[2 * a]) || ftn_det::f2u(hi[a]) != ftn_det::f2u(S[2 * a + 1])) return false;
+        return true;
+    };
+    std::vector<uint8_t> xmask(n, 0);
+    parallel_for(n, [&](size_t q0, size_t q1) {
+        for (size_t q = q0; q < q1; q++) {
+            uint8_t m = 0;
+            for (int s = 0; s < 4; s++) { const float* S = slot(q, s); if ((meta(S) >> 24) == 1u && !leaf_is_implicit(S)) m |= (uint8_t)(1u << s); }
+            xmask[q] = m;
+        }
+    });
+    std::vector<uint32_t> xbase(n, 0);
+    { uint32_t run = 0; for (size_t q = 0; q < n; q++) { xbase[q] = run; run += (uint32_t)__builtin_popcount(xmask[q]); } out->xbox.assign(2 * (size_t)run, make_float4(0.0f, 0.0f, 0.0f, 0.0f)); }
+    if (out->xbox.size() / 2 >= (1u << 30)) return;
+    out->rec.assign((size_t)16 * n, 0u);
+    std::atomic<bool> bad{false};
+    parallel_for(n, [&](size_t q0, size_t q1) {
+    for (size_t q = q0; q < q1; q++) {
+        uint32_t* W = &out->rec[(size_t)16 * q];
+        bool used[4];
+        for (int s = 0; s < 4; s++) used[s] = !((meta(slot(q, s)) >> 25) & 1u);
+        for (int a = 0; a < 3; a++) {
+            float org = FTN_INF, top = -FTN_INF;
+            for (int s = 0; s < 4; s++) if (used[s]) { org = std::min(org, slot(q, s)[2 * a]); top = std::max(top, slot(q, s)[2 * a + 1]); }
+            if (!(std::fabs(org) < FTN_INF && std::fabs(top) < FTN_INF)) { bad = true; break; }
+            const double ext = (double)top - (double)org;
+            int e = ext > 0.0 ? (int)ceil(log2(ext / 255.0)) : -126;
+            if (e < -126) e = -126;
+            for (;; e++) {
+                const double st = ldexp(1.0, e);
+                if (ceil(((double)top - (double)org) / st) <= 254.0 || e >= 126) break;
+            }
+            const double stp = ldexp(1.0, e), o = (double)org;
+            memcpy(&W[a], &org, 4);
+            W[3] |= (uint32_t)(e + 127) << (8 * a);
+            for (int s = 0; s < 4; s++) {
+                uint32_t ql = 255u, qh = 0u;
+                if (used[s]) {
+                    const double lo = slot(q, s)[2 * a], hi = slot(q, s)[2 * a + 1];
+                    double l = floor((lo - o) / stp), h = ceil((hi - o) / stp);
+                    while (l > 0.0 && o + l * stp > lo) l -= 1.0;
+                    while (o + h * stp < hi) h += 1.0;
+                    if (l < 0.0 || h > 255.0 || o + l * stp > lo || o + h * stp < hi) { bad = true; break; }
+                    ql = (uint32_t)l; qh = (uint32_t)h;
+                }
+                W[4 + 2 * a] |= ql << (8 * s); W[5 + 2 * a] |= qh << (8 * s);
+            }
+        }
+        uint32_t xi = xbase[q];
+        for (int s = 0; s < 4; s++) {
+            const float* S = slot(q, s);
+            const uint32_t link = ftn_det::f2u(S[6]), m = meta(S);
+            uint32_t l = 0xffffffffu;
+            if (!used[s]) l = 0xffffffffu;
+            else if (!((m >> 24) & 1u)) l = link >> 1;
+            else if (link & 0x40000000u) bad = true;
+            else if (!((xmask[q] >> s) & 1u)) l = link;
+            else {
+                l = 0xc0000000u | xi;
+                out->xbox[2 * (size_t)xi] = make_float4(S[0], S[2], S[4], ftn_det::u2f(link & 0x7fffffffu));
+                out->xbox[2 * (size_t)xi + 1] = make_float4(S[1], S[3], S[5], 0.0f);
+                xi++;
+            }
+            W[10 + s] = l;
+        }
+        W[14] = meta(slot(q, 0)) & 0x00ffffffu;
+    }
+    });
+    if (bad) { out->rec.clear(); out->xbox.clear(); return; }
+    out->n_records = (uint32_t)n; out->stack_bound = qb.stack_bound; out->ok = true;
 }
 
 static int bvh_default_threads() {
@@ -701,7 +788,7 @@
     int device = 0;
     HostScene host;
     DScene d; uint32_t stack_entries = 1;
-    DevBuf<float4> nodes, geom, fat, srec, quad, oct_xbox; DevBuf<uint4> prim_info, oct; DevBuf<float> N, UV, T; DevBuf<DSphere> spheres; DevBuf<ftn_material> materials; DevBuf<DLight> lights;
+    DevBuf<float4> nodes, geom, fat, srec, quad, oct_xbox, quad64_xbox; DevBuf<uint4> prim_info, oct, quad64; DevBuf<float> N, UV, T; DevBuf<DSphere> spheres; DevBuf<ftn_material> materials; DevBuf<DLight> lights;
     DevBuf<uint32_t> inf_lights; DevBuf<unsigned char> prim_class; std::vector<DevBuf<float>> misc; std::vector<DevBuf<float4>> misc4;
     DevBuf<ftn_texture> textures; DevBuf<ftn_material_textures> mtex; DevBuf<DImage> images; DevBuf<float4> texels;
     DevBuf<float4> accA, accB, accC; DevBuf<DTile> tiles; DevBuf<DevStats> stats; size_t acc_pixels = 0;
@@ -709,7 +796,7 @@
     WavefrontState* wf = nullptr;
     std::vector<DTile> sel; int32_t tile_key[10] = {0};
     ~ftn_scene() {
-        nodes.release(); geom.release(); fat.release(); srec.release(); quad.release(); oct.release(); oct_xbox.release(); prim_info.release(); N.release(); UV.release(); T.release(); spheres.release(); materials.release(); lights.release(); inf_lights.release(); prim_class.release();
+        nodes.release(); geom.release(); fat.release(); srec.release(); quad.release(); quad64.release(); quad64_xbox.release(); oct.release(); oct_xbox.release(); prim_info.release(); N.release(); UV.release(); T.release(); spheres.release(); materials.release(); lights.release(); inf_lights.release(); prim_class.release();
         for (auto& b : misc) b.release();
         for (auto& b : misc4) b.release();
         textures.release(); mtex.release(); images.release(); texels.release();
@@ -791,14 +878,26 @@
     clk.mark("upload nodes");
     if (n_fat && n_fat < (1u << 25)) { if ((rc = sc->fat.upload(fat.data(), fat.size()))) return rc; }
     uint32_t n_quads = 0, quad_bound = 0;
+    QuadBvh qb;
     if (!env_is("FTN_QUAD", 0)) {
-        QuadBvh qb; build_quads(hs.nodes, &qb);
+        build_quads(hs.nodes, &qb);
         if (qb.ok && qb.n_records) {
             if ((rc = sc->quad.upload(reinterpret_cast<const float4*>(qb.rec.data()), (size_t)8 * qb.n_records))) return rc;
             n_quads = qb.n_records; quad_bound = qb.stack_bound;
         }
     }
     clk.mark("four-box records (host + upload)");
+    uint32_t n_quad64 = 0, quad64_bound = 0;
+    if (!env_is("FTN_QUAD64", 0) && n_quads != 0 && d->n_spheres == 0) {
+        Quad64Bvh q6; build_quad64s(qb, geom, &q6);
+        if (q6.ok && q6.n_records) {
+            if ((rc = sc->quad64.upload(reinterpret_cast<const uint4*>(q6.rec.data()), (size_t)4 * q6.n_records))) return rc;
+            if (!q6.xbox.empty() && (rc = sc->quad64_xbox.upload(q6.xbox.data(), q6.xbox.size()))) return rc;
+            n_quad64 = q6.n_records; quad64_bound = q6.stack_bound;
+        }
+    }
+    qb = QuadBvh();
+    clk.mark("64-byte four-box records (host + upload)");
     uint32_t n_octs = 0, oct_bound = 0;
     if (!env_is("FTN_OCT", 0) && n_quads != 0 && d->n_spheres == 0) {
         OctBvh ob; build_octs(hs.nodes, geom, &ob);
@@ -963,6 +1062,7 @@
     D.srec = sc->srec.p; D.prim_class = sc->prim_class.p;
     D.quad = sc->quad.p; D.n_quads = n_quads; D.quad_stack_bound = quad_bound;
     D.oct = sc->oct.p; D.oct_xbox = sc->oct_xbox.p; D.n_octs = n_octs; D.oct_stack_bound = oct_bound;
+    D.quad64 = sc->quad64.p; D.quad64_xbox = sc->quad64_xbox.p; D.n_quad64 = n_quad64; D.quad64_stack_bound = quad64_bound;
     D.fat = sc->fat.p; D.n_fat = n_fat; D.root_is_leaf = (!hs.nodes.empty() && hs.nodes[0].is_leaf) ? 1u : 0u;
     for (int k = 0; k < 3; k++) { D.root_lo[k] = hs.nodes.empty() ? 0.0f : hs.nodes[0].bmin[k]; D.root_hi[k] = hs.nodes.empty() ? 0.0f : hs.nodes[0].bmax[k]; }
     if (lights.size() == 1 && lights[0].kind == LK_INFINITE) { D.env_only = 1; D.env0 = lights[0]; }
@@ -1041,6 +1141,21 @@
     return FTN_OK;
 }
 
+extern "C" int ftn_bvh_quad64s(const ftn_bvh_node* nodes, uint32_t n_nodes, uint32_t* records_out, uint32_t* n_records_out, uint32_t* stack_bound_out, float* xbox_out, uint32_t* n_xbox_out) {
+    if (!nodes && n_nodes) return fail(FTN_ERR_INVALID_ARGUMENT, "null nodes");
+    std::vector<ftn_bvh_node> v(nodes, nodes + n_nodes);
+    for (uint32_t i = 0; i < n_nodes; i++) if (!v[i].is_leaf && (v[i].idx <= i + 1 || v[i].idx >= n_nodes || v[i].axis > 2)) return fail(FTN_ERR_INVALID_ARGUMENT, "not a flattened BVH (bvh.rs:133-158)");
+    QuadBvh qb; build_quads(v, &qb);
+    Quad64Bvh q6; build_quad64s(qb, std::vector<float4>(), &q6);
+    if (!q6.ok) return fail(FTN_ERR_UNSUPPORTED, "no interior node, a non-finite box, or more than 2^24 four-box records");
+    if (records_out) memcpy(records_out, q6.rec.data(), q6.rec.size() * sizeof(uint32_t));
+    if (n_records_out) *n_records_out = q6.n_records;
+    if (stack_bound_out) *stack_bound_out = q6.stack_bound;
+    if (xbox_out) memcpy(xbox_out, q6.xbox.data(), q6.xbox.size() * sizeof(float4));
+    if (n_xbox_out) *n_xbox_out = (uint32_t)(q6.xbox.size() / 2);
+    return FTN_OK;
+}
+
 int ftn_bvh_octs(const ftn_bvh_node* nodes, uint32_t n_nodes, uint32_t* records_out, uint32_t* n_records_out, uint32_t* stack_bound_out, float* xbox_out, uint32_t* n_xbox_out) {
     if (!nodes && n_nodes) return fail(FTN_ERR_INVALID_ARGUMENT, "null nodes");
     std::vector<ftn_bvh_node> v(nodes, nodes + n_nodes);
@@ -1081,7 +1196,7 @@
     if (!s || !m) return fail(FTN_ERR_INVALID_ARGUMENT, "null scene / output");
     memset(m, 0, sizeof(*m));
     m->oct = s->oct.n * sizeof(uint4) + s->oct_xbox.n * sizeof(float4);
-    m->nodes = s->nodes.n * sizeof(float4); m->quad = s->quad.n * sizeof(float4); m->fat = s->fat.n * sizeof(float4); m->geom = s->geom.n * sizeof(float4);
+    m->nodes = s->nodes.n * sizeof(float4); m->quad = s->quad.n * sizeof(float4) + s->quad64.n * sizeof(uint4) + s->quad64_xbox.n * sizeof(float4); m->fat = s->fat.n * sizeof(float4); m->geom = s->geom.n * sizeof(float4);
     m->srec = s->srec.n * sizeof(float4); m->indexed_attributes = s->prim_info.n * sizeof(uint4) + (s->N.n + s->UV.n + s->T.n) * sizeof(float);
     m->prim_class = s->prim_class.n;
     m->lights = s->lights.n * sizeof(DLight) + s->inf_lights.n * sizeof(uint32_t);
diff --git a/fountain_amd/csrc/ftn_trace4.hip b/fountain_amd/csrc/ftn_trace4.hip
--- a/fountain_amd/csrc/ftn_trace4.hip
+++ b/fountain_amd/csrc/ftn_trace4.hip
@@ -72,6 +72,32 @@
     __device__ inline bool empty() const { return sp == base; }
 };
 
+enum : uint32_t { T8_IDLE = 0, T8_NODE = 1, T8_LEAF = 2, T8_LEAF_IN = 3  };
+#define T8_XBOX 0x40000000u
+__device__ inline bool ray_out_of_range8(float ox, float oy, float oz, float ix, float iy, float iz) {
+    const float big_i = 1.152921504606846976e18f , big_o = 1.099511627776e12f ;
+    return !(fabsf(ix) <= big_i && fabsf(iy) <= big_i && fabsf(iz) <= big_i && fabsf(ox) <= big_o && fabsf(oy) <= big_o && fabsf(oz) <= big_o);
+}
+struct T8Axis { float a, bn, bf; uint32_t n03, n47, f03, f47; };
+__device__ inline T8Axis t8_axis(float org, uint32_t ebyte, float o, float inv, uint32_t lo03, uint32_t lo47, uint32_t hi03, uint32_t hi47) {
+    T8Axis A;
+    const float step = __uint_as_float(ebyte << 23);
+    A.a = step * inv;
+    const float b = (org - o) * inv;
+    const float m = (fabsf(b) + 255.0f * fabsf(A.a)) * 9.5367431640625e-07f;
+    A.bn = b - m; A.bf = b + m;
+    const bool neg = inv < 0.0f;
+    A.n03 = neg ? hi03 : lo03; A.n47 = neg ? hi47 : lo47; A.f03 = neg ? lo03 : hi03; A.f47 = neg ? lo47 : hi47;
+    return A;
+}
+#define T8_BYTE(w, k) ((float)(((w) >> (8 * (k))) & 0xffu))
+#define T8_CHILD(c, t0v, t1v) \
+    { const uint32_t kx_ = (c) & 3; \
+      const t4_f2 tx_ = __builtin_elementwise_fma((t4_f2){T8_BYTE((c) < 4 ? X.n03 : X.n47, kx_), T8_BYTE((c) < 4 ? X.f03 : X.f47, kx_)}, (t4_f2){X.a, X.a}, (t4_f2){X.bn, X.bf}); \
+      const t4_f2 ty_ = __builtin_elementwise_fma((t4_f2){T8_BYTE((c) < 4 ? Y.n03 : Y.n47, kx_), T8_BYTE((c) < 4 ? Y.f03 : Y.f47, kx_)}, (t4_f2){Y.a, Y.a}, (t4_f2){Y.bn, Y.bf}); \
+      const t4_f2 tz_ = __builtin_elementwise_fma((t4_f2){T8_BYTE((c) < 4 ? Z.n03 : Z.n47, kx_), T8_BYTE((c) < 4 ? Z.f03 : Z.f47, kx_)}, (t4_f2){Z.a, Z.a}, (t4_f2){Z.bn, Z.bf}); \
+      t0v = fmax_(fmax_(fmax_(0.0f, tx_.x), ty_.x), tz_.x); t1v = fmin_(t_max, fmin_(fmin_(tx_.y, ty_.y), tz_.y) * k2); }
+
 struct T4Lane { uint32_t mode, cur, lp; bool finish; };
 
 template <bool CHECK>
@@ -87,14 +113,7 @@
 }
 
 template <bool CHECK>
-__device__ inline void t4_record_step(const DScene& S, const RaySetup& R, T4Stack<uint2>& St, T4Lane& L) {
-    const float4* rec = reinterpret_cast<const float4*>(reinterpret_cast<const char*>(S.quad) + L.cur);
-    const float4 q0 = rec[0], q1 = rec[1], q2 = rec[2], q3 = rec[3], q4 = rec[4], q5 = rec[5], q6 = rec[6], q7 = rec[7];
-    float ta, tb, tc, td, x1;
-    const bool ha = slab4(q0, q1, R.o, R.inv, R.t_max, &ta, &x1), hb = slab4(q2, q3, R.o, R.inv, R.t_max, &tb, &x1);
-    const bool hc = slab4(q4, q5, R.o, R.inv, R.t_max, &tc, &x1), hd = slab4(q6, q7, R.o, R.inv, R.t_max, &td, &x1);
-    const uint32_t ea = ha ? __float_as_uint(q1.z) : T4_NONE, eb = hb ? __float_as_uint(q3.z) : T4_NONE, ec = hc ? __float_as_uint(q5.z) : T4_NONE, ed = hd ? __float_as_uint(q7.z) : T4_NONE;
-    const uint32_t ax = __float_as_uint(q1.w) & R.neg24;
+__device__ __forceinline__ void t4_visit(T4Stack<uint2>& St, T4Lane& L, float t_max, uint32_t ea, uint32_t eb, uint32_t ec, uint32_t ed, float ta, float tb, float tc, float td, uint32_t ax) {
     const bool sA = (ax & 0xffu) != 0, sR = (ax & 0xff00u) != 0, sB = (ax & 0xff0000u) != 0;
     const uint32_t ex0 = sA ? eb : ea, ex1 = sA ? ea : eb, ey0 = sB ? ed : ec, ey1 = sB ? ec : ed;
     const float tx0 = sA ? tb : ta, tx1 = sA ? ta : tb, ty0 = sB ? td : tc, ty1 = sB ? tc : td;
@@ -108,11 +127,37 @@
     if (h012 || h3) {
         const uint32_t next = h0 ? e0 : (h1 ? e1 : (h2 ? e2 : e3));
         if (next >> 31) { L.lp = next & 0x7fffffffu; L.mode = T4_LEAF; } else L.cur = next;
-    } else t4_pop_next<CHECK>(St, L, R.t_max);
-}
-
-template <bool COUNT, bool SPHERES, int BURST>
-__global__ void __launch_bounds__(256, (SPHERES ? 1 : 5)) k_wf_trace4(DScene S, WfBuffers W, const uint32_t* __restrict__ queue, const uint32_t* count_ptr, uint32_t* head, DevStats* stats,
+    } else t4_pop_next<CHECK>(St, L, t_max);
+}
+
+template <bool CHECK>
+__device__ inline void t4_record_step(const DScene& S, const RaySetup& R, T4Stack<uint2>& St, T4Lane& L) {
+    const float4* rec = reinterpret_cast<const float4*>(reinterpret_cast<const char*>(S.quad) + L.cur);
+    const float4 q0 = rec[0], q1 = rec[1], q2 = rec[2], q3 = rec[3], q4 = rec[4], q5 = rec[5], q6 = rec[6], q7 = rec[7];
+    float ta, tb, tc, td, x1;
+    const bool ha = slab4(q0, q1, R.o, R.inv, R.t_max, &ta, &x1), hb = slab4(q2, q3, R.o, R.inv, R.t_max, &tb, &x1);
+    const bool hc = slab4(q4, q5, R.o, R.inv, R.t_max, &tc, &x1), hd = slab4(q6, q7, R.o, R.inv, R.t_max, &td, &x1);
+    const uint32_t ea = ha ? __float_as_uint(q1.z) : T4_NONE, eb = hb ? __float_as_uint(q3.z) : T4_NONE, ec = hc ? __float_as_uint(q5.z) : T4_NONE, ed = hd ? __float_as_uint(q7.z) : T4_NONE;
+    t4_visit<CHECK>(St, L, R.t_max, ea, eb, ec, ed, ta, tb, tc, td, __float_as_uint(q1.w) & R.neg24);
+}
+
+template <bool CHECK>
+__device__ __forceinline__ void t4q_record_step(const DScene& S, T4Stack<uint2>& St, T4Lane& L, V3 o, V3 inv, float t_max, uint32_t neg24) {
+    const uint4* rec = reinterpret_cast<const uint4*>(reinterpret_cast<const char*>(S.quad64) + L.cur);
+    const uint4 r0 = rec[0], r1 = rec[1], r2 = rec[2], r3 = rec[3];
+    const float k2 = 1.0f + 4.0f * gamma_n(3);
+    const T8Axis X = t8_axis(__uint_as_float(r0.x), r0.w & 0xffu, o.x, inv.x, r1.x, r1.x, r1.y, r1.y);
+    const T8Axis Y = t8_axis(__uint_as_float(r0.y), (r0.w >> 8) & 0xffu, o.y, inv.y, r1.z, r1.z, r1.w, r1.w);
+    const T8Axis Z = t8_axis(__uint_as_float(r0.z), (r0.w >> 16) & 0xffu, o.z, inv.z, r2.x, r2.x, r2.y, r2.y);
+    float ta, a1, tb, b1, tc, c1, td, d1;
+    T8_CHILD(0, ta, a1) T8_CHILD(1, tb, b1) T8_CHILD(2, tc, c1) T8_CHILD(3, td, d1)
+    const uint32_t ea = !(ta > a1) ? r2.z : T4_NONE, eb = !(tb > b1) ? r2.w : T4_NONE, ec = !(tc > c1) ? r3.x : T4_NONE, ed = !(td > d1) ? r3.y : T4_NONE;
+    t4_visit<CHECK>(St, L, t_max, ea, eb, ec, ed, ta, tb, tc, td, r3.z & neg24);
+}
+
+enum : uint32_t { T4_LEAF_IN = 3 };
+template <bool COUNT, bool SPHERES, int BURST, bool Q64 = false>
+__global__ void __launch_bounds__(256, (SPHERES ? 1 : (Q64 ? T4Q_WAVES : 5))) k_wf_trace4(DScene S, WfBuffers W, const uint32_t* __restrict__ queue, const uint32_t* count_ptr, uint32_t* head, DevStats* stats,
                                                    uint32_t refill, uint32_t leaf_batch, uint32_t chunk_max, uint32_t lds_entries, uint2* __restrict__ spill, uint32_t spill_levels) {
     T4Stack<uint2> St;
     extern __shared__ uint2 lds_stack2[];
@@ -149,7 +194,8 @@
                 load_queued_ray<false>(W, q_entry, &a, &b, &rid);
                 ray_setup<SPHERES>(R, a, b);
                 St.sp = St.base; L.cur = 0; found = false; hprim = -1; hb0 = 0.0f; hb1 = 0.0f; hb2 = 0.0f;
-                if (ray_is_exceptional(R.o.x, R.o.y, R.o.z, R.inv.x, R.inv.y, R.inv.z)) hand_back = true;
+                if (ray_is_exceptional(R.o.x, R.o.y, R.o.z, R.inv.x, R.inv.y, R.inv.z) || (Q64 && ray_out_of_range8(R.o.x, R.o.y, R.o.z, R.inv.x, R.inv.y, R.inv.z)))
+                    hand_back = true;
                 else if (S.n_nodes == 0 || !slab_test(rlo, rhi, R.o, R.inv, R.t_max)) { W.hit[rid] = make_float4(FTN_INF, 0.0f, 0.0f, 0.0f); W.hit_prim[rid] = -1; }
                 else if (S.root_is_leaf) { L.lp = 0; L.mode = T4_LEAF; }
                 else L.mode = T4_NODE;
@@ -157,7 +203,7 @@
             if (__ballot(hand_back) != 0) wave_push(hand_back, q_entry, W.q_exc_closest, &W.counters[CTR(32)]);
             Q.chunk_next += (need < avail ? need : avail);
         }
-        const unsigned long long m_node = __ballot(L.mode == T4_NODE), m_leaf = __ballot(L.mode == T4_LEAF);
+        const unsigned long long m_node = __ballot(L.mode == T4_NODE), m_leaf = __ballot(L.mode >= T4_LEAF);
         if ((m_node | m_leaf) == 0) { if (Q.exhausted) break; else continue; }
         L.finish = false;
         if (COUNT) occ[0]++;
@@ -167,21 +213,36 @@
                 const bool on = L.mode == T4_NODE && !L.finish;
                 if (COUNT && on) n_rec++;
                 if (COUNT) { const unsigned long long m_on = __ballot(on); if (m_on) { occ[1]++; occ[2] += (unsigned long long)__popcll(m_on); } }
-                if (__builtin_expect(__ballot(on && (st_tiny || St.sp > st_soft)) == 0, 1)) { if (on) t4_record_step<false>(S, R, St, L); }
-                else if (on) t4_record_step<true>(S, R, St, L);
+                if (__builtin_expect(__ballot(on && (st_tiny || St.sp > st_soft)) == 0, 1)) {
+                    if (on) { if (Q64) t4q_record_step<false>(S, St, L, R.o, R.inv, R.t_max, R.neg24); else t4_record_step<false>(S, R, St, L); }
+                } else if (on) { if (Q64) t4q_record_step<true>(S, St, L, R.o, R.inv, R.t_max, R.neg24); else t4_record_step<true>(S, R, St, L); }
             }
         } else {
             if (COUNT) { occ[3]++; occ[4] += (unsigned long long)__popcll(m_leaf); }
-            if (L.mode == T4_LEAF) {
-                const uint32_t prim = L.lp;
+            if (L.mode >= T4_LEAF) {
+                uint32_t prim = L.lp;
+                const bool entering = Q64 && L.mode == T4_LEAF, explicit_box = entering && (L.lp & T8_XBOX);
+                float4 x0 = make_float4(0.0f, 0.0f, 0.0f, 0.0f), x1 = x0;
+                if (Q64) prim &= 0x3fffffffu;
+                if (explicit_box) { x0 = S.quad64_xbox[2 * (size_t)prim]; x1 = S.quad64_xbox[2 * (size_t)prim + 1]; prim = __float_as_uint(x0.w); }
                 float4 g0 = S.geom[S.geom_stride * prim], g1 = S.geom[S.geom_stride * prim + 1], g2 = S.geom[S.geom_stride * prim + 2];
                 pin4(g0); pin4(g1); pin4(g2);
-                if (COUNT) n_prim++;
-                float t = 0.0f, b0 = 0.0f, b1 = 0.0f, b2 = 0.0f;
-                const bool hh = prim_hit<SPHERES>(S, prim, g0, g1, g2, R.o, R.dorig, R.t_max, R.kz, R.sx, R.sy, R.sz, &t, &b0, &b1, &b2);
-                if (hh) { found = true; R.t_max = t; hprim = (int)prim; hb0 = b0; hb1 = b1; hb2 = b2; }
-                if (__float_as_uint(g0.w) & GF_LEAF_END) t4_pop_next<true>(St, L, R.t_max);
-                else L.lp++;
+                bool pass = true;
+                if (entering) {
+                    if (!explicit_box) {
+                        x0 = make_float4(fmin_(fmin_(g0.x, g1.x), g2.x), fmin_(fmin_(g0.y, g1.y), g2.y), fmin_(fmin_(g0.z, g1.z), g2.z), 0.0f);
+                        x1 = make_float4(fmax_(fmax_(g0.x, g1.x), g2.x), fmax_(fmax_(g0.y, g1.y), g2.y), fmax_(fmax_(g0.z, g1.z), g2.z), 0.0f);
+                    }
+                    pass = slab_test(x0, x1, R.o, R.inv, R.t_max);
+                }
+                if (pass) {
+                    if (COUNT) n_prim++;
+                    float t = 0.0f, b0 = 0.0f, b1 = 0.0f, b2 = 0.0f;
+                    const bool hh = prim_hit<SPHERES>(S, prim, g0, g1, g2, R.o, R.dorig, R.t_max, R.kz, R.sx, R.sy, R.sz, &t, &b0, &b1, &b2);
+                    if (hh) { found = true; R.t_max = t; hprim = (int)prim; hb0 = b0; hb1 = b1; hb2 = b2; }
+                }
+                if (!pass || (__float_as_uint(g0.w) & GF_LEAF_END)) t4_pop_next<true>(St, L, R.t_max);
+                else { L.lp = prim + 1u; if (Q64) L.mode = T4_LEAF_IN; }
             }
         }
         if (L.finish) {
@@ -312,32 +373,6 @@
     if (blockIdx.x == 0 && threadIdx.x == 0) atomicAdd(&stats->rays_any, (unsigned long long)count);
 }
 
-enum : uint32_t { T8_IDLE = 0, T8_NODE = 1, T8_LEAF = 2, T8_LEAF_IN = 3  };
-#define T8_XBOX 0x40000000u
-__device__ inline bool ray_out_of_range8(float ox, float oy, float oz, float ix, float iy, float iz) {
-    const float big_i = 1.152921504606846976e18f , big_o = 1.099511627776e12f ;
-    return !(fabsf(ix) <= big_i && fabsf(iy) <= big_i && fabsf(iz) <= big_i && fabsf(ox) <= big_o && fabsf(oy) <= big_o && fabsf(oz) <= big_o);
-}
-struct T8Axis { float a, bn, bf; uint32_t n03, n47, f03, f47; };
-__device__ inline T8Axis t8_axis(float org, uint32_t ebyte, float o, float inv, uint32_t lo03, uint32_t lo47, uint32_t hi03, uint32_t hi47) {
-    T8Axis A;
-    const float step = __uint_as_float(ebyte << 23);
-    A.a = step * inv;
-    const float b = (org - o) * inv;
-    const float m = (fabsf(b) + 255.0f * fabsf(A.a)) * 9.5367431640625e-07f;
-    A.bn = b - m; A.bf = b + m;
-    const bool neg = inv < 0.0f;
-    A.n03 = neg ? hi03 : lo03; A.n47 = neg ? hi47 : lo47; A.f03 = neg ? lo03 : hi03; A.f47 = neg ? lo47 : hi47;
-    return A;
-}
-#define T8_BYTE(w, k) ((float)(((w) >> (8 * (k))) & 0xffu))
-#define T8_CHILD(c, t0v, t1v) \
-    { const uint32_t kx_ = (c) & 3; \
-      const t4_f2 tx_ = __builtin_elementwise_fma((t4_f2){T8_BYTE((c) < 4 ? X.n03 : X.n47, kx_), T8_BYTE((c) < 4 ? X.f03 : X.f47, kx_)}, (t4_f2){X.a, X.a}, (t4_f2){X.bn, X.bf}); \
-      const t4_f2 ty_ = __builtin_elementwise_fma((t4_f2){T8_BYTE((c) < 4 ? Y.n03 : Y.n47, kx_), T8_BYTE((c) < 4 ? Y.f03 : Y.f47, kx_)}, (t4_f2){Y.a, Y.a}, (t4_f2){Y.bn, Y.bf}); \
-      const t4_f2 tz_ = __builtin_elementwise_fma((t4_f2){T8_BYTE((c) < 4 ? Z.n03 : Z.n47, kx_), T8_BYTE((c) < 4 ? Z.f03 : Z.f47, kx_)}, (t4_f2){Z.a, Z.a}, (t4_f2){Z.bn, Z.bf}); \
-      t0v = fmax_(fmax_(fmax_(0.0f, tx_.x), ty_.x), tz_.x); t1v = fmin_(t_max, fmin_(fmin_(tx_.y, ty_.y), tz_.y) * k2); }
-
 template <bool CHECK, int POLICY>
 __device__ __forceinline__ void t8_any_step(const DScene& S, T4Stack<uint32_t>& St, T4Lane& L, V3 o, V3 inv, float t_max) {
     const uint4* rec = reinterpret_cast<const uint4*>(reinterpret_cast<const char*>(S.oct) + L.cur);
@@ -485,6 +520,17 @@
     p.lds_closest = (size_t)p.entries_closest * 256u * 8u; p.lds_any = (size_t)p.entries_any * 256u * 4u;
     auto per_cu = [](size_t lds, uint32_t wg) { return (unsigned)std::max<size_t>(1, std::min<size_t>(wg, (size_t)(158 * 1024) / std::max<size_t>(lds, 1))); };
     p.grid_closest = (unsigned)n_cu * per_cu(p.lds_closest, wg_c); p.grid_any = (unsigned)n_cu * per_cu(p.lds_any, wg_a);
+    if (S.quad64 && S.n_quad64) {
+        const uint32_t wg_q = knob_wg_closest ? knob_wg_closest : (uint32_t)T4Q_WAVES, budget_q = ((158u * 1024u) / wg_q) & ~1023u;
+        const uint32_t bound_q = S.quad64_stack_bound ? S.quad64_stack_bound : 1u;
+        uint32_t eq = knob_entries_closest ? knob_entries_closest : budget_q / (256u * 8u);
+        p.entries_q64 = eq < bound_q ? eq : bound_q;
+        if (p.entries_q64 == 0) p.entries_q64 = 1;
+        p.spill_q64 = bound_q - p.entries_q64;
+        p.lds_q64 = (size_t)p.entries_q64 * 256u * 8u;
+        p.grid_q64 = (unsigned)n_cu * per_cu(p.lds_q64, wg_q);
+        p.q64_ok = true;
+    }
     if (S.oct && S.n_octs) {
         const uint32_t wg_8 = knob_wg_oct ? knob_wg_oct : 5u, budget_8 = ((158u * 1024u) / wg_8) & ~1023u, bound8 = S.oct_stack_bound ? S.oct_stack_bound : 1u;
         const uint32_t e8 = knob_entries_oct ? knob_entries_oct : budget_8 / (256u * 4u);
@@ -499,9 +545,13 @@
 
 void launch_trace4(int kind, bool count, bool spheres, unsigned grid, size_t lds, uint32_t lds_entries, void* spill, hipStream_t stream, const DScene& S, const WfBuffers& W,
                    const uint32_t* queue, const uint32_t* count_ptr, uint32_t* head, DevStats* stats, uint32_t refill, uint32_t leaf_batch, uint32_t chunk, uint32_t burst, uint32_t any_policy, uint32_t spill_levels) {
-    const bool any = kind != T4K_CLOSEST;
+    const bool any = kind == T4K_ANY || kind == T4K_ANY_OCT;
 #define FTN_T4(K, SPILL_T, ...) hipLaunchKernelGGL((K<__VA_ARGS__>), dim3(grid), dim3(256), lds, stream, S, W, queue, count_ptr, head, stats, refill, leaf_batch, chunk, lds_entries, (SPILL_T)spill, spill_levels)
-    if (kind == T4K_ANY_OCT) {
+    if (kind == T4K_CLOSEST_Q64) {
+        if (count) FTN_T4(k_wf_trace4, uint2*, true, false, 2, true);
+        else if (burst <= 1) FTN_T4(k_wf_trace4, uint2*, false, false, 1, true); else if (burst == 2) FTN_T4(k_wf_trace4, uint2*, false, false, 2, true);
+        else if (burst == 3) FTN_T4(k_wf_trace4, uint2*, false, false, 3, true); else FTN_T4(k_wf_trace4, uint2*, false, false, 4, true);
+    } else if (kind == T4K_ANY_OCT) {
 #define FTN_T8(C, B) do { if (any_policy == 0) FTN_T4(k_wf_trace8_any, uint32_t*, C, B, 0); else FTN_T4(k_wf_trace8_any, uint32_t*, C, B, 1); } while (0)
         if (count) FTN_T8(true, 2);
         else if (burst <= 1) FTN_T8(false, 1); else if (burst == 2) FTN_T8(false, 2); else FTN_T8(false, 3);
diff --git a/fountain_amd/csrc/ftn_wavefront.hip b/fountain_amd/csrc/ftn_wavefront.hip
--- a/fountain_amd/csrc/ftn_wavefront.hip
+++ b/fountain_amd/csrc/ftn_wavefront.hip
@@ -1005,7 +1005,7 @@
     uint32_t* host_counters = nullptr;
     int n_cu = 256;
     void* dl_mem[8] = {nullptr, nullptr, nullptr, nullptr, nullptr, nullptr, nullptr, nullptr}; size_t dl_paths = 0; uint32_t dl_levels = 0, dl_slots = 0; bool dl_tex = false;
-    Trace4Plan t4; bool t4_on = false, t8_on = false;
+    Trace4Plan t4; bool t4_on = false, t8_on = false, q64_on = false;
     void* ser_mem[4] = {nullptr, nullptr, nullptr, nullptr}; size_t ser_paths = 0; bool ser_tex = false; uint32_t* ser_host = nullptr;
     void* t4_spill_c = nullptr; void* t4_spill_a = nullptr; size_t t4_spill_c_bytes = 0, t4_spill_a_bytes = 0;
 };
@@ -1080,7 +1080,9 @@
     st->t4_on = S.quad != nullptr && knob("FTN_TRACE4", 1) != 0;
     if (!st->t4_on) return FTN_OK;
     st->t4 = trace4_plan(S, st->n_cu, knob("FTN_T4_ENTRIES", 0), knob("FTN_T4_ENTRIES_ANY", 0), knob("FTN_T4_WG", 0), knob("FTN_T4_WG_ANY", 0), knob("FTN_T8_WG", 0), knob("FTN_T8_ENTRIES", 0));
-    const size_t need_c = (size_t)st->t4.grid_closest * 256u * st->t4.spill_closest * sizeof(uint2);
+    st->q64_on = st->t4.q64_ok && S.n_spheres == 0 && knob("FTN_QUAD64", 1) != 0;
+    const size_t need_c = std::max<size_t>((size_t)st->t4.grid_closest * 256u * st->t4.spill_closest * sizeof(uint2),
+                                           st->q64_on ? (size_t)st->t4.grid_q64 * 256u * st->t4.spill_q64 * sizeof(uint2) : 0);
     st->t8_on = st->t4.oct_ok && S.n_spheres == 0 && knob("FTN_T8", 1) != 0;
     const size_t need_a8 = st->t8_on ? (size_t)st->t4.grid_oct * 256u * st->t4.spill_oct * sizeof(uint32_t) : 0;
     const size_t need_a = std::max<size_t>(need_a8, (size_t)st->t4.grid_any * 256u * st->t4.spill_any * sizeof(uint32_t));
@@ -1093,17 +1095,18 @@
                          const uint32_t* queue, const uint32_t* count_ptr, uint32_t* head, uint32_t max_rays, bool camera_rays = false) {
     if (st->t4_on && count != 1) {
         const Trace4Plan& T = st->t4;
-        const bool oct = any && st->t8_on;
-        const unsigned g = std::min<unsigned>(oct ? T.grid_oct : (any ? T.grid_any : T.grid_closest), std::max<unsigned>(1u, (max_rays + 255u) / 256u));
+        const bool oct = any && st->t8_on, q64 = !any && st->q64_on;
+        const unsigned g = std::min<unsigned>(oct ? T.grid_oct : (any ? T.grid_any : (q64 ? T.grid_q64 : T.grid_closest)), std::max<unsigned>(1u, (max_rays + 255u) / 256u));
         uint32_t chunk4 = knob("FTN_TRACE_CHUNK", 128);
         while (chunk4 > 64u && (uint64_t)chunk4 * g * 4u * 4u > (uint64_t)max_rays) chunk4 >>= 1;
         if (oct) launch_trace4(T4K_ANY_OCT, count == 2, false, g, T.lds_oct, T.entries_oct, st->t4_spill_a, stream, P.S, W, queue, count_ptr, head, P.stats,
                                camera_rays ? knob("FTN_T8_REFILL1", 16) : knob("FTN_T8_REFILL", 24), camera_rays ? knob("FTN_T8_LEAF_BATCH1", 16) : knob("FTN_T8_LEAF_BATCH", 16), chunk4, knob("FTN_T8_BURST", 2), knob("FTN_T8_POLICY", 1), T.spill_oct);
-        else launch_trace4(any ? T4K_ANY : T4K_CLOSEST, count == 2, spheres, g, any ? T.lds_any : T.lds_closest, any ? T.entries_any : T.entries_closest, any ? st->t4_spill_a : st->t4_spill_c, stream, P.S, W,
+        else launch_trace4(any ? T4K_ANY : (q64 ? T4K_CLOSEST_Q64 : T4K_CLOSEST), count == 2, spheres, g, any ? T.lds_any : (q64 ? T.lds_q64 : T.lds_closest),
+                      any ? T.entries_any : (q64 ? T.entries_q64 : T.entries_closest), any ? st->t4_spill_a : st->t4_spill_c, stream, P.S, W,
                       queue, count_ptr, head, P.stats,
                       any ? knob("FTN_T4_ANY_REFILL", 32) : (camera_rays ? knob("FTN_T4_REFILL0", 64) : knob("FTN_T4_REFILL", 32)),
                       any ? knob("FTN_T4_ANY_LEAF_BATCH", 16) : (camera_rays ? knob("FTN_T4_LEAF_BATCH0", 2) : knob("FTN_T4_LEAF_BATCH", 16)), chunk4,
-                      any ? knob("FTN_T4_ANY_BURST", 4) : (camera_rays ? knob("FTN_T4_BURST0", 3) : knob("FTN_T4_BURST", 2)), knob("FTN_T4_ANY_POLICY", 1), any ? T.spill_any : T.spill_closest);
+                      any ? knob("FTN_T4_ANY_BURST", 4) : (camera_rays ? knob("FTN_T4_BURST0", 3) : knob("FTN_T4_BURST", 2)), knob("FTN_T4_ANY_POLICY", 1), any ? T.spill_any : (q64 ? T.spill_q64 : T.spill_closest));
         const unsigned ge = std::min<unsigned>(grid, (unsigned)st->n_cu);
         uint32_t* ecount = &W.counters[CTR(any ? 33 : 32)]; uint32_t* ehead = &W.counters[CTR(any ? 48 : 40)];
         DevStats* none = nullptr;
diff --git a/fountain_amd/csrc/ftn_wf_common.h b/fountain_amd/csrc/ftn_wf_common.h
--- a/fountain_amd/csrc/ftn_wf_common.h
+++ b/fountain_amd/csrc/ftn_wf_common.h
@@ -161,8 +161,12 @@
     size_t lds_closest, lds_any;
     unsigned grid_closest, grid_any;
     bool oct_ok; uint32_t entries_oct, spill_oct; size_t lds_oct; unsigned grid_oct;
+    bool q64_ok; uint32_t entries_q64, spill_q64; size_t lds_q64; unsigned grid_q64;
 };
-enum : int { T4K_CLOSEST = 0, T4K_ANY = 1, T4K_ANY_OCT = 2 };
+enum : int { T4K_CLOSEST = 0, T4K_ANY = 1, T4K_ANY_OCT = 2, T4K_CLOSEST_Q64 = 3 };
+#ifndef T4Q_WAVES
+#define T4Q_WAVES 6
+#endif
 Trace4Plan trace4_plan(const DScene& S, int n_cu, uint32_t knob_entries_closest, uint32_t knob_entries_any, uint32_t knob_wg_closest, uint32_t knob_wg_any, uint32_t knob_wg_oct, uint32_t knob_entries_oct);
 void launch_trace4(int kind, bool count, bool spheres, unsigned grid, size_t lds, uint32_t lds_entries, void* spill, hipStream_t stream, const DScene& S, const WfBuffers& W,
                    const uint32_t* queue, const uint32_t* count_ptr, uint32_t* head, DevStats* stats, uint32_t refill, uint32_t leaf_batch, uint32_t chunk, uint32_t burst, uint32_t any_policy, uint32_t spill_levels);
```

Result: faster. 3211, median of 6 (+4.0%).
